# NguyenThaiHoc1/CustomKnowledgeGraphEmbedding

Measured on AMD Instinct MI355X. Metric: scored (pos+neg) triples/sec, WN18RR InterHT d=1000 n_neg=256, 1/2/4/8 GPU, higher is better.
Workload: dtype f32; 1 GPU; WN18RR InterHT d=1000 -de -tr gamma=24 n_neg=256 bz=512; global_batch=512, n_neg=256, hidden_dim=1000, score_function=InterHT, parallelism=single

## Files before the change

### customknowledgegraphembedding_amd/_lib.py

```python
from __future__ import annotations

import ctypes
import os
import threading

_HERE = os.path.dirname(os.path.abspath(__file__))
LIB_PATH = os.environ.get("KGE_HIP_LIB", os.path.join(_HERE, "libkge_hip.so"))

FN_IDS = {
    "TransE": 0,
    "DistMult": 1,
    "ComplEx": 2,
    "RotatE": 3,
    "InterHT": 4,
    "pRotatE": 5,
    "PairRE": 7,
}
HEAD_BATCH, TAIL_BATCH, SINGLE = 0, 1, 3

_c_i64 = ctypes.c_int64
_c_f = ctypes.c_float
_c_p = ctypes.c_void_p
_c_i = ctypes.c_int



class Forms(ctypes.Structure):
    _fields_ = [("step_order", ctypes.c_int), ("xcd_phases", ctypes.c_int), ("tile_rows", ctypes.c_int),
                ("tile_q2slots", ctypes.c_int), ("tile_waves", ctypes.c_int), ("gemm_form", ctypes.c_int),
                ("transparse_form", ctypes.c_int)]


_ORDERS = {"row": 0, "xcd": 1, "tile": 2}


def forms(step_order=None, xcd_phases=0, tile_rows=0, tile_q2slots=None, tile_waves=0, gemm_form=0,
          transparse_form=0):
    so = -1 if step_order is None else (_ORDERS[step_order] if isinstance(step_order, str) else int(step_order))
    return Forms(so, int(xcd_phases), int(tile_rows or 0), -1 if tile_q2slots is None else int(tile_q2slots),
                 int(tile_waves or 0), int(gemm_form), int(transparse_form))


SIGNATURES = {
    "kge_abi_version": (_c_i, []),
    "kge_last_error": (ctypes.c_char_p, []),
    "kge_max_dim": (_c_i64, [_c_i]),
    "kge_step_forward_order": (_c_i, [_c_i64, _c_i64]),
    "kge_score_indexed": (
        _c_i,
        [_c_i, _c_i, _c_p, _c_i64, _c_i64, _c_p, _c_i64, _c_i64, _c_i64, _c_p, _c_p, _c_i64,
         _c_i64, _c_i64, _c_i64, _c_f, _c_f, _c_f, _c_p, _c_i64, _c_p],
    ),
    "kge_step_forward": (
        _c_i,
        [_c_i, _c_i, _c_p, _c_i64, _c_i64, _c_p, _c_i64, _c_i64, _c_i64, _c_p, _c_p, _c_i64,
         _c_i64, _c_i64, _c_i64, _c_f, _c_f, _c_f, _c_f, _c_i, _c_p, _c_i64, _c_p, _c_p, _c_p, _c_p, _c_p],
    ),
    "kge_score_indexed_ex": (
        _c_i,
        [_c_i, _c_i, _c_p, _c_i64, _c_i64, _c_p, _c_i64, _c_i64, _c_i64, _c_p, _c_p, _c_i64,
         _c_i64, _c_i64, _c_i64, _c_f, _c_f, _c_f, _c_p, _c_i64, _c_p, _c_p],
    ),
    "kge_step_forward_ex": (
        _c_i,
        [_c_i, _c_i, _c_p, _c_i64, _c_i64, _c_p, _c_i64, _c_i64, _c_i64, _c_p, _c_p, _c_i64,
         _c_i64, _c_i64, _c_i64, _c_f, _c_f, _c_f, _c_f, _c_i, _c_p, _c_i64, _c_p, _c_p, _c_p, _c_p, _c_p, _c_p],
    ),
    "kge_step_plan_size": (_c_i64, [_c_i, _c_i64, _c_i64, _c_i64, _c_i64, _c_i64, _c_i64, _c_i64, _c_i64]),
    "kge_step_plan": (
        _c_i, [_c_i, _c_i, _c_i64, _c_i64, _c_i64, _c_i64, _c_i64, _c_p, _c_p, _c_i64, _c_i64, _c_i64, _c_i64, _c_p,
               _c_p]),
    "kge_step_forward_planned": (
        _c_i,
        [_c_i, _c_i, _c_p, _c_i64, _c_i64, _c_p, _c_i64, _c_i64, _c_i64, _c_i64, _c_i64, _c_i64, _c_f, _c_f, _c_f,
         _c_f, _c_i, _c_p, _c_p, _c_p, _c_i64, _c_i, _c_p, _c_p, _c_i64, _c_p, _c_p, _c_p, _c_p],
    ),
    "kge_step_planner_create": (
        _c_i, [_c_p, _c_i, _c_p, _c_i64, _c_i64, _c_p, _c_i64, _c_i64, _c_i64, _c_i64, _c_i64, _c_i64, _c_f, _c_f, _c_f,
               _c_f, _c_i, _c_p, _c_p, _c_i64, _c_p]),
    "kge_step_planner_set_modulus": (_c_i, [_c_p, _c_f]),
    "kge_step_planner_set_sweep": (_c_i, [_c_p, _c_i]),
    "kge_step_planner_set_form": (_c_i, [_c_p, _c_i, _c_i]),
    "kge_step_board_size": (_c_i64, []),
    "kge_step_planner_set_board": (_c_i, [_c_p, _c_p, _c_i64]),
    "kge_step_planner_set_lead": (_c_i, [_c_p, _c_i]),
    "kge_step_planner_get": (_c_i, [_c_p, _c_i]),
    "kge_step_planner_plan_size": (_c_i64, [_c_i, _c_i64, _c_i64, _c_i64, _c_i64, _c_i64, _c_i64, _c_i64, _c_i64]),
    "kge_step_planner_set_rows": (_c_i, [_c_p, _c_i]),
    "kge_step_planned_rows": (_c_i, [_c_i, _c_i64, _c_i64, _c_i64, _c_i64, _c_i64, _c_i64, _c_i64, _c_i64, _c_i,
                                     _c_i64, _c_p]),
    "kge_step_planner_set_clocks": (_c_i, [_c_p, _c_p, _c_i64]),
    "kge_step_planner_plan": (_c_i, [_c_p, _c_p, _c_p, _c_i64, _c_i]),
    "kge_step_planner_step": (_c_i, [_c_p, _c_p, _c_p, _c_i64, _c_i, _c_p, _c_p, _c_p, _c_p]),
    "kge_step_planner_destroy": (_c_i, [_c_p]),
    "kge_step_finish": (
        _c_i,
        [_c_i, _c_p, _c_i64, _c_i64, _c_p, _c_i64, _c_i64, _c_i64, _c_p, _c_i64, _c_i64,
         _c_f, _c_f, _c_f, _c_p, _c_i64, _c_i64, _c_f, _c_i, _c_p, _c_p, _c_p, _c_p],
    ),
    "kge_score_sharded": (
        _c_i,
        [_c_i, _c_i, _c_p, _c_i64, _c_p, _c_i64, _c_i64, _c_i64, _c_p, _c_i64, _c_i64, _c_i64,
         _c_p, _c_p, _c_i64, _c_i64, _c_i64, _c_i64, _c_f, _c_f, _c_f, _c_p, _c_i64, _c_p],
    ),
    "kge_gather_rows": (
        _c_i, [_c_p, _c_i64, _c_i64, _c_i64, _c_p, _c_i64, _c_i64, _c_i64, _c_p, _c_i64, _c_p]),
    "kge_build_id": (ctypes.c_char_p, []),
    "kge_source_hash": (ctypes.c_char_p, []),
    "kge_shard_plan": (
        _c_i, [_c_p, _c_p, _c_i64, _c_i64, _c_i64, _c_i64, _c_i, _c_i, _c_i, _c_i, _c_i, _c_p, _c_p, _c_p, _c_p, _c_p,
               _c_p, _c_p, _c_p]),
    "kge_shard_gather_queries": (
        _c_i, [_c_p, _c_i64, _c_i64, _c_i64, _c_p, _c_i64, _c_i, _c_i, _c_i64, _c_i, _c_i, _c_i, _c_i, _c_p, _c_p,
               _c_p, _c_p, _c_p, _c_p]),
    "kge_shard_score": (
        _c_i,
        [_c_i, _c_i, _c_p, _c_i64, _c_i64, _c_p, _c_p, _c_i64, _c_i64, _c_i64, _c_p, _c_i64, _c_i64, _c_i64,
         _c_p, _c_i64, _c_i64, _c_i64, _c_f, _c_f, _c_f, _c_p, _c_p, _c_p, _c_p, _c_p, _c_i, _c_i, _c_i64,
         _c_i64, _c_p, _c_p],
    ),
    "kge_shard_finish": (
        _c_i, [_c_p, _c_p, _c_p, _c_p, _c_p, _c_i64, _c_i64, _c_i64, _c_i64, _c_i, _c_i, _c_i, _c_f, _c_i, _c_p,
               _c_i64, _c_p, _c_p, _c_p, _c_p]),
    "kge_comm_unique_id": (_c_i, [_c_p]),
    "kge_comm_loopback_group": (_c_p, [_c_i]),
    "kge_comm_loopback_group_destroy": (_c_i, [_c_p]),
    "kge_comm_loopback_init": (_c_i, [_c_p, _c_p, _c_i]),
    "kge_comm_init": (_c_i, [_c_p, _c_p, _c_i, _c_i]),
    "kge_comm_destroy": (_c_i, [_c_p]),
    "kge_comm_all_to_allv": (_c_i, [_c_p, _c_p, _c_p, _c_p, _c_p, _c_p]),
    "kge_comm_all_reduce_sum": (_c_i, [_c_p, _c_p, _c_i64, _c_p]),
    "kge_shard_exec_workspace_size": (_c_i64, [_c_i64, _c_i64, _c_i64, _c_i, _c_i]),
    "kge_shard_exec_host_ints": (_c_i64, [_c_i, _c_i]),
    "kge_shard_exec_create": (
        _c_i, [_c_p, _c_p, _c_i, _c_i, _c_i64, _c_i64, _c_i64, _c_i64, _c_i64, _c_i64, _c_i, _c_i, _c_i, _c_p, _c_i64,
               _c_p, _c_i64]),
    "kge_shard_exec_destroy": (_c_i, [_c_p]),
    "kge_shard_exec_host_wait_us": (ctypes.c_double, [_c_p, _c_i]),
    "kge_shard_exec_timings": (_c_i, [_c_p, _c_p, _c_i]),
    "kge_comm_size": (_c_i, [_c_p]),
    "kge_shard_exec_plan": (_c_i, [_c_p, _c_p, _c_p, _c_i64, _c_i, _c_p]),
    "kge_shard_exec_step": (
        _c_i, [_c_p, _c_p, _c_i64, _c_i64, _c_p, _c_i64, _c_i64, _c_i64, _c_p, _c_p, _c_i64, _c_i, _c_f, _c_f, _c_f,
               _c_f, _c_i, _c_p, _c_p, _c_i, _c_p, _c_i64, _c_p, _c_p, _c_p, _c_p]),
    "kge_eval_query": (
        _c_i, [_c_i, _c_i, _c_p, _c_i64, _c_i64, _c_p, _c_i64, _c_i64, _c_p, _c_i64, _c_i64, _c_p, _c_i64, _c_p]),
    "kge_eval_query_planes": (
        _c_i, [_c_i, _c_i, _c_p, _c_i64, _c_i64, _c_p, _c_i64, _c_i64, _c_p, _c_i64, _c_i64, _c_p, _c_i64, _c_p]),
    "kge_gemm_nt": (_c_i, [_c_p, _c_i64, _c_p, _c_i64, _c_p, _c_i64, _c_i64, _c_i64, _c_i64, _c_p]),
    "kge_gemm_nt_bf16x3": (_c_i, [_c_p, _c_i64, _c_p, _c_i64, _c_p, _c_i64, _c_i64, _c_i64, _c_i64, _c_p]),
    "kge_gemm_nt_bf16x3_ex": (_c_i, [_c_p, _c_i64, _c_p, _c_i64, _c_p, _c_i64, _c_i64, _c_i64, _c_i64, _c_p, _c_p]),
    "kge_split_bf16x3_bytes": (_c_i64, [_c_i64, _c_i64]),
    "kge_split_bf16x3": (_c_i, [_c_p, _c_i64, _c_i64, _c_i64, _c_p, _c_i64, _c_p]),
    "kge_gemm_nt_bf16x3_planes": (_c_i, [_c_p, _c_i64, _c_p, _c_i64, _c_i64, _c_p, _c_i64, _c_i64, _c_i64, _c_p]),
    "kge_eval_rank_planes_workspace_size": (_c_i64, [_c_i64, _c_i64]),
    "kge_eval_rank_planes": (_c_i, [_c_p, _c_i64, _c_p, _c_i64, _c_i64, _c_i64, _c_i64, _c_p, _c_p, _c_p, _c_i64, _c_p,
                                    _c_p, ctypes.c_size_t, _c_p]),
    "kge_eval_rank_planes_ex": (_c_i, [_c_p, _c_i64, _c_p, _c_i64, _c_i64, _c_i64, _c_i64, _c_p, _c_p, _c_p, _c_i64,
                                       _c_p, _c_p, ctypes.c_size_t, _c_p, _c_p]),
    "kge_eval_rank_planes_phases": (_c_i, [_c_p, _c_i64, _c_p, _c_i64, _c_i64, _c_i64, _c_i64, _c_p, _c_p, _c_p,
                                           _c_i64, _c_p, _c_p, ctypes.c_size_t, _c_i, _c_p, _c_p]),
    "kge_eval_rank_sweep_workspace_size": (_c_i64, [_c_i64, _c_i64]),
    "kge_eval_rank_sweep": (_c_i, [_c_i, _c_i, _c_p, _c_i64, _c_i64, _c_p, _c_i64, _c_i64, _c_i64, _c_p, _c_i64, _c_i64,
                                   _c_f, _c_f, _c_f, _c_p, _c_p, _c_p, _c_i64, _c_p, _c_p, ctypes.c_size_t, _c_p]),
    "kge_eval_rank_candidates": (_c_i, [_c_i, _c_i, _c_p, _c_i64, _c_i64, _c_p, _c_i64, _c_i64, _c_i64, _c_p, _c_i64,
                                        _c_i64, _c_f, _c_f, _c_f, _c_p, _c_p, _c_i64, _c_i64, _c_p, _c_p, _c_i64, _c_p,
                                        _c_p, _c_p, _c_p]),
    "kge_eval_topk_sweep_workspace_size": (_c_i64, [_c_i64, _c_i64]),
    "kge_eval_topk_sweep": (_c_i, [_c_i, _c_i, _c_p, _c_i64, _c_i64, _c_p, _c_i64, _c_i64, _c_i64, _c_p, _c_i64, _c_i64,
                                   _c_f, _c_f, _c_f, _c_p, _c_p, _c_i64, _c_i64, _c_p, _c_i64, _c_p, _c_i64, _c_p,
                                   ctypes.c_size_t, _c_p]),
    "kge_topk_rows": (_c_i, [_c_p, _c_i64, _c_i64, _c_i64, _c_p, _c_p, _c_i64, _c_i64, _c_p, _c_i64, _c_p, _c_i64,
                             _c_p]),
    "kge_eval_topk_planes_workspace_size": (_c_i64, [_c_i64, _c_i64, _c_i64]),
    "kge_eval_topk_planes": (_c_i, [_c_p, _c_i64, _c_p, _c_i64, _c_i64, _c_i64, _c_i64, _c_p, _c_p, _c_i64, _c_i64,
                                    _c_p, _c_i64, _c_p, _c_i64, _c_p, ctypes.c_size_t, _c_p]),
    "kge_gemm_nt_bf16x3_planes_ex": (_c_i, [_c_p, _c_i64, _c_p, _c_i64, _c_i64, _c_p, _c_i64, _c_i64, _c_i64, _c_p,
                                            _c_p]),
    "kge_rank_filtered": (_c_i, [_c_p, _c_i64, _c_i64, _c_i64, _c_p, _c_p, _c_p, _c_p, _c_p]),
    "kge_score_dense": (
        _c_i,
        [_c_i, _c_i, _c_p, _c_i64, _c_p, _c_i64, _c_i64, _c_p, _c_i64, _c_i64, _c_i64, _c_i64,
         _c_f, _c_f, _c_f, _c_p, _c_i64, _c_p],
    ),
    "kge_score_dense_bwd": (
        _c_i,
        [_c_i, _c_i, _c_p, _c_i64, _c_p, _c_i64, _c_i64, _c_p, _c_i64, _c_i64, _c_i64, _c_i64,
         _c_f, _c_f, _c_f, _c_p, _c_i64, _c_p, _c_p, _c_p, _c_p, _c_p],
    ),
    "kge_neg_reduce": (_c_i, [_c_p, _c_i64, _c_i64, _c_i64, _c_f, _c_i, _c_p, _c_p]),
    "kge_neg_reduce_bwd": (
        _c_i, [_c_p, _c_i64, _c_i64, _c_i64, _c_f, _c_i, _c_i, _c_p, _c_p, _c_i64, _c_p]),
    "kge_log_sigmoid": (_c_i, [_c_p, _c_i64, _c_p, _c_p]),
    "kge_log_sigmoid_bwd": (_c_i, [_c_p, _c_p, _c_i64, _c_p, _c_p]),
    "kge_adam_update": (
        _c_i, [_c_p, _c_p, _c_p, _c_p, _c_i64, _c_f, _c_f, _c_f, _c_f, _c_i64, _c_i, _c_i, _c_p]),
    "kge_step_backward_workspace_size": (_c_i64, [_c_i, _c_i64, _c_i64, _c_i64, _c_i64]),
    "kge_step_backward": (
        _c_i,
        [_c_i, _c_i, _c_p, _c_i64, _c_i64, _c_p, _c_i64, _c_i64, _c_i64, _c_p, _c_p, _c_i64,
         _c_i64, _c_i64, _c_i64, _c_f, _c_f, _c_f, _c_f, _c_i, _c_i, _c_p, _c_i64, _c_p, _c_p, _c_p,
         _c_p, _c_p, _c_p, _c_p, _c_p, _c_i64, _c_p],
    ),
    "kge_step_backward_adam_workspace_size": (_c_i64, [_c_i, _c_i64, _c_i64, _c_i64, _c_i64, _c_i64, _c_i64]),
    "kge_step_backward_adam": (
        _c_i,
        [_c_i, _c_i, _c_p, _c_i64, _c_i64, _c_p, _c_i64, _c_i64, _c_i64, _c_p, _c_p, _c_i64,
         _c_i64, _c_i64, _c_i64, _c_f, _c_f, _c_p, _c_f, _c_f, _c_i, _c_i, _c_p, _c_i64, _c_p, _c_p, _c_p,
         _c_p, _c_p, _c_p, _c_p, _c_p, _c_p, _c_f, _c_f, _c_f, _c_f, _c_i64, _c_i, _c_p, _c_p, _c_i64, _c_p],
    ),
    "kge_train_step_workspace_size": (_c_i64, [_c_i, _c_i64, _c_i64, _c_i64, _c_i64, _c_i64, _c_i64]),
    "kge_train_step": (
        _c_i,
        [_c_i, _c_i, _c_p, _c_i64, _c_i64, _c_p, _c_i64, _c_i64, _c_i64, _c_p, _c_p, _c_i64,
         _c_i64, _c_i64, _c_i64, _c_f, _c_f, _c_f, _c_i, _c_i, _c_p, _c_p, _c_p, _c_p, _c_p,
         _c_p, _c_p, _c_p, _c_p, _c_f, _c_f, _c_f, _c_f, _c_i64, _c_i, _c_p, _c_i64, _c_p],
    ),
    "kge_train_step_reg_workspace_size": (_c_i64, [_c_i, _c_i64, _c_i64, _c_i64, _c_i64, _c_i64, _c_i64]),
    "kge_train_step_reg": (
        _c_i,
        [_c_i, _c_i, _c_p, _c_i64, _c_i64, _c_p, _c_i64, _c_i64, _c_i64, _c_p, _c_p, _c_i64,
         _c_i64, _c_i64, _c_i64, _c_f, _c_f, _c_f, _c_i, _c_i, _c_p, _c_p, _c_p, _c_p, _c_p,
         _c_p, _c_p, _c_p, _c_p, _c_f, _c_f, _c_f, _c_f, _c_i64, _c_i, _c_p, _c_i64, _c_p, _c_f, _c_p],
    ),
    "kge_train_step_lazy_workspace_size": (_c_i64, [_c_i, _c_i64, _c_i64, _c_i64, _c_i64, _c_i64, _c_i64]),
    "kge_train_step_lazy": (
        _c_i,
        [_c_i, _c_i, _c_p, _c_i64, _c_i64, _c_p, _c_i64, _c_i64, _c_i64, _c_p, _c_p, _c_i64,
         _c_i64, _c_i64, _c_i64, _c_f, _c_f, _c_f, _c_i, _c_i, _c_p, _c_p, _c_p, _c_p, _c_p,
         _c_p, _c_p, _c_p, _c_p, _c_f, _c_f, _c_f, _c_f, _c_i64, _c_i, _c_p, _c_i64, _c_p, _c_p],
    ),
    "kge_sampler_create": (_c_p, [_c_p, _c_i64, _c_i64, _c_i64, _c_i64, _c_i]),
    "kge_sampler_seed": (_c_i, [_c_p, ctypes.c_uint32]),
    "kge_sampler_get": (_c_i, [_c_p, _c_p, _c_i64, _c_p, _c_p, _c_p]),
    "kge_sampler_destroy": (None, [_c_p]),
    "kge_dsampler_table_size": (_c_i64, [_c_i64]),
    "kge_dsampler_table_build": (_c_i, [_c_p, _c_i64, _c_i64, _c_i64, _c_p, _c_i64]),
    "kge_dsampler_sample": (_c_i, [_c_p, _c_i64, _c_p, _c_i64, _c_i64, _c_i64, _c_i, ctypes.c_uint64, _c_i64, _c_p,
                                   _c_p, _c_p, _c_i64, _c_p, _c_p]),
    "kge_filter_table_size": (_c_i64, [_c_i64]),
    "kge_filter_table_build": (_c_i, [_c_p, _c_i64, _c_p, _c_i64]),
# ... 101 lines not shown
```

### customknowledgegraphembedding_amd/csrc/kge_abi.hip

```cpp
#include <string.h>

#include <algorithm>
#include <cmath>

#include <string>

#include "kge_device.h"
#include "kge_scan.h"

namespace kge_impl {
namespace {

__global__ __launch_bounds__(kBlock) void neg_reduce_kernel(const float* __restrict__ s, int64_t B, int64_t N,
                                                            int64_t ld, float T, int adversarial,
                                                            float* __restrict__ out) {
    const int64_t b = (int64_t)blockIdx.x * kWavesPerBlock + (threadIdx.x >> 6);
    if (b >= B) return;
    const int lane = threadIdx.x & 63;
    const float res = row_reduce_fast(s + b * ld, N, T, adversarial, lane);
    if (lane == 0) out[b] = res;
}

__global__ __launch_bounds__(kBlock) void neg_rows_kernel(ScoreParams p) {
    const int64_t b = (int64_t)blockIdx.x * kWavesPerBlock + (threadIdx.x >> 6);
// ... 379 lines not shown

int check_launch(const char* what) {
    const hipError_t e = hipGetLastError();
    if (e != hipSuccess) return fail(KGE_EHIP, std::string(what) + ": " + hipGetErrorString(e));
    return ok();
}

bool aligned(const void* ptr, int bytes) { return ptr == nullptr || ((uintptr_t)ptr % (uintptr_t)bytes) == 0; }

bool valid_fn(int fn) {
    switch (fn) {
        case KGE_TRANSE:
        case KGE_DISTMULT:
        case KGE_COMPLEX:
        case KGE_ROTATE:
        case KGE_INTERHT:
        case KGE_PROTATE:
        case KGE_PAIRRE: return true;
        default: return false;
    }
}

int check_rel_width(int fn, int64_t D, int64_t rel_off, int64_t rel_ld) {
    if (fn == KGE_PAIRRE && (rel_off < 0 || rel_ld < rel_off + 2 * D))
        return fail(KGE_EINVAL, "PairRE relation rows hold two halves: rel_ld >= rel_off + 2 D");
    return 0;
}

int refuse_sharded(int fn, const char* who) {
    if (fn == KGE_PAIRRE) return fail(KGE_ENOTSUP, std::string(who) + ": PairRE has no row-sharded form");
    return 0;
}

struct Tables {
    int fn;
    const float* ent;
    int64_t nentity, ent_ld;
    const float* rel;
    int64_t nrelation, rel_ld, rel_off;
    int64_t D;
    float gamma, emb_range, modulus;
};
struct Batch {
    int mode;
    const int64_t* pos;
    const int64_t* neg;
    int64_t neg_ld, B, N;
};
struct StepGrads {
    float temperature;
    int adversarial, detach;
    const float* neg_scores;
    int64_t ns_ld;
    const float* pos_scores;
    const float* d_out_neg;
    const float* d_out_pos;
    float* d_ent;
    float* d_rel;
    float* d_modulus;
    const float* cand_stats;
};

int pick_vg(const ScoreParams& p, int& V, int& G) {
    const int cand[3] = {4, 2, 1};
    V = 1;
    for (int v : cand) {
        if (p.D % v == 0 && p.q_ld % v == 0 && p.r_ld % v == 0 && p.r_off % v == 0 && p.c_ld % v == 0 &&
            aligned(p.qent, 4 * v) && aligned(p.rel, 4 * v) && aligned(p.cent, 4 * v) &&
            aligned(p.qent_pos, 4 * v) && aligned(p.sh_dq, 4 * v)) {
            V = v;
            break;
        }
    }
    const int groups = (p.D / V + kWave - 1) / kWave;
    G = 1;
    while (G < groups) G <<= 1;
    if (G > kMaxG)
        return fail(KGE_ENOTSUP, "per-half dim " + std::to_string(p.D) + " exceeds the register-resident limit " +
                                     std::to_string(kMaxG * kWave * V) + " for vector width " + std::to_string(V));
    return 0;
}

int pick_cpw(int64_t B, int64_t N) {
    if (N <= 1) return 1;
    int64_t cpw = 16;
    while (cpw > 4 && B * ((N + cpw - 1) / cpw) < 8192) cpw >>= 1;
    return (int)cpw;
}

int pick_cpw_sharded(int64_t B, int64_t N) {
    if (N <= 1) return 1;
    int64_t cpw = 512;
    while (cpw > 16 && B * ((N + cpw - 1) / cpw) < 8192) cpw >>= 1;
    return (int)cpw;
}

int dispatch(int fn, const ScoreParams& p, int kind, hipStream_t st, int blocks, bool ch, int V, int G) {
    switch (fn) {
        case KGE_TRANSE: return launch_transe(p, kind, st, blocks, ch, V, G);
        case KGE_DISTMULT: return launch_distmult(p, kind, st, blocks, ch, V, G);
        case KGE_COMPLEX: return launch_complex(p, kind, st, blocks, ch, V, G);
        case KGE_ROTATE: return launch_rotate(p, kind, st, blocks, ch, V, G);
        case KGE_INTERHT: return launch_interht(p, kind, st, blocks, ch, V, G);
        case KGE_PROTATE: return launch_protate(p, kind, st, blocks, ch, V, G);
        case KGE_PAIRRE: return launch_pairre(p, kind, st, blocks, ch, V, G);
        default: return KGE_EINVAL;
    }
}

int check_fn_mode(int fn, int mode) {
    if (mode != KGE_HEAD_BATCH && mode != KGE_TAIL_BATCH && mode != KGE_SINGLE)
        return fail(KGE_EINVAL, "mode must be 0 (head-batch), 1 (tail-batch) or 3 (single)");
    if (!valid_fn(fn)) return fail(KGE_EINVAL, "unknown score function id " + std::to_string(fn));
    return 0;
}

int run_score(int fn, int mode, ScoreParams& p, int kind, void* stream) {
    int rc = check_fn_mode(fn, mode);
    if (rc) return rc;
    if (p.B < 0 || p.N < 0 || p.D <= 0) return fail(KGE_EINVAL, "bad shape (B, N, D)");
    if (p.B == 0 || (p.N == 0 && kind != KIND_RANK_CAND)) return ok();
    const bool no_rows =
        p.c_rows == 0 && (kind == KIND_SHARD_FWD_GRAD || kind == KIND_SHARD_POS || kind == KIND_SHARD_EPILOGUE);
    rc = check_rel_width(fn, p.D, p.r_off, p.r_ld);
    if (rc) return rc;
    if (!p.qent || !p.rel || (!p.cent && !no_rows)) return fail(KGE_EINVAL, "null table pointer");
    int V = 1, G = 1;
    rc = pick_vg(p, V, G);
    if (rc) return rc;
    if (kind == KIND_BWD) {
        int g1 = 1;
        while (g1 * kWave < p.D) g1 <<= 1;
        if (g1 <= kBwdMaxG) {
            V = 1;
            G = g1;
        }
    }
    const KindInfo& k = kKinds[kind];
    int64_t waves = 0;
    switch (k.grid) {
        case GRID_WAVE_PER_ROW:
            if (kind == KIND_FINISH) p.cpw = p.wpr = 1;
            waves = p.B;
            break;
        case GRID_BLOCK_PER_ROW: waves = p.B * kWavesPerBlock; break;
        case GRID_WAVE_PER_ENT: waves = p.lz_list ? p.lz_rows : p.c_rows; break;
        case GRID_BLOCK_PER_ENT: waves = (p.lz_list ? p.lz_rows : p.c_rows) * kWavesPerBlock; break;
        case GRID_XCD_SLICES:
            waves = (p.B + kWavesPerBlock - 1) / kWavesPerBlock * kWavesPerBlock * 8;
            if (kind == KIND_STEP_FWD_XCD && p.xcd_phases > 1) waves *= p.xcd_phases;
            break;
        case GRID_TILE_GROUPS: {
            if (p.tile_rows < 1 || p.tile_lds > kTileLdsMax) return fail(KGE_EINVAL, "tile plan missing");
            const int64_t groups = (p.B + p.tile_rows - 1) / p.tile_rows;
            p.tile_blocks = (int)(groups * 8);
            waves = (groups * 8 + (p.tile_next.plan ? p.tile_plan_blocks : 0)) * kWavesPerBlock;
            break;
        }
        case GRID_CAND_PER_WAVE:
            p.cpw = p.skip_foreign ? pick_cpw_sharded(p.B, p.N) : pick_cpw(p.B, p.N);
            p.wpr = (int)((p.N + p.cpw - 1) / p.cpw);
            waves = p.B * p.wpr;
            break;
        case GRID_STEP_EPILOGUE: {
            const int64_t ev = p.B * p.N + 3 * p.B;
            const int64_t sb = std::min<int64_t>(std::max<int64_t>((ev + 4 * kBlock - 1) / (4 * kBlock), 1), 256);
            waves = (3 * p.B + kWavesPerBlock - 1) / kWavesPerBlock * kWavesPerBlock + (sb + 1) * kWavesPerBlock;
            break;
        }
        case GRID_SHARD_EPILOGUE:
            waves = (2 * p.B + kWavesPerBlock - 1) / kWavesPerBlock * kWavesPerBlock + kWavesPerBlock;
            break;
        case GRID_RANK_PAIRS: waves = p.B + p.rk.nf; break;
        case GRID_RANK_SWEEP:
            if (p.tile_rows < 1 || p.rk.chunks < 1 || p.tile_lds > kTileLdsMax) return fail(KGE_EINVAL, "sweep plan missing");
            waves = (p.B + p.tile_rows - 1) / p.tile_rows * 8 * p.rk.chunks * kWavesPerBlock;
            break;
        case GRID_TOPK_SWEEP:
            if (p.tile_rows < 1 || p.tk.chunks < 1 || p.tile_lds > kTileLdsMax || p.tk.k < 1 || p.tk.k > kTopkMax || !p.tk.parts)
                return fail(KGE_EINVAL, "sweep plan missing");
            waves = (p.B + p.tile_rows - 1) / p.tile_rows * 8 * p.tk.chunks * kWavesPerBlock;
            break;
        case GRID_RANK_CAND: {
            p.wpr = rank_cand_wpr(p.N);
            const int64_t rows = kWavesPerBlock / p.wpr;
            waves = (p.B + rows - 1) / rows * kWavesPerBlock;
            break;
        }
    }
    const int64_t blocks = (waves + kWavesPerBlock - 1) / kWavesPerBlock;
    if (blocks > INT32_MAX) return fail(KGE_EINVAL, "problem too large for one launch");
    const bool ch = k.ch && mode == KGE_HEAD_BATCH;
    if (k.no_protate && (G > k.max_g || fn == KGE_PROTATE))
        return fail(KGE_ENOTSUP, "the fused forward + query gradient needs D / V <= 256 and no pRotatE");
    if (G > k.max_g) return fail(KGE_ENOTSUP, "dimension too large");
    if (k.g_whole_waves && G % kWavesPerBlock) return fail(KGE_ENOTSUP, "the streaming backward needs G % 4 == 0");
    rc = kind_has(kind, fn, ch, G) ? dispatch(fn, p, kind, (hipStream_t)stream, (int)blocks, ch, V, G) : KGE_ENOTSUP;
    if (rc) return fail(rc, "no kernel for this (function, width) combination");
    return check_launch(k.what);
}

float phase_div_for(int fn, float emb_range) {
    const double pi = (fn == KGE_PROTATE) ? 3.14159262358979323846 : 3.14159265358979323846;
    return (float)((double)emb_range / pi);
}

void fill_indexed(ScoreParams& p, const Tables& t, const Batch& b) {
    memset(&p, 0, sizeof(p));
    const bool ch = b.mode == KGE_HEAD_BATCH;
    p.qent = t.ent;
    p.q_idx = b.pos ? b.pos + (ch ? 2 : 0) : nullptr;
    p.q_ld = t.ent_ld;
    p.q_stride = 3;
    p.q_rows = t.nentity;
    p.rel = t.rel;
    p.r_idx = b.pos ? b.pos + 1 : nullptr;
    p.r_ld = t.rel_ld;
    p.r_stride = 3;
    p.r_rows = t.nrelation;
    p.r_off = t.rel_off;
    p.cent = t.ent;
    p.c_ld = t.ent_ld;
    p.c_rows = t.nentity;
    if (b.mode == KGE_SINGLE) {
        p.c_idx = b.pos ? b.pos + 2 : nullptr;
        p.c_stride = 3;
    } else {
        p.c_idx = b.neg;
        p.c_stride = b.neg_ld;
    }
    p.B = b.B;
    p.N = b.mode == KGE_SINGLE ? 1 : b.N;
    p.D = (int)t.D;
    p.gamma = t.gamma;
    p.phase_div = phase_div_for(t.fn, t.emb_range);
    p.modulus = t.modulus;
}
Batch single_of(const Batch& b) { return {KGE_SINGLE, b.pos, nullptr, 0, b.B, 1}; }

void fill_dense(ScoreParams& p, int fn, int mode, const float* head, int64_t head_ld, const float* rel,
                int64_t rel_ld, int64_t rel_off, const float* tail, int64_t tail_ld, int64_t B, int64_t N, int64_t D,
                float gamma, float emb_range, float modulus) {
    memset(&p, 0, sizeof(p));
    const bool ch = mode == KGE_HEAD_BATCH;
    if (mode == KGE_SINGLE) N = 1;
    p.qent = ch ? tail : head;
    p.q_ld = ch ? tail_ld : head_ld;
    p.q_rows = B;
    p.rel = rel;
    p.r_ld = rel_ld;
    p.r_off = rel_off;
    p.r_rows = B;
    p.cent = ch ? head : tail;
    p.c_ld = ch ? head_ld : tail_ld;
    p.c_dense = N;
    p.c_rows = B * N;
    p.B = B;
    p.N = N;
    p.D = (int)D;
    p.gamma = gamma;
    p.phase_div = phase_div_for(fn, emb_range);
    p.modulus = modulus;
}

bool empty(int64_t B, int64_t N) { return B == 0 || N == 0; }

int xcd_phases(int64_t nentity, int64_t ent_ld, const kge_forms* forms) {
    const int forced = forms ? forms->xcd_phases : 0;
    if (forced > 0) return std::min(forced, 16);
    const int64_t bytes = nentity * ent_ld * 4, mall = (int64_t)256 << 20, phase = (int64_t)96 << 20;
    if (bytes <= mall) return 1;
    return (int)std::min<int64_t>((bytes + phase - 1) / phase, 8);
}

int step_order(int64_t nentity, int64_t N, const kge_forms* forms = nullptr) {
    const int forced = forms ? forms->step_order : -1;
    if (nentity >= (int64_t)8 << 25) return 0;
    if (forced >= 0 && forced <= 2) return forced;
    return N >= 128 ? 2 : 0;
}
bool use_xcd_order(int64_t nentity, int64_t N, const kge_forms* forms = nullptr) {
    return step_order(nentity, N, forms) != 0;
}

int tile_plan(int fn, ScoreParams& p, const kge_forms* forms = nullptr) {
    int V = 1, G = 1;
    if (pick_vg(p, V, G)) return 0;
    if (G > kFwdGradMaxG || p.N + 1 > 65536 || p.c_rows <= 0) return 0;
    const int64_t opb = (int64_t)G * kWave * V * 4;
    int64_t P2 = 0;
    if (fn == KGE_INTERHT && p.B <= kTileSortMaxB) {
        P2 = kWave;
        while (P2 < p.B) P2 <<= 1;
    }
    const int64_t row_bytes = (int64_t)p.D * 4 * (is_split(fn) ? 2 : 1);
    p.tile_waves = row_bytes >= 4096 ? 12 : 16;
    p.tile_depth = 2;
    const int fw = forms ? forms->tile_waves : 0;
    if (fw == 8 || fw == 12 || fw == 16) p.tile_waves = fw;
    const int64_t NT = (int64_t)p.tile_waves * kWave;
    const int64_t qrow = tile_nq(fn) * opb + 8 + 8 + 8 + 4, lrow = (p.N + 1) * 4;
    const int64_t fixed = kTileBuckets * 4 + 16;
    const int64_t sort_ints = P2 ? (kTileSortMaxB + NT - 1) / NT * p.tile_waves * kTileSortRel : 0;
    auto lds = [&](int64_t R, int64_t QS) { return R * qrow + QS * opb + fixed + std::max(R * lrow, sort_ints * 4); };
    int64_t R = kTileRows;
    if (forms && forms->tile_rows > 0) R = std::min<int64_t>(R, forms->tile_rows);
    while (R >= 1 && lds(R, 0) > kTileLdsMax) --R;
    if (R < 1) return 0;
    int64_t QS = 0;
    if (fn == KGE_INTERHT)
        while (QS < R && lds(R, QS + 1) <= kTileLdsMax) ++QS;
    if (forms && forms->tile_q2slots >= 0) QS = std::min<int64_t>(QS, forms->tile_q2slots);
#ifdef KGE_PROFILING_KNOBS
    p.tile_dry = getenv("KGE_TILE_DRY") ? std::max(1, atoi(getenv("KGE_TILE_DRY"))) : 0;
    if (getenv("KGE_TILE_NOSORT")) P2 = 0;
#endif
    p.tile_rows = (int)R;
    p.tile_q2slots = (int)QS;
    p.tile_sort = (int)P2;
    p.tile_lds = (int)lds(R, QS);
    return 1;
}

int planned_tile_params(const Tables& t, int64_t B, int64_t N, ScoreParams& p, const kge_forms* forms = nullptr) {
    if (B <= 0 || N <= 0 || t.D <= 0 || t.nentity <= 0 || t.nentity >= ((int64_t)1 << 31) || B >= ((int64_t)1 << 31))
        return 0;
    Tables a = t;
    a.ent = a.rel = reinterpret_cast<const float*>((uintptr_t)4096);
    fill_indexed(p, a, {KGE_TAIL_BATCH, nullptr, nullptr, 0, B, N});
    return tile_plan(t.fn, p, forms) ? p.tile_rows : 0;
}

int planned_tile_layout(int fn, ScoreParams& p, int64_t R) {
    int V = 1, G = 1;
    if (pick_vg(p, V, G)) return 0;
    const int64_t opb = (int64_t)G * kWave * V * 4;
    const int64_t qrow = tile_nq(fn) * opb + 8 + 8 + 8 + 4, fixed = kTileBuckets * 4 + 16;
    auto lds = [&](int64_t r, int64_t qs) { return r * qrow + qs * opb + fixed; };
    if (R < 1 || R > std::min(kTileMaxRows, 2 * p.tile_waves) || lds(R, 0) > kTileLdsMax) return 0;
    int64_t QS = 0;
    if (fn == KGE_INTERHT)
        while (QS < R && lds(R, QS + 1) <= kTileLdsMax) ++QS;
    p.tile_rows = (int)R;
    p.tile_q2slots = (int)QS;
    p.tile_lds = (int)lds(R, QS);
    return 1;
}

template <class Cap>
int planned_rows_rule(const Tables& t, int64_t B, int64_t N, int waves, int64_t plan_bytes, Cap cap) {
    ScoreParams tp;
    const int R0 = planned_tile_params(t, B, N, tp);
    if (!R0) return 0;
    const int qs0 = tp.tile_q2slots;
    if (waves) tp.tile_waves = waves;
    const int64_t c0 = cap(R0);
    if (c0 <= 0 || 8 * plan_groups(B, R0) <= c0 - 8) return R0;
    for (int R = R0 + 1; R <= kTileMaxRows; ++R) {
        if (!planned_tile_layout(t.fn, tp, R) || tp.tile_q2slots < qs0) continue;
        if (plan_bytes > 0 && plan_words(B, N, R) * 4 > plan_bytes) continue;
        const int64_t c = cap(R);
        if (c > 0 && 8 * plan_groups(B, R) <= c - 8) return R;
    }
    return R0;
}

struct SweepForm {
    int waves, depth, lead, tag;
    int rev;
    int* board;
    long long* clk;
};

void planned_sweep_defaults(int fn, int64_t D, int& waves, int& depth, int& lead) {
    const int64_t row_bytes = D * 4 * (is_split(fn) ? 2 : 1);
    waves = row_bytes >= 4096 ? 12 : 16;
    depth = 2;
    lead = 0;
    if (row_bytes >= 4096 && fn == KGE_INTERHT) lead = 12;
    if (row_bytes >= 4096 && fn == KGE_ROTATE) depth = 1;
}

PlanArgs plan_args(const ScoreParams& tp, const Tables& t, const Batch& b, void* plan) {
    PlanArgs a;
    a.pos = b.pos;
    a.neg = b.neg;
    a.neg_ld = b.neg_ld;
    a.B = b.B;
    a.N = b.N;
    a.nent = t.nentity;
    a.nrel = t.nrelation;
    a.mode = b.mode;
    a.R = tp.tile_rows;
    a.sort = tp.tile_sort != 0;
    a.plan = reinterpret_cast<int*>(plan);
    return a;
}

int launch_neg_rows(const ScoreParams& p, const char* what, void* stream) {
    const int64_t blocks = (p.B + kWavesPerBlock - 1) / kWavesPerBlock;
    hipLaunchKernelGGL(neg_rows_kernel, dim3((unsigned)blocks), dim3(kBlock), 0, (hipStream_t)stream, p);
    return check_launch(what);
}

}

int set_error(int code, const char* msg) { return fail(code, msg); }
}

using namespace kge_impl;

extern "C" {

int kge_abi_version(void) { return KGE_ABI_VERSION; }

const char* kge_last_error(void) { return g_last_error.c_str(); }

int64_t kge_max_dim(int fn) {
    if (!valid_fn(fn)) return 0;
    return (int64_t)kMaxG * kWave * 4;
}

int kge_step_forward_order(int64_t nentity, int64_t N) { return step_order(nentity, N); }

int kge_score_indexed(int fn, int mode, const float* ent, int64_t nentity, int64_t ent_ld, const float* rel,
                      int64_t nrelation, int64_t rel_ld, int64_t rel_off, const int64_t* pos, const int64_t* neg,
                      int64_t neg_ld, int64_t B, int64_t N, int64_t D, float gamma, float emb_range, float modulus,
                      float* scores, int64_t scores_ld, void* stream) {
    return kge_score_indexed_ex(fn, mode, ent, nentity, ent_ld, rel, nrelation, rel_ld, rel_off, pos, neg, neg_ld, B,
                                N, D, gamma, emb_range, modulus, scores, scores_ld, nullptr, stream);
}

int kge_score_indexed_ex(int fn, int mode, const float* ent, int64_t nentity, int64_t ent_ld, const float* rel,
                         int64_t nrelation, int64_t rel_ld, int64_t rel_off, const int64_t* pos, const int64_t* neg,
                         int64_t neg_ld, int64_t B, int64_t N, int64_t D, float gamma, float emb_range, float modulus,
                         float* scores, int64_t scores_ld, const kge_forms* forms, void* stream) {
    int rc = check_fn_mode(fn, mode);
    if (rc) return rc;
    if (B < 0 || N < 0 || D <= 0) return fail(KGE_EINVAL, "bad shape (B, N, D)");
    if (empty(B, mode == KGE_SINGLE ? 1 : N)) return ok();
    if (!pos) return fail(KGE_EINVAL, "pos must not be NULL");
    if (mode != KGE_SINGLE && !neg) return fail(KGE_EINVAL, "neg must not be NULL in head/tail-batch mode");
    if (!scores) return fail(KGE_EINVAL, "scores must not be NULL");
    const Tables t = {fn, ent, nentity, ent_ld, rel, nrelation, rel_ld, rel_off, D, gamma, emb_range, modulus};
    ScoreParams p;
    fill_indexed(p, t, {mode, pos, neg, neg_ld, B, N});
    p.out = scores;
    p.out_ld = scores_ld;
    if (mode != KGE_SINGLE && nentity < ((int64_t)1 << 31) && use_xcd_order(nentity, N, forms)) {
        if (step_order(nentity, N, forms) == 2 && tile_plan(fn, p, forms))
            return run_score(fn, mode, p, KIND_SCORE_TILE, stream);
        return run_score(fn, mode, p, KIND_SCORE_SHARD_XCD, stream);
    }
    return run_score(fn, mode, p, KIND_FWD, stream);
}

int kge_step_finish(int fn, const float* ent, int64_t nentity, int64_t ent_ld, const float* rel, int64_t nrelation,
                    int64_t rel_ld, int64_t rel_off, const int64_t* pos, int64_t B, int64_t D, float gamma,
                    float emb_range, float modulus, const float* neg_scores, int64_t N, int64_t ns_ld,
                    float temperature, int adversarial, float* out_neg, float* pos_scores, float* out_pos,
                    void* stream) {
    int rc = check_fn_mode(fn, KGE_SINGLE);
    if (rc) return rc;
    if (B < 0 || N <= 0 || D <= 0) return fail(KGE_EINVAL, "bad shape (B, N, D)");
    if (B == 0) return ok();
    if (!pos || !neg_scores || !out_neg || !out_pos) return fail(KGE_EINVAL, "null pointer");
    const Tables t = {fn, ent, nentity, ent_ld, rel, nrelation, rel_ld, rel_off, D, gamma, emb_range, modulus};
    ScoreParams f;
    fill_indexed(f, t, {KGE_SINGLE, pos, nullptr, 0, B, 1});
    f.neg_scores = neg_scores;
    f.ns_ld = ns_ld;
    f.n_neg = N;
    f.temperature = temperature;
    f.adversarial = adversarial;
    f.out_neg = out_neg;
    f.out_pos_raw = pos_scores;
    f.out_pos_ls = out_pos;
    return run_score(fn, KGE_SINGLE, f, KIND_FINISH, stream);
}

int kge_step_forward(int fn, int mode, const float* ent, int64_t nentity, int64_t ent_ld, const float* rel,
                     int64_t nrelation, int64_t rel_ld, int64_t rel_off, const int64_t* pos, const int64_t* neg,
                     int64_t neg_ld, int64_t B, int64_t N, int64_t D, float gamma, float emb_range, float modulus,
                     float temperature, int adversarial, float* neg_scores, int64_t ns_ld, float* out_neg,
                     float* pos_scores, float* out_pos, float* cand_stats, void* stream) {
    return kge_step_forward_ex(fn, mode, ent, nentity, ent_ld, rel, nrelation, rel_ld, rel_off, pos, neg, neg_ld, B, N,
                               D, gamma, emb_range, modulus, temperature, adversarial, neg_scores, ns_ld, out_neg,
                               pos_scores, out_pos, cand_stats, nullptr, stream);
}

int kge_step_forward_ex(int fn, int mode, const float* ent, int64_t nentity, int64_t ent_ld, const float* rel,
                        int64_t nrelation, int64_t rel_ld, int64_t rel_off, const int64_t* pos, const int64_t* neg,
                        int64_t neg_ld, int64_t B, int64_t N, int64_t D, float gamma, float emb_range, float modulus,
                        float temperature, int adversarial, float* neg_scores, int64_t ns_ld, float* out_neg,
                        float* pos_scores, float* out_pos, float* cand_stats, const kge_forms* forms, void* stream) {
    int rc = check_fn_mode(fn, mode);
    if (rc) return rc;
    if (mode == KGE_SINGLE) return fail(KGE_EINVAL, "kge_step_forward needs a negative mode (0 or 1)");
    if (B < 0 || N <= 0 || D <= 0) return fail(KGE_EINVAL, "bad shape (B, N, D)");
    if (B == 0) return ok();
    if (!pos || !neg || !neg_scores || !out_neg || !out_pos) return fail(KGE_EINVAL, "null pointer");
    const Tables t = {fn, ent, nentity, ent_ld, rel, nrelation, rel_ld, rel_off, D, gamma, emb_range, modulus};
    ScoreParams p;
    fill_indexed(p, t, {mode, pos, neg, neg_ld, B, N});
    p.out = neg_scores;
    p.out_ld = ns_ld;
    p.cand_stats = reinterpret_cast<float2*>(cand_stats);
    p.pos_base = pos;
    p.temperature = temperature;
    p.adversarial = adversarial;
    p.out_neg = out_neg;
    p.out_pos_raw = pos_scores;
    p.out_pos_ls = out_pos;
    const int order = step_order(nentity, N, forms);
    if (!(cand_stats && fn == KGE_INTERHT) && order != 0) {
        if (order == 2 && tile_plan(fn, p, forms)) {
            p.tile_pos = 1;
            rc = run_score(fn, mode, p, KIND_STEP_FWD_TILE, stream);
        } else {
            p.xcd_phases = xcd_phases(nentity, ent_ld, forms);
            rc = run_score(fn, mode, p, KIND_STEP_FWD_XCD, stream);
        }
        if (rc) return rc;
        return launch_neg_rows(p, "kge_step_forward row reductions", stream);
    }
    return run_score(fn, mode, p, (cand_stats && fn == KGE_INTERHT) ? KIND_STEP_FWD_STATS : KIND_STEP_FWD, stream);
}

static int64_t step_plan_bytes(const Tables& t, int64_t B, int64_t N) {
    if (!valid_fn(t.fn)) return 0;
    ScoreParams tp;
    const int R = planned_tile_params(t, B, N, tp);
    return R ? plan_words(B, N, R) * 4 : 0;
}

int64_t kge_step_plan_size(int fn, int64_t nentity, int64_t ent_ld, int64_t nrelation, int64_t rel_ld,
                           int64_t rel_off, int64_t B, int64_t N, int64_t D) {
    return step_plan_bytes({fn, nullptr, nentity, ent_ld, nullptr, nrelation, rel_ld, rel_off, D, 0.f, 0.f, 0.f}, B, N);
}

static int step_plan(const Tables& t, const Batch& b, void* plan, void* stream, int rows = 0) {
    if (!valid_fn(t.fn)) return fail(KGE_EINVAL, "unknown score function id " + std::to_string(t.fn));
    if (b.mode != KGE_HEAD_BATCH && b.mode != KGE_TAIL_BATCH)
        return fail(KGE_EINVAL, "kge_step_plan needs a negative mode (0 or 1)");
    if (b.B <= 0 || b.N <= 0 || t.D <= 0) return fail(KGE_EINVAL, "bad shape (B, N, D)");
    if (!b.pos || !b.neg || !plan) return fail(KGE_EINVAL, "null pointer");
    if (!aligned(plan, 16)) return fail(KGE_EINVAL, "the plan must be 16-B aligned");
    ScoreParams tp;
    if (!planned_tile_params(t, b.B, b.N, tp))
        return fail(KGE_ENOTSUP, "the tile form does not apply to this shape (kge_step_plan_size is 0)");
    if (rows) tp.tile_rows = rows;
    const PlanArgs a = plan_args(tp, t, b, plan);
    const unsigned groups = (unsigned)plan_groups(b.B, tp.tile_rows);
    if (tp.tile_waves == 16)
        hipLaunchKernelGGL(tile_plan_kernel<16>, dim3(groups), dim3(16 * kWave), plan_lds_ints(16 * kWave) * 4,
                           (hipStream_t)stream, a);
    else
        hipLaunchKernelGGL(tile_plan_kernel<12>, dim3(groups), dim3(12 * kWave), plan_lds_ints(12 * kWave) * 4,
                           (hipStream_t)stream, a);
    return check_launch("kge_step_plan");
}

int kge_step_plan(int fn, int mode, int64_t nentity, int64_t ent_ld, int64_t nrelation, int64_t rel_ld,
                  int64_t rel_off, const int64_t* pos, const int64_t* neg, int64_t neg_ld, int64_t B, int64_t N,
                  int64_t D, void* plan, void* stream) {
    return step_plan({fn, nullptr, nentity, ent_ld, nullptr, nrelation, rel_ld, rel_off, D, 0.f, 0.f, 0.f},
                     {mode, pos, neg, neg_ld, B, N}, plan, stream);
}

struct StepOut {
    float* neg_scores;
    int64_t ns_ld;
    float *out_neg, *pos_scores, *out_pos;
};

static int step_forward_planned(const Tables& t, const Batch& b, float temperature, int adversarial, const void* plan,
                                const Batch& next, void* next_plan, const StepOut& o, const SweepForm* sf,
                                void* stream, int rows = 0, int* occ = nullptr, int plan_blocks = 0) {
    int rc = check_fn_mode(t.fn, b.mode);
    if (rc) return rc;
    if (b.mode == KGE_SINGLE) return fail(KGE_EINVAL, "kge_step_forward_planned needs a negative mode (0 or 1)");
    if (b.B <= 0 || b.N <= 0 || t.D <= 0) return fail(KGE_EINVAL, "bad shape (B, N, D)");
    if (!t.ent || !t.rel || !plan || !o.neg_scores || !o.out_neg || !o.out_pos) return fail(KGE_EINVAL, "null pointer");
    if (next_plan) {
        if (next.mode != KGE_HEAD_BATCH && next.mode != KGE_TAIL_BATCH)
            return fail(KGE_EINVAL, "the next batch needs a negative mode (0 or 1)");
        if (!next.pos || !next.neg) return fail(KGE_EINVAL, "next_plan needs next_pos and next_neg");
        if (next_plan == plan) return fail(KGE_EINVAL, "next_plan must not be the plan this step reads");
        if (!aligned(next_plan, 16)) return fail(KGE_EINVAL, "the plan must be 16-B aligned");
    }
    if (!aligned(plan, 16)) return fail(KGE_EINVAL, "the plan must be 16-B aligned");
    ScoreParams tp;
    const int R = planned_tile_params(t, b.B, b.N, tp);
    ScoreParams p;
    fill_indexed(p, t, {b.mode, nullptr, nullptr, 0, b.B, b.N});
    kge_forms fm = {-1, 0, 0, -1, sf ? sf->waves : 0, 0, 0};
    if (!R || !tile_plan(t.fn, p, &fm) || p.tile_rows != R)
        return fail(KGE_ENOTSUP, "the tile form does not apply to these tables (unaligned rows, or "
                                 "kge_step_plan_size is 0): use kge_step_forward");
    if (!planned_tile_layout(t.fn, p, rows ? rows : R))
        return fail(KGE_ENOTSUP, "this many rows per group do not fit a block of the planned step");
    tp.tile_rows = p.tile_rows;
    p.out = o.neg_scores;
    p.out_ld = o.ns_ld;
    p.pos_base = nullptr;
    p.temperature = temperature;
    p.adversarial = adversarial;
    p.out_neg = o.out_neg;
    p.out_pos_raw = o.pos_scores;
    p.out_pos_ls = o.out_pos;
    p.tile_pos = 1;
    p.tile_plan = reinterpret_cast<const int*>(plan);
    if (sf) {
        p.tile_rev = sf->rev;
        p.tile_depth = sf->depth;
        p.tile_board = sf->board;
        p.tile_tag = sf->tag;
        p.tile_lead = sf->lead;
        p.tile_clk = sf->clk;
    }
    if (next_plan) {
        p.tile_next = plan_args(tp, t, next, next_plan);
        const int ng = (int)plan_groups(next.B, tp.tile_rows);
        p.tile_plan_blocks = (plan_blocks > 0 && p.tile_waves == kTileSharedWaves) ? std::min(plan_blocks, ng) : ng;
        p.tile_lds = std::max(p.tile_lds, plan_lds_ints(p.tile_waves * kWave) * 4);
    }
    p.tile_occ = occ;
    rc = run_score(t.fn, b.mode, p, KIND_STEP_FWD_TILE, stream);
    if (rc || occ) return rc;
    return launch_neg_rows(p, "kge_step_forward_planned row reductions", stream);
}

int kge_step_forward_planned(int fn, int mode, const float* ent, int64_t nentity, int64_t ent_ld, const float* rel,
                             int64_t nrelation, int64_t rel_ld, int64_t rel_off, int64_t B, int64_t N, int64_t D,
                             float gamma, float emb_range, float modulus, float temperature, int adversarial,
                             const void* plan, const int64_t* next_pos, const int64_t* next_neg, int64_t next_neg_ld,
                             int next_mode, void* next_plan, float* neg_scores, int64_t ns_ld, float* out_neg,
                             float* pos_scores, float* out_pos, void* stream) {
    const Tables t = {fn, ent, nentity, ent_ld, rel, nrelation, rel_ld, rel_off, D, gamma, emb_range, modulus};
    return step_forward_planned(t, {mode, nullptr, nullptr, 0, B, N}, temperature, adversarial, plan,
                                {next_mode, next_pos, next_neg, next_neg_ld, B, N}, next_plan,
                                {neg_scores, ns_ld, out_neg, pos_scores, out_pos}, nullptr, stream);
}

int planner_row_rule(int fn, int64_t D) {
    const int64_t row_bytes = D * 4 * (is_split(fn) ? 2 : 1);
    return row_bytes >= 4096 && (fn == KGE_INTERHT || fn == KGE_ROTATE);
}

struct kge_step_planner {
    Tables t = {};
    int64_t B = 0, N = 0;
    float temperature = 1.f;
    int adversarial = 1;
    void* plans[2] = {nullptr, nullptr};
    int cur = -1;
    int mode = 0;
    int sweep = 1;
    int waves = 0, depth = 0, lead = -1;
    int* board = nullptr;
    long long* clk = nullptr;
    int cus = 0;
    int64_t groups = 0;
    int rows = 0;
    int rule = 0;
    int plan_blocks = 0;
    int64_t plan_bytes = 0;
    int64_t steps = 0;
    void* stream = nullptr;
};

static SweepForm planner_form(const kge_step_planner* sp, int64_t groups = -1) {
    if (groups < 0) groups = sp->groups;
    SweepForm f = {0, 0, 0, 0, sp->sweep ? (int)(sp->steps & 1) : 0, nullptr, sp->clk};
    planned_sweep_defaults(sp->t.fn, sp->t.D, f.waves, f.depth, f.lead);
    if (sp->waves) f.waves = sp->waves;
    if (sp->depth) f.depth = sp->depth;
    if (f.waves == 8) f.depth = 2;
    if (sp->lead >= 0) f.lead = sp->lead;
    f.tag = (int)(sp->steps % kSweepTagMask) + 1;
    if (sp->board && f.lead > 0 && groups <= kSweepBoardLine && groups * 8 <= sp->cus) f.board = sp->board;
    return f;
}

static int64_t planner_capacity(const kge_step_planner* sp, int R) {
    if (sp->cus <= 0) return 0;
    const SweepForm sf = planner_form(sp, plan_groups(sp->B, R));
    int per_cu = INT32_MAX;
    float* const none = reinterpret_cast<float*>(sp->plans[0]);
    const int64_t* const ids = reinterpret_cast<const int64_t*>(sp->plans[0]);
    for (int mode : {KGE_HEAD_BATCH, KGE_TAIL_BATCH}) {
        int occ = 0;
        if (step_forward_planned(sp->t, {mode, nullptr, nullptr, 0, sp->B, sp->N}, sp->temperature, sp->adversarial,
                                 sp->plans[0], {mode, ids, ids, sp->N, sp->B, sp->N}, sp->plans[1],
                                 {none, sp->N, none, none, none}, &sf, sp->stream, R, &occ, 8))
            return 0;
        per_cu = std::min(per_cu, occ);
    }
    return (int64_t)sp->cus * per_cu;
}

static int planner_rows(kge_step_planner* sp) {
    if (!sp->rows) {
        sp->rows = planned_rows_rule(sp->t, sp->B, sp->N, planner_form(sp).waves, sp->plan_bytes,
                                     [&](int R) { return sp->rule ? planner_capacity(sp, R) : 0; });
        if (plan_groups(sp->B, sp->rows) > sp->groups) sp->clk = nullptr;
        sp->groups = plan_groups(sp->B, sp->rows);
        const int64_t cap = sp->rule ? planner_capacity(sp, sp->rows) : 0;
        sp->plan_blocks = (cap > 0 && 8 * sp->groups <= cap - 8) ? 8 : 0;
    }
    return sp->rows;
}

int64_t kge_step_planner_plan_size(int fn, int64_t nentity, int64_t ent_ld, int64_t nrelation, int64_t rel_ld,
                                   int64_t rel_off, int64_t B, int64_t N, int64_t D) {
    const Tables t = {fn, nullptr, nentity, ent_ld, nullptr, nrelation, rel_ld, rel_off, D, 0.f, 0.f, 0.f};
    if (!valid_fn(fn)) return 0;
    ScoreParams tp;
    const int R0 = planned_tile_params(t, B, N, tp);
    int64_t words = 0;
    for (int R = R0; R0 && R <= kTileMaxRows; ++R) words = std::max(words, plan_words(B, N, R));
    return words * 4;
}

int kge_step_planned_rows(int fn, int64_t nentity, int64_t ent_ld, int64_t nrelation, int64_t rel_ld, int64_t rel_off,
                          int64_t B, int64_t N, int64_t D, int waves, int64_t capacity, int* out) {
    if (!valid_fn(fn)) return fail(KGE_EINVAL, "unknown score function id " + std::to_string(fn));
    if (!out || (waves != 0 && waves != 8 && waves != 12 && waves != 16))
        return fail(KGE_EINVAL, "kge_step_planned_rows: out[4]; waves 0, 8, 12 or 16");
    const Tables t = {fn, nullptr, nentity, ent_ld, nullptr, nrelation, rel_ld, rel_off, D, 0.f, 0.f, 0.f};
    const int R = planned_rows_rule(t, B, N, waves, 0, [&](int) { return capacity; });
    ScoreParams tp;
    if (!R || !planned_tile_params(t, B, N, tp)) return fail(KGE_ENOTSUP, "the tile form does not apply to this shape");
    if (waves) tp.tile_waves = waves;
    if (!planned_tile_layout(fn, tp, R)) return fail(KGE_ENOTSUP, "the rows do not fit this wave count");
    out[0] = R;
    out[1] = tp.tile_q2slots;
    out[2] = std::max(tp.tile_lds, plan_lds_ints(tp.tile_waves * kWave) * 4);
    out[3] = (int)(8 * plan_groups(B, R));
    return ok();
}

int kge_step_planner_create(kge_step_planner** out, int fn, const float* ent, int64_t nentity, int64_t ent_ld,
                            const float* rel, int64_t nrelation, int64_t rel_ld, int64_t rel_off, int64_t B, int64_t N,
                            int64_t D, float gamma, float emb_range, float modulus, float temperature, int adversarial,
                            void* plan0, void* plan1, int64_t plan_bytes, void* stream) {
    if (!out) return fail(KGE_EINVAL, "kge_step_planner_create: null pointer");
    *out = nullptr;
    const Tables t = {fn, ent, nentity, ent_ld, rel, nrelation, rel_ld, rel_off, D, gamma, emb_range, modulus};
    const int64_t need = step_plan_bytes(t, B, N);
    if (need <= 0) return fail(KGE_ENOTSUP, "kge_step_planner_create: the tile form does not apply to this shape");
    if (!ent || !rel || !plan0 || !plan1 || plan0 == plan1) return fail(KGE_EINVAL, "kge_step_planner_create: bad pointers");
    if (plan_bytes < need || !aligned(plan0, 16) || !aligned(plan1, 16))
        return fail(KGE_EINVAL, "kge_step_planner_create: plan buffers too small or not 16-B aligned");
    kge_step_planner* sp = new kge_step_planner;
    sp->t = t;
    sp->B = B;
    sp->N = N;
    sp->temperature = temperature;
    sp->adversarial = adversarial;
    sp->plans[0] = plan0;
    sp->plans[1] = plan1;
    sp->stream = stream;
    sp->plan_bytes = plan_bytes;
    sp->rule = planner_row_rule(fn, D);
    ScoreParams tp;
    sp->groups = plan_groups(B, planned_tile_params(t, B, N, tp));
    int dev = 0;
    if (hipGetDevice(&dev) != hipSuccess ||
        hipDeviceGetAttribute(&sp->cus, hipDeviceAttributeMultiprocessorCount, dev) != hipSuccess)
        sp->cus = 0;
    *out = sp;
    return ok();
}

int kge_step_planner_set_form(kge_step_planner* sp, int waves, int depth) {
    if (!sp) return fail(KGE_EINVAL, "kge_step_planner_set_form: null pointer");
    if ((waves != 0 && waves != 8 && waves != 12 && waves != 16) || depth < 0 || depth > 2 || (waves == 8 && depth == 1))
        return fail(KGE_EINVAL, "kge_step_planner_set_form: waves 0, 8, 12 or 16; depth 0, 1 or 2 (8 waves: not 1)");
    if (waves) {
        ScoreParams tp, tw;
        kge_forms fm = {-1, 0, 0, -1, waves, 0, 0};
        if (planned_tile_params(sp->t, sp->B, sp->N, tw, &fm) != planned_tile_params(sp->t, sp->B, sp->N, tp))
            return fail(KGE_ENOTSUP, "kge_step_planner_set_form: this wave count changes the rows per group");
    }
    if (waves && sp->rows > 2 * waves)
        return fail(KGE_ENOTSUP, "kge_step_planner_set_form: this wave count changes the rows per group");
    sp->waves = waves;
    sp->depth = depth;
    return ok();
}

int kge_step_planner_set_rows(kge_step_planner* sp, int rows) {
    if (!sp) return fail(KGE_EINVAL, "kge_step_planner_set_rows: null pointer");
    const bool chosen = rows > 0 || rows < KGE_PLANNER_ROWS_RULE;
    if (chosen) {
        ScoreParams tp;
        if (rows < 0 || !planned_tile_params(sp->t, sp->B, sp->N, tp)) return fail(KGE_EINVAL, "kge_step_planner_set_rows: bad rows");
        tp.tile_waves = planner_form(sp).waves;
        if (!planned_tile_layout(sp->t.fn, tp, rows))
            return fail(KGE_ENOTSUP, "kge_step_planner_set_rows: this many rows do not fit a block of this form");
        if (plan_words(sp->B, sp->N, rows) * 4 > sp->plan_bytes)
            return fail(KGE_EINVAL, "kge_step_planner_set_rows: the plan buffers are too small (kge_step_planner_plan_size)");
        if (plan_groups(sp->B, rows) > sp->groups) sp->clk = nullptr;
        sp->groups = plan_groups(sp->B, rows);
    }
    sp->rule = rows == KGE_PLANNER_ROWS_RULE || (rows == 0 && planner_row_rule(sp->t.fn, sp->t.D));
    sp->plan_blocks = 0;
    sp->rows = chosen ? rows : 0;
    return ok();
}

int64_t kge_step_board_size(void) { return (int64_t)kSweepBoardInts * 4; }

int kge_step_planner_set_board(kge_step_planner* sp, void* board, int64_t board_bytes) {
    if (!sp) return fail(KGE_EINVAL, "kge_step_planner_set_board: null pointer");
    if (board && (board_bytes < kge_step_board_size() || !aligned(board, 4)))
        return fail(KGE_EINVAL, "kge_step_planner_set_board: kge_step_board_size bytes, 4-B aligned");
    sp->board = reinterpret_cast<int*>(board);
    return ok();
}

int kge_step_planner_set_lead(kge_step_planner* sp, int lead) {
    if (!sp) return fail(KGE_EINVAL, "kge_step_planner_set_lead: null pointer");
    if (lead < -1 || lead >= kTileBuckets) return fail(KGE_EINVAL, "kge_step_planner_set_lead: -1, 0 or 1..255 buckets");
    sp->lead = lead;
    return ok();
}

int kge_step_planner_get(const kge_step_planner* sp, int what) {
    if (!sp) return -1;
    const SweepForm f = planner_form(sp);
    switch (what) {
        case KGE_PLANNER_WAVES: return f.waves;
        case KGE_PLANNER_DEPTH: return f.depth;
        case KGE_PLANNER_LEAD: return f.lead;
        case KGE_PLANNER_THROTTLE: return f.board != nullptr;
        case KGE_PLANNER_TAG: return f.tag;
        case KGE_PLANNER_ROWS: return sp->rows;
        case KGE_PLANNER_PLAN_BLOCKS:
            return !sp->rows ? 0 : (sp->plan_blocks > 0 && f.waves == kTileSharedWaves) ? (int)std::min<int64_t>(sp->plan_blocks, sp->groups) : (int)sp->groups;
        default: return -1;
    }
}

int kge_step_planner_set_clocks(kge_step_planner* sp, void* clocks, int64_t clocks_bytes) {
#ifdef KGE_PROFILING_KNOBS
    if (!sp) return fail(KGE_EINVAL, "kge_step_planner_set_clocks: null pointer");
    if (clocks && (clocks_bytes < kge_sweep_clk_words(sp->groups) * 8 || !aligned(clocks, 8)))
        return fail(KGE_EINVAL, "kge_step_planner_set_clocks: groups * (8 * 40 + 2) * 8 bytes, 8-B aligned");
    sp->clk = reinterpret_cast<long long*>(clocks);
    return ok();
#else
    (void)sp;
    (void)clocks;
    (void)clocks_bytes;
    return fail(KGE_ENOTSUP, "kge_step_planner_set_clocks: a -DKGE_PROFILING_KNOBS build only");
#endif
}

int kge_step_planner_set_modulus(kge_step_planner* sp, float modulus) {
    if (!sp) return fail(KGE_EINVAL, "kge_step_planner_set_modulus: null pointer");
    sp->t.modulus = modulus;
    return ok();
}

int kge_step_planner_set_sweep(kge_step_planner* sp, int alternate) {
    if (!sp) return fail(KGE_EINVAL, "kge_step_planner_set_sweep: null pointer");
    if (alternate != 0 && alternate != 1) return fail(KGE_EINVAL, "kge_step_planner_set_sweep: 0 or 1");
    sp->sweep = alternate;
    return ok();
}

int kge_step_planner_plan(kge_step_planner* sp, const int64_t* pos, const int64_t* neg, int64_t neg_ld, int mode) {
    if (!sp) return fail(KGE_EINVAL, "kge_step_planner_plan: null pointer");
    const int buf = sp->cur < 0 ? 0 : sp->cur;
    const int rc = step_plan(sp->t, {mode, pos, neg, neg_ld, sp->B, sp->N}, sp->plans[buf], sp->stream, planner_rows(sp));
    if (rc) return rc;
    sp->cur = buf;
    sp->mode = mode;
    return ok();
}

int kge_step_planner_step(kge_step_planner* sp, const int64_t* next_pos, const int64_t* next_neg, int64_t next_neg_ld,
                          int next_mode, float* neg_scores, float* out_neg, float* pos_scores, float* out_pos) {
    if (!sp) return fail(KGE_EINVAL, "kge_step_planner_step: null pointer");
    if (sp->cur < 0) return fail(KGE_EINVAL, "kge_step_planner_step: no batch planned (kge_step_planner_plan first)");
    const bool nxt = next_pos && next_neg;
    const int rows = planner_rows(sp);
    const SweepForm sf = planner_form(sp);
    const int rc = step_forward_planned(sp->t, {sp->mode, nullptr, nullptr, 0, sp->B, sp->N}, sp->temperature,
                                        sp->adversarial, sp->plans[sp->cur],
                                        {next_mode, next_pos, next_neg, next_neg_ld, sp->B, sp->N},
                                        nxt ? sp->plans[1 - sp->cur] : nullptr,
                                        {neg_scores, sp->N, out_neg, pos_scores, out_pos}, &sf, sp->stream, rows,
                                        nullptr, sp->plan_blocks);
    if (rc) return rc;
    ++sp->steps;
    if (nxt) {
        sp->cur = 1 - sp->cur;
        sp->mode = next_mode;
    } else {
        sp->cur = -1;
    }
    return ok();
}

int kge_step_planner_destroy(kge_step_planner* sp) {
    delete sp;
    return ok();
}

int kge_score_sharded(int fn, int mode, const float* qent, int64_t q_ld, const float* rel, int64_t nrelation,
                      int64_t rel_ld, int64_t rel_off, const float* shard, int64_t shard_rows, int64_t shard_ld,
                      int64_t shard_lo, const int64_t* pos, const int64_t* neg, int64_t neg_ld, int64_t B, int64_t N,
                      int64_t D, float gamma, float emb_range, float modulus, float* scores, int64_t scores_ld,
                      void* stream) {
    int rc = check_fn_mode(fn, mode);
    if (rc) return rc;
    rc = refuse_sharded(fn, "kge_score_sharded");
    if (rc) return rc;
    if (B < 0 || N < 0 || D <= 0 || shard_rows < 0) return fail(KGE_EINVAL, "bad shape");
    if (empty(B, mode == KGE_SINGLE ? 1 : N)) return ok();
    if (!pos || (mode != KGE_SINGLE && !neg) || !scores || !qent || !shard)
        return fail(KGE_EINVAL, "null pointer");
    const Tables t = {fn, shard, shard_rows, shard_ld, rel, nrelation, rel_ld, rel_off, D, gamma, emb_range, modulus};
    ScoreParams p;
    fill_indexed(p, t, {mode, pos, neg, neg_ld, B, N});
    p.qent = qent;
    p.q_idx = nullptr;
    p.q_ld = q_ld;
    p.q_rows = B;
    p.c_base = shard_lo;
    p.skip_foreign = 1;
    p.out = scores;
    p.out_ld = scores_ld;
    if (mode != KGE_SINGLE && shard_lo >= 0 && shard_lo + shard_rows < ((int64_t)1 << 31) &&
        use_xcd_order(shard_rows, N))
        return run_score(fn, mode, p, KIND_SCORE_SHARD_XCD, stream);
    return run_score(fn, mode, p, KIND_FWD, stream);
}

int kge_shard_score(int fn, int mode, const float* qent, int64_t q_rows, int64_t q_ld, const int64_t* q_idx,
                    const float* rel, int64_t nrelation, int64_t rel_ld, int64_t rel_off, const float* shard,
                    int64_t shard_rows, int64_t shard_ld, int64_t shard_lo, const int64_t* pos, int64_t B, int64_t N,
                    int64_t D, float gamma, float emb_range, float modulus, const int* bucket,
                    const int* bucket_start, const int* pre, const int* cnt, const int* tot, int world, int rank,
                    int64_t home_B, int64_t home0, float* send, void* stream) {
    if (mode != KGE_HEAD_BATCH && mode != KGE_TAIL_BATCH)
        return fail(KGE_EINVAL, "kge_shard_score: mode must be 0 (head-batch) or 1 (tail-batch)");
    int rc = check_fn_mode(fn, mode);
    if (rc) return rc;
    rc = refuse_sharded(fn, "kge_shard_score");
    if (rc) return rc;
    if (B < 0 || N < 0 || D <= 0 || shard_rows <= 0 || q_rows < 0) return fail(KGE_EINVAL, "bad shape");
    if (world < 1 || rank < 0 || rank >= world || home_B <= 0 || B % home_B || home0 < 0 ||
        home0 + B / home_B > world)
        return fail(KGE_EINVAL, "kge_shard_score: rows must be whole homes of home_B rows");
    if (shard_lo < 0 || shard_rows >= ((int64_t)1 << 25))
        return fail(KGE_ENOTSUP, "kge_shard_score: the shard must hold < 2^25 rows");
    if (B == 0) return ok();
    if (!pos || !send || !qent || !q_idx || !shard || !bucket || !bucket_start || !pre || !cnt || !tot)
        return fail(KGE_EINVAL, "null pointer");
    const Tables t = {fn, shard, shard_rows, shard_ld, rel, nrelation, rel_ld, rel_off, D, gamma, emb_range, modulus};
    ScoreParams p;
    fill_indexed(p, t, {mode, pos, nullptr, 0, B, N + 1});
    p.qent = qent;
    p.q_idx = q_idx;
    p.q_stride = 1;
    p.q_ld = q_ld;
    p.q_rows = q_rows;
    p.c_idx = nullptr;
    p.c_base = shard_lo;
    p.skip_foreign = 1;
    p.pos_base = pos;
    p.bk_ent = reinterpret_cast<const int2*>(bucket);
    p.bk_start = bucket_start;
    p.bk_ld = N + 1;
    p.cmp_pre = pre;
    p.cmp_cnt = cnt;
    p.cmp_tot = tot;
    p.cmp_home0 = home0;
    p.home_B = home_B;
    p.world = world;
    p.rank = rank;
    p.out = send;
    p.out_ld = 0;
    return run_score(fn, mode, p, KIND_SHARD_BUCKET, stream);
}

int kge_gather_rows(const float* table, int64_t rows, int64_t ld, int64_t lo, const int64_t* ids, int64_t id_stride,
                    int64_t n, int64_t width, float* out, int64_t out_ld, void* stream) {
    if (n < 0 || width < 0 || rows < 0) return fail(KGE_EINVAL, "bad shape");
    if (n == 0 || width == 0) return ok();
    if (!table || !ids || !out) return fail(KGE_EINVAL, "null pointer");
    const int vec4 = (width % 4 == 0 && ld % 4 == 0 && out_ld % 4 == 0 && aligned(table, 16) && aligned(out, 16));
    const int64_t blocks = (n + kWavesPerBlock - 1) / kWavesPerBlock;
    hipLaunchKernelGGL(gather_owned_kernel, dim3((unsigned)blocks), dim3(kBlock), 0, (hipStream_t)stream, table, rows,
                       ld, lo, ids, id_stride, n, width, out, out_ld, vec4);
    return check_launch("kge_gather_rows");
}

int kge_eval_query(int fn, int mode, const float* ent, int64_t nentity, int64_t ent_ld, const float* rel,
                   int64_t nrelation, int64_t rel_ld, const int64_t* pos, int64_t B, int64_t D, float* Q, int64_t ldq,
                   void* stream) {
    int rc = check_fn_mode(fn, mode);
    if (rc) return rc;
    if (fn != KGE_DISTMULT && fn != KGE_COMPLEX)
        return fail(KGE_ENOTSUP, "kge_eval_query: only DistMult and ComplEx score as a dense contraction");
    if (mode == KGE_SINGLE) return fail(KGE_EINVAL, "kge_eval_query needs mode 0 or 1");
    if (B < 0 || D <= 0) return fail(KGE_EINVAL, "bad shape");
    if (B == 0) return ok();
    if (!ent || !rel || !pos || !Q) return fail(KGE_EINVAL, "null pointer");
    ScoreParams p;
    fill_indexed(p, {fn, ent, nentity, ent_ld, rel, nrelation, rel_ld, 0, D, 0.f, 1.f, 0.f},
                 {mode, pos, nullptr, 0, B, 1});
    int V = 1, G = 1;
    rc = pick_vg(p, V, G);
    if (rc) return rc;
    if (ldq % V) V = 1;
    while (V > 1 && !aligned(Q, 4 * V)) V >>= 1;
    G = 1;
    while (G * kWave * V < D) G <<= 1;
    if (G > kMaxG) return fail(KGE_ENOTSUP, "dimension too large");
    const int64_t blocks = (B + kWavesPerBlock - 1) / kWavesPerBlock;
    rc = launch_eval_query_any(fn, mode == KGE_HEAD_BATCH, p, (hipStream_t)stream, (int)blocks, V, G, Q, ldq);
    if (rc) return fail(rc, "no eval-query kernel for this width");
    return check_launch("kge_eval_query");
}

int kge_eval_query_planes(int fn, int mode, const float* ent, int64_t nentity, int64_t ent_ld, const float* rel,
                          int64_t nrelation, int64_t rel_ld, const int64_t* pos, int64_t B, int64_t D, void* planes,
                          int64_t plane_rows, void* stream) {
    int rc = check_fn_mode(fn, mode);
    if (rc) return rc;
    if (fn != KGE_DISTMULT && fn != KGE_COMPLEX)
        return fail(KGE_ENOTSUP, "kge_eval_query_planes: only DistMult and ComplEx score as a dense contraction");
    if (mode == KGE_SINGLE) return fail(KGE_EINVAL, "kge_eval_query_planes needs mode 0 or 1");
    if (B < 0 || D <= 0 || plane_rows < B) return fail(KGE_EINVAL, "bad shape");
    if (B == 0) return ok();
    if (!ent || !rel || !pos || !planes) return fail(KGE_EINVAL, "null pointer");
    if (!aligned(planes, 16)) return fail(KGE_EINVAL, "kge_eval_query_planes: planes not 16-B aligned");
    ScoreParams p;
    fill_indexed(p, {fn, ent, nentity, ent_ld, rel, nrelation, rel_ld, 0, D, 0.f, 1.f, 0.f},
                 {mode, pos, nullptr, 0, B, 1});
    int V = 1, G = 1;
    rc = pick_vg(p, V, G);
    if (rc) return rc;
    if (V != 4) return fail(KGE_ENOTSUP, "kge_eval_query_planes needs D % 4 == 0 and 16-B aligned tables");
// ... 1285 lines not shown
```

### customknowledgegraphembedding_amd/csrc/kge_device.h

```cpp
#pragma once

#include <math.h>

#include <type_traits>

#include "kge_internal.h"

namespace kge_impl {

template <int V>
struct alignas(4 * V) vecf {
    float a[V];
};

template <int V>
__device__ __forceinline__ vecf<V> vzero() {
    vecf<V> r;
#pragma unroll
    for (int i = 0; i < V; ++i) r.a[i] = 0.f;
    return r;
}

template <int V>
__device__ __forceinline__ vecf<V> vload(const float* p, bool ok) {
// ... 718 lines not shown
        const uint64_t m = __ballot(own);
        const int cnt = __popcll(m);
        const int n32 = (int)n;
        if (cnt == 0) continue;
        const int row32 = (int)row;
        const int d = lane - fill;
        const bool take = d >= 0 && d < cnt;
        const int src = kth_set_bit(m, take ? d : 0);
        const int r1 = lane_pull(row32, src), n1 = lane_pull(n32, src);
        if (take) {
            buf_row = r1;
            buf_n = n1;
        }
        if (fill + cnt >= kWave) {
            body(buf_row, buf_n, kWave);
            const int rest = fill + cnt - kWave;
            const int src2 = kth_set_bit(m, lane < rest ? (kWave - fill) + lane : 0);
            buf_row = lane_pull(row32, src2);
            buf_n = lane_pull(n32, src2);
            fill = rest;
        } else {
            fill += cnt;
        }
    }
    if (fill > 0) body(buf_row, buf_n, fill);
}

template <int FN, bool CH, int V, int G>
__device__ __forceinline__ void score_owned(const ScoreParams& p, const Query<FN, CH, V, G>& q, int64_t b, int64_t lo,
                                            int64_t hi, int lane) {
    for_owned_runs(p, b, lo, hi, lane, true, [&](int row, int n, int cnt) {
        const int64_t my_id = (int64_t)row + p.c_base;
        float2 st;
        const float s = score_lanes<FN, CH, V, G, false>(p, q, my_id, cnt, lane, st);
        if (lane < cnt) p.out[b * p.out_ld + n] = s;
    });
}

template <class Body>
__device__ __forceinline__ void for_slice_runs_sorted(const ScoreParams& p, int64_t b, int64_t e_lo, int64_t e_hi,
                                                      bool take_invalid, bool zero_foreign, int lane, Body&& body) {
    int buf_key = INT32_MAX, buf_id = -1, buf_n = 0, fill = 0;
    auto flush = [&](int cnt) {
        const int key = wave_sort_asc(lane < cnt ? buf_key : INT32_MAX, lane);
        const int src = key & (kWave - 1);
        const int id = lane_pull(buf_id, src), n = lane_pull(buf_n, src);
        body(id, n, cnt);
    };
    for (int64_t c0 = 0; c0 < p.N; c0 += kWave) {
        const int64_t n = c0 + lane;
        int64_t id = -1;
        if (n < p.N) id = p.c_idx[b * p.c_stride + n];
        const bool valid = id >= p.c_base && id < p.c_base + p.c_rows;
        const bool own = n < p.N && (valid ? (id >= e_lo && id < e_hi) : take_invalid);
        if (zero_foreign && n < p.N && !valid) p.out[b * p.out_ld + n] = 0.f;
        const int n32 = (int)n;
        const uint64_t m = __ballot(own);
        const int cnt = __popcll(m);
        if (cnt == 0) continue;
        const int id32 = valid ? (int)id : -1, rl = valid ? (int)(id - e_lo) : 0;
        const int d = lane - fill;
        const bool take = d >= 0 && d < cnt;
        const int src = kth_set_bit(m, take ? d : 0);
        const int i1 = lane_pull(id32, src), n1 = lane_pull(n32, src), r1 = lane_pull(rl, src);
        if (take) {
            buf_id = i1;
            buf_n = n1;
            buf_key = (r1 << 6) | lane;
        }
        if (fill + cnt >= kWave) {
            flush(kWave);
            const int rest = fill + cnt - kWave;
            const int src2 = kth_set_bit(m, lane < rest ? (kWave - fill) + lane : 0);
            buf_id = lane_pull(id32, src2);
            buf_n = lane_pull(n32, src2);
            buf_key = (lane_pull(rl, src2) << 6) | lane;
            fill = rest;
        } else {
            fill += cnt;
        }
    }
    if (fill > 0) flush(fill);
}

template <int FN, bool CH, int V, int G>
__global__ __attribute__((amdgpu_flat_work_group_size(1, kBlock), amdgpu_waves_per_eu(G <= 4 ? 4 : 1))) void
step_fwd_xcd_kernel(ScoreParams p) {
    __shared__ vecf<V> q2img[kWavesPerBlock][FN == KGE_INTERHT ? G * kWave : 1];
    const int P = p.xcd_phases > 1 ? p.xcd_phases : 1;
    const int64_t per_phase = (p.B + kWavesPerBlock - 1) / kWavesPerBlock * 8;
    const int phase = (int)(blockIdx.x / per_phase);
    const int64_t bi = blockIdx.x - phase * per_phase;
    const int x = (int)(bi & 7) + 8 * phase;
    const int w = threadIdx.x >> 6;
    const int64_t b = (bi >> 3) * kWavesPerBlock + w;
    if (b >= p.B) return;
    const int lane = threadIdx.x & 63;
    const int64_t S = (p.c_rows + 8 * P - 1) / (8 * P);
    const int64_t e_lo = min((int64_t)x * S, p.c_rows), e_hi = min(p.c_rows, e_lo + S);
    const int64_t t = p.pos_base[b * 3 + 2];
    const bool t_here = (t >= 0 && t < p.c_rows) ? (t >= e_lo && t < e_hi) : x == 0;
    Query<FN, CH, V, G> q;
    int64_t qi, ri;
    bool qok, rok;
    build_query_for<FN, CH, V, G>(p, b, lane, q, qi, ri, qok, rok);
    auto run = [&](const auto& qq) {
        for_slice_runs_sorted(p, b, e_lo, e_hi, x == 0, false, lane, [&](int id, int n, int cnt) {
            float2 st;
            const float s = score_lanes<FN, CH, V, G, false, std::decay_t<decltype(qq)>, 1>(p, qq, (int64_t)id, cnt, lane, st);
            if (lane < cnt) p.out[b * p.out_ld + n] = s;
        });
        if (!t_here) return;
        bool ok;
        Cand<FN, V, G> c;
        c.load(cand_row(p, t, ok), ok, p.D, lane);
        float s;
        if constexpr (!CH) {
            s = cand_score<FN, false, V, G>(c, fresh(qq), p);
        } else {
            Query<FN, false, V, G> qp;
            const int64_t hi = p.pos_base[b * 3], rj = p.pos_base[b * 3 + 1];
            const bool hok = hi >= 0 && hi < p.q_rows, rjok = rj >= 0 && rj < p.r_rows;
            qp.build(p.qent + (hok ? hi : 0) * p.q_ld, hok, p.rel + (rjok ? rj : 0) * p.r_ld + p.r_off, rjok, p.D,
                     lane, p);
            s = cand_score<FN, false, V, G>(c, qp, p);
        }
        if (lane == 0) {
            if (p.out_pos_raw) p.out_pos_raw[b] = s;
            p.out_pos_ls[b] = log_sigmoid(s);
        }
    };
    if constexpr (FN == KGE_INTERHT) {
        QueryL2<FN, CH, V, G> ql;
#pragma unroll
        for (int k = 0; k < G; ++k) {
            q2img[w][lane + k * kWave] = q.q2[k];
            ql.q0[k] = q.q0[k];
            ql.q1[k] = q.q1[k];
        }
        ql.q2 = LdsOperand<V>{q2img[w], lane};
        run(ql);
    } else {
        run(q);
    }
}


template <int V, int G>
struct TileQueryIH {
    LdsOperand<V> q0, q1;
    vecf<V> q2[G];
};

template <int NWV>
__device__ void tile_plan_group(const PlanArgs& a, int g, int* sm) {
    constexpr int NT = NWV * kWave, NB = kTileSortRel, MU = (kTileSortMaxB + NT - 1) / NT;
    const int t = threadIdx.x, lane = t & 63, w = t >> 6;
    const int R = a.R;
    const int64_t g0 = (int64_t)g * R;
    const int nr = (int)min<int64_t>(R, a.B - g0);
    int* brow = sm;
    int* hist = brow + kTileMaxRows;
    int* wc = hist + 8 * kTileBuckets;
    if (a.sort) {
        int bk[MU], wr[MU];
        int64_t rv[MU];
#pragma unroll
        for (int u = 0; u < MU; ++u) rv[u] = a.pos[min<int64_t>(u * NT + t, a.B - 1) * 3 + 1];
#pragma unroll
        for (int u = 0; u < MU; ++u) {
            const int64_t rr = rv[u];
            bk[u] = u * NT + t >= a.B ? NB : ((rr >= 0 && rr < a.nrel) ? (int)min<int64_t>(rr, NB - 2) : NB - 1);
        }
        for (int i = t; i < MU * NWV * NB; i += NT) wc[i] = 0;
        __syncthreads();
#pragma unroll
        for (int u = 0; u < MU; ++u) {
            wr[u] = 0;
            if (u * NT >= a.B) continue;
            uint64_t todo = __ballot(bk[u] < NB);
            while (todo) {
                const int v = __builtin_amdgcn_readlane(bk[u], __builtin_ctzll(todo));
                const uint64_t m = __ballot(bk[u] == v);
                if (bk[u] == v) wr[u] = lanes_below(m);
                if (lane == 0) wc[(u * NWV + w) * NB + v] = __popcll(m);
                todo &= ~m;
            }
        }
        __syncthreads();
        if (w == 0) {
            int y[MU * NWV];
#pragma unroll
            for (int c = 0; c < MU * NWV; ++c) y[c] = wc[c * NB + lane];
            int run = 0;
#pragma unroll
            for (int c = 0; c < MU * NWV; ++c) {
                const int v = y[c];
                y[c] = run;
                run += v;
            }
            int incl = run;
#pragma unroll
            for (int o = 1; o < kWave; o <<= 1) {
                const int v = __shfl_up(incl, o, kWave);
                if (lane >= o) incl += v;
            }
            const int base = incl - run;
#pragma unroll
            for (int c = 0; c < MU * NWV; ++c) wc[c * NB + lane] = y[c] + base;
        }
        __syncthreads();
#pragma unroll
        for (int u = 0; u < MU; ++u) {
            if (bk[u] >= NB) continue;
            const int64_t rank = wc[(u * NWV + w) * NB + bk[u]] + wr[u];
            if (rank >= g0 && rank < g0 + nr) brow[rank - g0] = u * NT + t;
        }
    } else if (t < nr) {
        brow[t] = (int)(g0 + t);
    }
    for (int i = t; i < 8 * kTileBuckets; i += NT) hist[i] = 0;
    __syncthreads();
    const int Np = a.mode == KGE_HEAD_BATCH ? (int)a.N : (int)a.N + 1;
    const int nf = nr * Np;
    const int64_t S = (a.nent + 7) / 8;
    const int S32 = (int)S;
    const float invS = 1.f / (float)S, bscale = (float)kTileBuckets / (float)S, inv_np = 1.f / (float)Np;
    auto item_row = [&](int f, int& r) {
        r = (int)((float)f * inv_np);
        if (r * Np > f) --r;
        if ((r + 1) * Np <= f) ++r;
        const int n = f - r * Np;
        const int64_t b = brow[r];
        const int64_t* src = n < a.N ? a.neg + b * a.neg_ld + n : a.pos + b * 3 + 2;
        return src;
    };
    auto classify = [&](int f, int r, int64_t id, int& key, int& idc, int& code) {
        const int n = f - r * Np;
        const bool valid = id >= 0 && id < a.nent;
        const int i32 = valid ? (int)id : 0;
        int x = min(7, (int)((float)i32 * invS));
        if (x * S32 > i32) --x;
        if (x < 7 && (x + 1) * S32 <= i32) ++x;
        const int bk = valid ? min(kTileBuckets - 1, (int)((float)(i32 - x * S32) * bscale)) : 0;
        if (!valid) x = 0;
        key = x * kTileBuckets + bk;
        idc = valid ? (int)id : -1;
        code = (r << 16) | n;
    };
    auto item = [&](int f, int& key, int& idc, int& code) {
        int r;
        const int64_t id = *item_row(f, r);
        classify(f, r, id, key, idc, code);
    };
    constexpr int TPI = 17;
    const bool in_regs = nf <= TPI * NT;
    int ky[TPI], ic[TPI], cd[TPI], rk[TPI];
    int64_t ph = -1, pr = -1, pt = -1;
    if (t < nr) {
        const int64_t b = brow[t];
        ph = a.pos[b * 3];
        pr = a.pos[b * 3 + 1];
        pt = a.pos[b * 3 + 2];
    }
    if (in_regs) {
        int64_t idv[TPI];
        int rr[TPI];
#pragma unroll
        for (int u = 0; u < TPI; ++u) idv[u] = *item_row(min(u * NT + t, nf - 1), rr[u]);
#pragma unroll
        for (int u = 0; u < TPI; ++u) {
            const int f = u * NT + t;
            ky[u] = -1;
            if (f < nf) classify(f, rr[u], idv[u], ky[u], ic[u], cd[u]);
        }
#pragma unroll
        for (int u = 0; u < TPI; ++u)
            if (ky[u] >= 0) rk[u] = atomicAdd(&hist[ky[u]], 1);
    } else {
        for (int f = t; f < nf; f += NT) {
            int k, i, c;
            item(f, k, i, c);
            atomicAdd(&hist[k], 1);
        }
    }
    __syncthreads();
    if (w == 0) {
        constexpr int PL = 8 * kTileBuckets / kWave;
        int v[PL], sum = 0;
#pragma unroll
        for (int i = 0; i < PL; ++i) {
            v[i] = hist[lane * PL + i];
            sum += v[i];
        }
        int incl = sum;
#pragma unroll
        for (int o = 1; o < kWave; o <<= 1) {
            const int y = __shfl_up(incl, o, kWave);
            if (lane >= o) incl += y;
        }
        int run = incl - sum;
        int* soff = a.plan + plan_soff(a.B, R) + (int64_t)g * 9;
        if ((lane * PL) % kTileBuckets == 0) soff[lane * PL / kTileBuckets] = run;
        if (lane == kWave - 1) soff[8] = incl;
#pragma unroll
        for (int i = 0; i < PL; ++i) {
            hist[lane * PL + i] = run;
            run += v[i];
        }
    }
    __syncthreads();
    int2* list = reinterpret_cast<int2*>(a.plan + plan_list(a.B, R)) + (int64_t)g * R * (a.N + 1);
    if (in_regs) {
#pragma unroll
        for (int u = 0; u < TPI; ++u)
            if (ky[u] >= 0) list[hist[ky[u]] + rk[u]] = make_int2(ic[u], cd[u]);
    } else {
        for (int f = t; f < nf; f += NT) {
            int k, i, c;
            item(f, k, i, c);
            list[atomicAdd(&hist[k], 1)] = make_int2(i, c);
        }
    }
    auto chk = [](int64_t id, int64_t n) { return (id >= 0 && id < n) ? (int)id : -1; };
    if (t < R)
        reinterpret_cast<int4*>(a.plan + kPlanHdr)[(int64_t)g * R + t] =
            t < nr ? make_int4(brow[t], chk(ph, a.nent), chk(pr, a.nrel), chk(pt, a.nent)) : make_int4(-1, -1, -1, -1);
    if (g == 0 && t == 0) {
        int* h = a.plan;
        h[0] = kPlanMagic;
        h[1] = (int)a.B;
        h[2] = (int)a.N;
        h[3] = a.mode;
        h[4] = R;
        h[5] = (int)a.nent;
        h[6] = a.sort;
    }
}

template <int NWV>
__global__ __launch_bounds__(NWV * kWave) void tile_plan_kernel(PlanArgs a) {
    extern __shared__ __attribute__((aligned(16))) unsigned char plan_smem[];
    tile_plan_group<NWV>(a, (int)blockIdx.x, reinterpret_cast<int*>(plan_smem));
}

template <int FN, bool CH, int V, int G, int NWV, int DEPTH, bool PLANNED = false, bool BOARD = false, bool SHARED = false>
__global__ __launch_bounds__(NWV * kWave) void step_fwd_tile_kernel(ScoreParams p) {
    static_assert(DEPTH == 1 || DEPTH == 2, "candidate rows in flight per wave");
    static_assert(PLANNED || !BOARD, "the board belongs to a planned step");
    extern __shared__ __attribute__((aligned(16))) unsigned char tile_smem[];
#ifdef KGE_PROFILING_KNOBS
    const long long clk_entry = wall_clock64();
#endif
    constexpr int NQ = tile_nq(FN);
    constexpr int W = G * kWave;
    constexpr int NT = NWV * kWave;
    const int R = p.tile_rows, QS = p.tile_q2slots;
    vecf<V>* qimg = reinterpret_cast<vecf<V>*>(tile_smem);
    vecf<V>* q2img = qimg + (size_t)R * NQ * W;
    int64_t* rrow = reinterpret_cast<int64_t*>(q2img + (size_t)QS * W);
    int64_t* brow = rrow + R;
    int64_t* qid = brow + R;
    int* q2slot = reinterpret_cast<int*>(qid + R);
    int* hist = q2slot + R;
    int* cntp = hist + kTileBuckets;
    int* list = cntp + 4;
    const int t = threadIdx.x, lane = t & 63, w = t >> 6;
    if constexpr (PLANNED) {
        if (p.tile_next.plan && (int)blockIdx.x >= p.tile_blocks) {
            if constexpr (SHARED) {
                const int ng = (int)plan_groups(p.tile_next.B, p.tile_next.R);
                for (int g = (int)blockIdx.x - p.tile_blocks; g < ng; g += p.tile_plan_blocks) {
                    tile_plan_group<NWV>(p.tile_next, g, reinterpret_cast<int*>(tile_smem));
                    __syncthreads();
                }
            } else {
                tile_plan_group<NWV>(p.tile_next, (int)blockIdx.x - p.tile_blocks, reinterpret_cast<int*>(tile_smem));
            }
#ifdef KGE_PROFILING_KNOBS
            if (p.tile_clk && t == 0) {
                long long* const pc = p.tile_clk + (int64_t)p.tile_blocks * kSweepClkMarks + 2 * ((int)blockIdx.x - p.tile_blocks);
                pc[0] = clk_entry;
                pc[1] = wall_clock64();
            }
#endif
            return;
        }
    }
    const int x = (int)(blockIdx.x & 7);
    const int gi = (int)(blockIdx.x >> 3);
    const int64_t g0 = (int64_t)gi * R;
    const int nr = (int)min<int64_t>(R, p.B - g0);
    if (nr <= 0) return;
    const int64_t S = (p.c_rows + 7) / 8;
    const int64_t e_lo = min((int64_t)x * S, p.c_rows), e_hi = min(p.c_rows, e_lo + S);
    const int64_t Np = (p.tile_pos && !CH) ? p.N + 1 : p.N;
    const float bscale = (float)kTileBuckets / (float)S;
    int cnt = 0;
    [[maybe_unused]] rsrc_t prs = make_rsrc(nullptr, 0u);
    [[maybe_unused]] int pre_id = 0, pre_code = 0;
    [[maybe_unused]] const int4* pmeta = nullptr;

    if constexpr (PLANNED) {
        const int* pl = p.tile_plan;
        pmeta = reinterpret_cast<const int4*>(pl + kPlanHdr) + (int64_t)gi * R;
        const int2* plist = reinterpret_cast<const int2*>(pl + plan_list(p.B, R)) + (int64_t)gi * R * (p.N + 1);
        constexpr bool TWO = NWV < kTileRows;
        static_assert(TWO || kTileMaxRows <= 2 * NWV, "two rows per wave (8 and 12 waves: the host caps the rows)");
        const int* so = pl + plan_soff(p.B, R) + (int64_t)gi * 9;
        const bool hasA = w < nr, hasB = TWO && w + NWV < nr;
        const int rA = hasA ? w : 0, rB = hasB ? w + NWV : rA;
        const int h0 = pl[0], h1 = pl[1], h2 = pl[2], h3 = pl[3], h4 = pl[4], h5 = pl[5], h6 = pl[6];
        const int plo = so[x], phi = so[x + 1];
        const int4 mA = pmeta[rA], mB = pmeta[rB];
        const int4 ml = pmeta[min(lane, R - 1)];
        const int mode = CH ? KGE_HEAD_BATCH : KGE_TAIL_BATCH;
        if (h0 != kPlanMagic || h1 != (int)p.B || h2 != (int)p.N || h3 != mode || h4 != R || h5 != (int)p.c_rows ||
            (h6 != 0) != (p.tile_sort != 0)) {
            if (x == 0)
                for (int r = w; r < nr; r += NWV) {
                    for (int64_t n = lane; n < p.N; n += kWave) p.out[(g0 + r) * p.out_ld + n] = __builtin_nanf("");
                    if (lane == 0) {
                        if (p.out_pos_raw) p.out_pos_raw[g0 + r] = __builtin_nanf("");
                        p.out_pos_ls[g0 + r] = __builtin_nanf("");
                    }
                }
            return;
        }
        cnt = max(phi - plo, 0);
        const bool inl = lane < nr;
        const int relv = (inl && ml.z >= 0 && ml.z < p.r_rows) ? ml.z : -1;
        if (w == 0 && inl) {
            brow[lane] = ml.x;
            qid[lane] = CH ? ml.w : ml.y;
            rrow[lane] = relv;
        }
        if (p.tile_dry == 1) return;
        prs = make_rsrc(plist + plo, (uint32_t)cnt * 8u);
        {
            const int ci = p.tile_rev ? cnt - 1 - (w + NWV * lane) : w + NWV * lane;
            const auto e = __builtin_amdgcn_raw_buffer_load_b64(prs, (uint32_t)((ci >= 0 && ci < cnt) ? ci : cnt) * 8u, 0, 0);
            pre_id = (int)e[0];
            pre_code = (int)e[1];
        }
        [[maybe_unused]] vecf<V> t2a[G], t2b[G];
        [[maybe_unused]] int slA = -1, slB = -1;
        [[maybe_unused]] int slv = -1;
        if constexpr (FN == KGE_INTERHT) {
            static_assert(kTileMaxRows <= kWave, "one lane per row");
            const int prev = __shfl_up(relv, 1, kWave);
            const bool open = inl && (lane == 0 || relv != prev);
            const uint64_t m = __ballot(open);
            const int sl = __popcll(m & (lane == 63 ? ~0ull : (2ull << lane) - 1)) - 1;
            slv = (inl && sl < QS) ? sl : -1;
            if (w == 0 && inl) q2slot[lane] = slv;
            auto third = [&](int r, bool has, int& slot, vecf<V>* t2) {
                const int s = __builtin_amdgcn_readlane(slv, r);
                const int sp = __builtin_amdgcn_readlane(slv, r > 0 ? r - 1 : 0);
                const int ri = __builtin_amdgcn_readlane(relv, r);
                slot = (has && s >= 0 && !(r > 0 && sp == s)) ? s : -1;
                const rsrc_t sr = make_rsrc(p.rel + (ri >= 0 ? ri : 0) * p.r_ld + p.r_off,
                                            (slot >= 0 && ri >= 0) ? (uint32_t)p.D * 4u : 0u);
#pragma unroll
                for (int k = 0; k < G; ++k) t2[k] = bload<V>(sr, goff<V>(lane, k));
            };
            third(rA, hasA, slA, t2a);
            if constexpr (TWO) third(rB, hasB, slB, t2b);
        }
        auto build_m = [&](const int4& m, bool has, Query<FN, CH, V, G>& q) {
            const int64_t qi = CH ? m.w : m.y, ri = m.z;
            const bool qok = has && qi >= 0 && qi < p.q_rows, rok = has && ri >= 0 && ri < p.r_rows;
            q.build(p.qent + (qok ? qi : 0) * p.q_ld, qok, p.rel + (rok ? ri : 0) * p.r_ld + p.r_off, rok, p.D, lane, p);
        };
        auto put_q = [&](int r, const Query<FN, CH, V, G>& q) {
            vecf<V>* qr = qimg + (size_t)r * NQ * W;
#pragma unroll
            for (int k = 0; k < G; ++k) {
                qr[lane + k * kWave] = q.q0[k];
                if constexpr (NQ > 1) qr[W + lane + k * kWave] = q.q1[k];
            }
        };
        {
            Query<FN, CH, V, G> qa, qb;
            build_m(mA, hasA, qa);
            if constexpr (TWO) build_m(mB, hasB, qb);
            if (hasA) put_q(rA, qa);
            if constexpr (TWO) {
                if (hasB) put_q(rB, qb);
            }
        }
        if constexpr (FN == KGE_INTERHT) {
            if (slA >= 0) {
#pragma unroll
                for (int k = 0; k < G; ++k) q2img[(size_t)slA * W + lane + k * kWave] = t2a[k];
            }
            if constexpr (TWO) {
                if (slB >= 0) {
#pragma unroll
                    for (int k = 0; k < G; ++k) q2img[(size_t)slB * W + lane + k * kWave] = t2b[k];
                }
            }
        }
        if constexpr (!TWO) {
            if (w + NWV < nr) {
                const int rC = w + NWV;
                Query<FN, CH, V, G> qc;
                build_m(pmeta[rC], true, qc);
                put_q(rC, qc);
                if constexpr (FN == KGE_INTERHT) {
                    const int s = __builtin_amdgcn_readlane(slv, rC), sp = __builtin_amdgcn_readlane(slv, rC - 1);
                    const int ri = __builtin_amdgcn_readlane(relv, rC);
                    if (s >= 0 && sp != s) {
                        const rsrc_t sr = make_rsrc(p.rel + (ri >= 0 ? ri : 0) * p.r_ld + p.r_off, ri >= 0 ? (uint32_t)p.D * 4u : 0u);
#pragma unroll
                        for (int k = 0; k < G; ++k) q2img[(size_t)s * W + lane + k * kWave] = bload<V>(sr, goff<V>(lane, k));
                    }
                }
            }
        }
        __syncthreads();
    } else {
        if (p.tile_sort) {
            constexpr int MU = (kTileSortMaxB + NT - 1) / NT, NB = kTileSortRel;
            int* wc = list;
            int bk[MU], wr[MU];
            int64_t rv[MU], qv[MU];
#pragma unroll
            for (int u = 0; u < MU; ++u) {
                const int i = u * NT + t;
                bk[u] = NB;
                rv[u] = qv[u] = 0;
                if (i < p.B) {
                    const int64_t rr = p.r_idx ? p.r_idx[i * p.r_stride] : i;
                    rv[u] = rr;
                    qv[u] = p.q_idx ? p.q_idx[i * p.q_stride] : i;
                    bk[u] = (rr >= 0 && rr < p.r_rows) ? (int)min<int64_t>(rr, NB - 2) : NB - 1;
                }
            }
            for (int i = t; i < MU * NWV * NB; i += NT) wc[i] = 0;
            __syncthreads();
#pragma unroll
            for (int u = 0; u < MU; ++u) {
                wr[u] = 0;
                if (u * NT >= p.B) continue;
                uint64_t todo = __ballot(bk[u] < NB);
                while (todo) {
                    const int v = __builtin_amdgcn_readlane(bk[u], __builtin_ctzll(todo));
                    const uint64_t m = __ballot(bk[u] == v);
                    if (bk[u] == v) wr[u] = lanes_below(m);
                    if (lane == 0) wc[(u * NWV + w) * NB + v] = __popcll(m);
                    todo &= ~m;
                }
            }
            __syncthreads();
            if (w == 0) {
                int y[MU * NWV];
#pragma unroll
                for (int c = 0; c < MU * NWV; ++c) y[c] = wc[c * NB + lane];
                int run = 0;
#pragma unroll
                for (int c = 0; c < MU * NWV; ++c) {
                    const int v = y[c];
                    y[c] = run;
                    run += v;
                }
                int incl = run;
#pragma unroll
                for (int o = 1; o < kWave; o <<= 1) {
                    const int v = __shfl_up(incl, o, kWave);
                    if (lane >= o) incl += v;
                }
// ... 21 lines not shown
        __syncthreads();
        if (p.tile_dry == 1) return;

        const int64_t nf = (int64_t)nr * Np;
        const int Np32 = (int)Np;
        const float inv_np = 1.f / (float)Np32;
        auto item = [&](int64_t f64, int& bucket, int& code) -> bool {
            const int f = (int)f64;
            int r = (int)((float)f * inv_np);
            if (r * Np32 > f) --r;
            if ((r + 1) * Np32 <= f) ++r;
            const int n = f - r * Np32;
            const int64_t b = brow[r];
            const int64_t id = n < p.N ? p.c_idx[b * p.c_stride + n] : p.pos_base[b * 3 + 2];
            const int64_t row = id - p.c_base;
            const bool valid = row >= 0 && row < p.c_rows;
            if (valid ? (row < e_lo || row >= e_hi) : x != 0) return false;
            bucket = valid ? min(kTileBuckets - 1, (int)((float)(int)(row - e_lo) * bscale)) : 0;
            code = (r << 16) | n;
            return true;
        };
        constexpr int TPI = NWV >= 16 ? 17 : 16;
        int wbk[TPI], wcd[TPI];
        const bool in_regs = nf <= (int64_t)TPI * NT;
        if (in_regs) {
#pragma unroll
            for (int u = 0; u < TPI; ++u) {
                const int64_t f = (int64_t)u * NT + t;
                wbk[u] = -1;
                if (f < nf && !item(f, wbk[u], wcd[u])) wbk[u] = -1;
            }
        }

        auto build_row = [&](int r, Query<FN, CH, V, G>& q, int64_t& ri, bool& rok) {
            const int64_t qi = qid[r];
            ri = rrow[r];
            bool qok = qi >= 0 && qi < p.q_rows;
            rok = ri >= 0 && ri < p.r_rows;
            q.build(p.qent + (qok ? qi : 0) * p.q_ld, qok, p.rel + (rok ? ri : 0) * p.r_ld + p.r_off, rok, p.D, lane, p);
        };
        auto put = [&](int r, const Query<FN, CH, V, G>& q, int64_t ri, bool rok) {
            vecf<V>* qr = qimg + (size_t)r * NQ * W;
#pragma unroll
            for (int k = 0; k < G; ++k) {
                qr[lane + k * kWave] = q.q0[k];
                if constexpr (NQ > 1) qr[W + lane + k * kWave] = q.q1[k];
            }
            if (lane == 0) rrow[r] = rok ? ri : -1;
        };
        if constexpr (2 * NWV <= kTileRows) {
            for (int r = w; r < nr; r += 2 * NWV) {
                const int r2 = r + NWV < nr ? r + NWV : r;
                Query<FN, CH, V, G> qa, qb;
                int64_t ri, ri2;
                bool rok, rok2;
                build_row(r, qa, ri, rok);
                build_row(r2, qb, ri2, rok2);
                put(r, qa, ri, rok);
                if (r2 != r) put(r2, qb, ri2, rok2);
            }
        } else {
            for (int r = w; r < nr; r += NWV) {
                Query<FN, CH, V, G> q;
                int64_t ri;
                bool rok;
                build_row(r, q, ri, rok);
                put(r, q, ri, rok);
            }
        }
        for (int i = t; i < kTileBuckets; i += NT) hist[i] = 0;
        __syncthreads();
        if (p.tile_dry == 2) return;
        if constexpr (FN == KGE_INTERHT) {
            static_assert(kTileMaxRows <= kWave, "one lane per row");
            if (w == 0) {
                const bool in = lane < nr;
                const int64_t cur = in ? rrow[lane] : 0;
                const bool open = in && (lane == 0 || cur != rrow[lane - 1]);
                const uint64_t m = __ballot(open);
                if (in) {
                    const int sl = __popcll(m & (lane == 63 ? ~0ull : (2ull << lane) - 1)) - 1;
                    q2slot[lane] = sl < QS ? sl : -1;
                }
            }
        }
        int wrk[TPI];
        if (in_regs) {
#pragma unroll
            for (int u = 0; u < TPI; ++u)
                if (wbk[u] >= 0) wrk[u] = atomicAdd(&hist[wbk[u]], 1);
        } else {
            for (int64_t f = t; f < nf; f += NT) {
                int bk, code;
                if (item(f, bk, code)) atomicAdd(&hist[bk], 1);
            }
        }
        __syncthreads();
        if (p.tile_dry == 3) return;
        if constexpr (FN == KGE_INTERHT) {
            for (int r = w; r < nr; r += NWV) {
                const int sl = q2slot[r];
                if (sl < 0 || (r > 0 && q2slot[r - 1] == sl)) continue;
                const int64_t ri = rrow[r];
                const rsrc_t sr = make_rsrc(p.rel + (ri >= 0 ? ri : 0) * p.r_ld + p.r_off, ri >= 0 ? (uint32_t)p.D * 4u : 0u);
#pragma unroll
                for (int k = 0; k < G; ++k) q2img[(size_t)sl * W + lane + k * kWave] = bload<V>(sr, goff<V>(lane, k));
            }
        }
        if (w == 0) {
            constexpr int PL = kTileBuckets / kWave;
            int v[PL], s = 0;
#pragma unroll
            for (int i = 0; i < PL; ++i) {
                v[i] = hist[lane * PL + i];
                s += v[i];
            }
            int incl = s;
#pragma unroll
            for (int o = 1; o < kWave; o <<= 1) {
                const int y = __shfl_up(incl, o, kWave);
                if (lane >= o) incl += y;
            }
            int run = incl - s;
#pragma unroll
            for (int i = 0; i < PL; ++i) {
                hist[lane * PL + i] = run;
                run += v[i];
            }
            if (lane == kWave - 1) cntp[0] = incl;
        }
        __syncthreads();
        if (in_regs) {
#pragma unroll
            for (int u = 0; u < TPI; ++u)
                if (wbk[u] >= 0) list[hist[wbk[u]] + wrk[u]] = wcd[u];
        } else {
            for (int64_t f = t; f < nf; f += NT) {
                int bk, code;
                if (item(f, bk, code)) list[atomicAdd(&hist[bk], 1)] = code;
            }
        }
        __syncthreads();
        cnt = cntp[0];
    }

    if (p.tile_dry) return;
    struct Item {
        Cand<FN, V, G> c;
        vecf<V> q2[FN == KGE_INTERHT ? G : 1];
    };
    constexpr bool has_board = BOARD;
    const rsrc_t brs = make_rsrc(has_board ? p.tile_board + x * kSweepBoardLine : nullptr, has_board ? kSweepBoardLine * 4u : 0u);
    const uint32_t boff_ld = (uint32_t)(lane & (kSweepBoardLine - 1)) * 4u;
    const uint32_t boff_st = t == 0 ? (uint32_t)gi * 4u : kSweepBoardLine * 4u;
    const int btag = p.tile_tag << kSweepTagShift;
    const bool bpeer = has_board && lane < (p.tile_blocks >> 3) && lane != gi;
    int bv = 0;
#ifdef KGE_PROFILING_KNOBS
    long long* const bclk = (PLANNED && p.tile_clk) ? p.tile_clk + ((int64_t)x * (p.tile_blocks >> 3) + gi) * kSweepClkMarks : nullptr;
    long long* const clk = w == 0 ? bclk : nullptr;
    int cmark = 0;
    if (clk && lane == 0) {
        clk[0] = wall_clock64();
        clk[5] = __builtin_amdgcn_s_getreg((3 << 11) | 20) & 15;
        clk[6] = clk_entry;
    }
#endif
    for (int c0 = w; c0 < cnt; c0 += NT) {
        const int nc = min(kWave, (cnt - c0 + NWV - 1) / NWV);
        int code = 0;
        int64_t my_id = 0;
        if (lane < nc) {
            const int ci = p.tile_rev ? cnt - 1 - (c0 + NWV * lane) : c0 + NWV * lane;
            if constexpr (PLANNED) {
                if (c0 == w) {
                    code = pre_code;
                    my_id = pre_id;
                } else {
                    const auto e = __builtin_amdgcn_raw_buffer_load_b64(prs, (uint32_t)ci * 8u, 0, 0);
                    code = (int)e[1];
                    my_id = (int)e[0];
                }
            } else {
                code = list[ci];
                const int r = code >> 16, n = code & 0xFFFF;
                const int64_t b = brow[r];
                my_id = n < p.N ? p.c_idx[b * p.c_stride + n] : p.pos_base[b * 3 + 2];
            }
        }
        auto load = [&](Item& it, int j) {
            bool ok;
            it.c.load(cand_row(p, readlane64(my_id, j), ok), ok, p.D, lane);
            if constexpr (FN == KGE_INTERHT) {
                const int r = __builtin_amdgcn_readlane(code, j) >> 16;
                const int sl = q2slot[r];
                if (sl >= 0) {
#pragma unroll
                    for (int k = 0; k < G; ++k) it.q2[k] = q2img[(size_t)sl * W + lane + k * kWave];
                } else {
                    const int64_t ri = rrow[r];
                    const rsrc_t sr = make_rsrc(p.rel + (ri >= 0 ? ri : 0) * p.r_ld + p.r_off,
                                                ri >= 0 ? (uint32_t)p.D * 4u : 0u);
#pragma unroll
                    for (int k = 0; k < G; ++k) it.q2[k] = bload<V>(sr, goff<V>(lane, k));
                }
            }
        };
        auto score = [&](const Item& it, int j) -> float {
            const int cj = __builtin_amdgcn_readlane(code, j);
            const int r = cj >> 16, n = cj & 0xFFFF;
            const vecf<V>* qr = qimg + (size_t)r * NQ * W;
            (void)n;
            if constexpr (FN == KGE_INTERHT) {
                TileQueryIH<V, G> q{{qr, lane}, {qr + W, lane}, {}};
#pragma unroll
                for (int k = 0; k < G; ++k) q.q2[k] = it.q2[k];
                return cand_score<FN, CH, V, G>(it.c, q, p);
            } else {
                const LdsQuery<V> q{{qr, lane}, {qr + (NQ > 1 ? W : 0), lane}, {qr, lane}};
                return cand_score<FN, CH, V, G>(it.c, q, p);
            }
        };
        const int my_bk = my_id >= e_lo ? max(0, min(kTileBuckets - 1, (int)((float)(int)(my_id - e_lo) * bscale))) : 0;
        const int my_prog = p.tile_rev ? kTileBuckets - 1 - my_bk : my_bk;
        auto fetch = [&](Item& it, int j) {
            const int own = __builtin_amdgcn_readlane(my_prog, j);
            if constexpr (has_board) {
                const bool led = bpeer && (bv & ~kSweepDone) == btag && (bv & kSweepDone) + p.tile_lead < own;
                if (__ballot(led)) __builtin_amdgcn_s_sleep(kSweepNap);
                vecf<1> pub;
                pub.a[0] = __int_as_float(btag | own);
                bstore<1>(brs, boff_st, pub);
                bv = (int)__builtin_amdgcn_raw_buffer_load_b32(brs, boff_ld, 0, kAuxSC1);
            }
#ifdef KGE_PROFILING_KNOBS
            if (clk) {
                while (cmark < 3 && own >= 64 * (cmark + 1)) {
                    ++cmark;
                    if (lane == 0) clk[cmark] = wall_clock64();
                }
            }
#endif
            load(it, j);
        };
        float my_score = 0.f;
        if constexpr (DEPTH == 2) {
            Item x0, x1;
            fetch(x0, 0);
            for (int j = 0; j < nc; j += 2) {
                if (j + 1 < nc) fetch(x1, j + 1);
                float s = score(x0, j);
                if (lane == j) my_score = s;
                if (j + 1 < nc) {
                    if (j + 2 < nc) fetch(x0, j + 2);
                    s = score(x1, j + 1);
                    if (lane == j + 1) my_score = s;
                }
            }
        } else {
            Item x0;
            for (int j = 0; j < nc; ++j) {
                fetch(x0, j);
                const float s = score(x0, j);
                if (lane == j) my_score = s;
            }
        }
        if (lane < nc) {
            const int r = code >> 16, n = code & 0xFFFF;
            const int64_t b = brow[r];
            if (n < p.N) {
                p.out[b * p.out_ld + n] = my_score;
            } else {
                if (p.out_pos_raw) p.out_pos_raw[b] = my_score;
                p.out_pos_ls[b] = log_sigmoid(my_score);
            }
        }
    }
    if constexpr (has_board) {
        vecf<1> pub;
        pub.a[0] = __int_as_float(btag | kSweepDone);
        bstore<1>(brs, boff_st, pub);
    }
#ifdef KGE_PROFILING_KNOBS
    if (clk && lane == 0) clk[4] = wall_clock64();
    if (bclk && lane == 0) bclk[kSweepClkWave + 2 * w] = wall_clock64();
#endif
    if constexpr (CH) {
        if (!p.tile_pos) return;
        for (int r = w; r < nr; r += NWV) {
            const int64_t b = brow[r];
            const int4 pm = PLANNED ? pmeta[r] : make_int4(0, 0, 0, 0);
            const int64_t tt = PLANNED ? pm.w : p.pos_base[b * 3 + 2], row = tt - p.c_base;
            const bool valid = row >= 0 && row < p.c_rows;
            if (valid ? (row < e_lo || row >= e_hi) : x != 0) continue;
            Query<FN, false, V, G> qp;
            const int64_t hi = PLANNED ? pm.y : p.pos_base[b * 3], rj = PLANNED ? pm.z : p.pos_base[b * 3 + 1];
            const bool hok = hi >= 0 && hi < p.q_rows, rjok = rj >= 0 && rj < p.r_rows;
            qp.build(p.qent + (hok ? hi : 0) * p.q_ld, hok, p.rel + (rjok ? rj : 0) * p.r_ld + p.r_off, rjok, p.D,
                     lane, p);
            bool ok;
            Cand<FN, V, G> c;
            c.load(cand_row(p, tt, ok), ok, p.D, lane);
            const float s = cand_score<FN, false, V, G>(c, qp, p);
            if (lane == 0) {
                if (p.out_pos_raw) p.out_pos_raw[b] = s;
                p.out_pos_ls[b] = log_sigmoid(s);
            }
        }
    }
#ifdef KGE_PROFILING_KNOBS
    if (bclk && lane == 0) bclk[kSweepClkWave + 2 * w + 1] = wall_clock64();
#endif
// ... 2403 lines not shown
```

### customknowledgegraphembedding_amd/csrc/kge_internal.h

```cpp
#pragma once

#include <hip/hip_runtime.h>
#include <stdint.h>

#include "kge_hip.h"

namespace kge_impl {

constexpr int kWave = 64;
constexpr int kBlock = 256;
constexpr int kWavesPerBlock = kBlock / kWave;
constexpr int kMaxG = 8;
constexpr int kBwdMaxG = 16;

enum Kind {
    KIND_FWD = 0,
    KIND_BWD = 1,
    KIND_FINISH = 2,
    KIND_BWD_ROWS = 3,
    KIND_BWD_ENT = 4,
    KIND_BWD_STREAM = 5,
    KIND_BWD_CHAIN = 6,
    KIND_FWD_STATS = 7,
    KIND_STEP_FWD = 8,
    KIND_STEP_FWD_STATS = 9,
    KIND_BWD_ENT_STREAM = 10,
    KIND_STEP_FWD_GRAD = 11,
    KIND_STEP_EPILOGUE = 12,
    KIND_SHARD_FWD_GRAD = 13,
    KIND_SHARD_POS = 14,
    KIND_SHARD_EPILOGUE = 15,
    KIND_STEP_FWD_XCD = 16,
    KIND_SCORE_SHARD_XCD = 17,
    KIND_SHARD_BUCKET = 18,
    KIND_STEP_FWD_TILE = 19,
    KIND_SCORE_TILE = 20,
    KIND_RANK_PAIRS = 21,
    KIND_RANK_SWEEP = 22,
    KIND_TOPK_SWEEP = 23,
    KIND_RANK_CAND = 24,
    KIND_COUNT
};
constexpr int kFwdGradMaxG = 4;
constexpr int kSweepMaxG = 4;
constexpr int kSweepWaves = 16;
constexpr int kSweepMaxRows = 16;
constexpr int kSweepLdsMax = 144 * 1024;
constexpr int kSweepMinBlocks = 256;
constexpr int kTopkMax = KGE_TOPK_MAX;
constexpr int kTopkEmpty = 0x7fffffff;
static_assert(kTopkMax <= kWave, "one list entry per lane");
inline int64_t sweep_chunks(int64_t groups, int64_t S) {
    const int64_t want = (kSweepMinBlocks + groups * 8 - 1) / (groups * 8);
    const int64_t most = S / (2 * kSweepWaves) > 1 ? S / (2 * kSweepWaves) : 1;
    const int64_t c = want < most ? want : most;
    return c > 1 ? c : 1;
}
constexpr int64_t topk_ws_lists(int64_t B) { return 8 * ((int64_t)kSweepMinBlocks / 8 * kSweepMaxRows + B); }

enum GridRule {
    GRID_WAVE_PER_ROW,
    GRID_BLOCK_PER_ROW,
    GRID_WAVE_PER_ENT,
    GRID_BLOCK_PER_ENT,
    GRID_XCD_SLICES,
    GRID_TILE_GROUPS,
    GRID_CAND_PER_WAVE,
    GRID_STEP_EPILOGUE,
    GRID_SHARD_EPILOGUE,
    GRID_RANK_PAIRS,
    GRID_RANK_SWEEP,
    GRID_TOPK_SWEEP,
    GRID_RANK_CAND,
};
constexpr int rank_cand_wpr(int64_t C) { return C <= kWave ? 1 : (C <= 2 * kWave ? 2 : kWavesPerBlock); }

struct KindInfo {
    GridRule grid;
    bool ch;
    int max_g;
    bool g_whole_waves;
    bool no_protate;
    bool interht_only;
    const char* what;
    bool distance_only = false;
    bool no_pairre = false;
};
constexpr KindInfo kKinds[KIND_COUNT] = {
                 {GRID_CAND_PER_WAVE, true, kMaxG, false, false, false, "kge score launch"},
                 {GRID_CAND_PER_WAVE, true, kBwdMaxG, false, false, false, "kge score backward launch"},
              {GRID_WAVE_PER_ROW, false, kMaxG, false, false, false, "kge finish launch"},
            {GRID_BLOCK_PER_ROW, true, kMaxG, false, false, false, "kge score launch"},
             {GRID_WAVE_PER_ENT, true, kMaxG, false, false, false, "kge score launch"},
          {GRID_BLOCK_PER_ROW, true, kMaxG, true, false, false, "kge score launch", false, true},
           {GRID_WAVE_PER_ROW, true, kMaxG, false, false, false, "kge score launch"},
           {GRID_CAND_PER_WAVE, true, kMaxG, false, false, true, "kge score launch"},
            {GRID_BLOCK_PER_ROW, true, kMaxG, false, false, false, "kge score launch"},
      {GRID_BLOCK_PER_ROW, true, kMaxG, false, false, true, "kge score launch"},
      {GRID_BLOCK_PER_ENT, true, kMaxG, true, false, false, "kge score launch"},
       {GRID_BLOCK_PER_ROW, true, kFwdGradMaxG, false, true, false, "kge score launch"},
       {GRID_STEP_EPILOGUE, true, kFwdGradMaxG, false, true, false, "kge score launch"},
      {GRID_BLOCK_PER_ROW, true, kFwdGradMaxG, false, true, false, "kge score launch", false, true},
           {GRID_WAVE_PER_ROW, false, kFwdGradMaxG, false, true, false, "kge score launch", false, true},
      {GRID_SHARD_EPILOGUE, true, kFwdGradMaxG, false, true, false, "kge score launch", false, true},
        {GRID_XCD_SLICES, true, kMaxG, false, false, false, "kge score launch"},
     {GRID_XCD_SLICES, true, kMaxG, false, false, false, "kge score launch"},
        {GRID_XCD_SLICES, true, kMaxG, false, false, false, "kge score launch", false, true},
       {GRID_TILE_GROUPS, true, kFwdGradMaxG, false, false, false, "kge score launch"},
          {GRID_TILE_GROUPS, true, kFwdGradMaxG, false, false, false, "kge score launch"},
          {GRID_RANK_PAIRS, true, kSweepMaxG, false, false, false, "kge_eval_rank_sweep", true},
          {GRID_RANK_SWEEP, true, kSweepMaxG, false, false, false, "kge_eval_rank_sweep", true},
          {GRID_TOPK_SWEEP, true, kSweepMaxG, false, false, false, "kge_eval_topk_sweep", true},
           {GRID_RANK_CAND, true, kMaxG, false, false, false, "kge_eval_rank_candidates"},
};
constexpr bool kind_has(int k, int fn, bool ch, int G) {
    return G <= kKinds[k].max_g && (!kKinds[k].g_whole_waves || G % kWavesPerBlock == 0) &&
           (!kKinds[k].distance_only || (fn != KGE_DISTMULT && fn != KGE_COMPLEX)) &&
           (!kKinds[k].no_protate || fn != KGE_PROTATE) && (!kKinds[k].interht_only || fn == KGE_INTERHT) &&
           (!kKinds[k].no_pairre || fn != KGE_PAIRRE) && (kKinds[k].ch || !ch);
}
constexpr int kTileBuckets = 256;
constexpr int kTileRows = 16;
constexpr int kTileMaxRows = 20;
constexpr int kTileLdsMax = 160 * 1024;
constexpr int kTileSortRel = 64;
constexpr int kTileSortMaxB = 2048;
constexpr int tile_nq(int fn) {
    return (fn == KGE_COMPLEX || fn == KGE_ROTATE || fn == KGE_INTERHT || fn == KGE_PAIRRE) ? 2 : 1;
}
constexpr int shard_nq(int fn) {
    return fn == KGE_INTERHT ? 3 : ((fn == KGE_COMPLEX || fn == KGE_ROTATE || fn == KGE_PAIRRE) ? 2 : 1);
}

constexpr int kSweepBoardLine = 32;
constexpr int kSweepBoardInts = 8 * kSweepBoardLine;
constexpr int kSweepTagShift = 9;
constexpr int kSweepDone = (1 << kSweepTagShift) - 1;
constexpr int kSweepTagMask = (1 << (31 - kSweepTagShift)) - 1;
constexpr int kSweepNap = 8;
constexpr int kSweepClkWave = 8;
constexpr int kSweepClkMarks = kSweepClkWave + 2 * 16;
constexpr int64_t kge_sweep_clk_words(int64_t groups) { return groups * 8 * kSweepClkMarks + groups * 2; }

constexpr int kPlanMagic = 0x4B475031;
constexpr int kPlanHdr = 16;
__host__ __device__ inline int64_t plan_groups(int64_t B, int R) { return (B + R - 1) / R; }
__host__ __device__ inline int64_t plan_soff(int64_t B, int R) { return kPlanHdr + plan_groups(B, R) * R * 4; }
__host__ __device__ inline int64_t plan_list(int64_t B, int R) { return (plan_soff(B, R) + plan_groups(B, R) * 9 + 3) & ~(int64_t)3; }
__host__ __device__ inline int64_t plan_words(int64_t B, int64_t N, int R) {
    return plan_list(B, R) + plan_groups(B, R) * R * (N + 1) * 2;
}
struct PlanArgs {
    const int64_t* pos;
    const int64_t* neg;
    int64_t neg_ld;
    int64_t B, N, nent, nrel;
    int mode;
    int R;
    int sort;
    int* plan;
};
__host__ __device__ constexpr int plan_lds_ints(int NT) {
    return kTileMaxRows + 8 * kTileBuckets + (kTileSortMaxB + NT - 1) / NT * (NT / 64) * kTileSortRel;
}

struct ScoreParams {
    const float* qent;
    const int64_t* q_idx;
    int64_t q_ld, q_stride, q_rows;
    const float* rel;
    const int64_t* r_idx;
    int64_t r_ld, r_stride, r_rows, r_off;
    const float* cent;
    const int64_t* c_idx;
    int64_t c_ld, c_stride, c_rows, c_dense;
    int64_t c_base;
    int skip_foreign;
    const int* cmp_pre;
    const int* cmp_cnt;
    const int* cmp_tot;
    int64_t cmp_home0;
    const int2* bk_ent;
    const int* bk_start;
    int64_t bk_ld;
    int xcd_phases;
    int tile_rows;
    int tile_lds;
    int tile_pos;
    int tile_q2slots;
    int tile_sort;
    int tile_waves;
    int tile_depth;
    int* tile_board;
    int tile_tag;
    int tile_lead;
    long long* tile_clk;
    int tile_dry;
    int tile_rev;
    const int* tile_plan;
    int* tile_occ;
    int tile_blocks;
    PlanArgs tile_next;
    int tile_plan_blocks;
    struct {
        const int64_t* truth;
        const int64_t* fptr;
        const int64_t* fids;
        int64_t nf;
        float* ts;
        int* cnt;
        float* fs;
        int chunks;
    } rk;
    struct {
        const int64_t* xptr;
        const int64_t* xids;
        int k;
        int chunks;
        int2* parts;
    } tk;
    float* out;
    int64_t out_ld;
    int64_t B, N;
    int D;
    int cpw;
    int wpr;
    float gamma;
    float phase_div;
    float modulus;
    const float* d_scores;
    int64_t d_ld;
    float* d_qent;
    float* d_rel;
    float* d_cent;
    float* d_modulus;
    const float* neg_scores;
    int64_t ns_ld, n_neg;
    float temperature;
    int adversarial;
    int detach;
    const float* dq_scale;
    const float* weight;
    const float* pos_raw;
    float* loss;
    float* loss_sum;
    int* ev_count;
    int* ev_cursor;
    int* ev_code_w;
    const int* ev_tile_sum;
    int* ev_off_fix;
    int ev_ntiles;
    float* out_neg;
    float* out_pos_raw;
    float* out_pos_ls;
    float* qbuf;
    float* qg_ent;
    float* qg_rel;
    float* dmod_part;
    int64_t slot0;
    float2* cand_stats;
    const int64_t* pos_base;
    float* dqbuf;
    int64_t ent_w, rel_w;
    const int* ev_off;
    const int* ev_code;
    const float* d_ns;
    const float* d_ps;
    int64_t Bn, Nn;
    float* d_out_ent;
    const float* qent_pos;
    float* sh_stats;
    const float* sh_stats_all;
    float* sh_dq;
    float* sh_A;
    float* sh_B;
    float* sh_merged;
    int64_t home_B;
    int world, rank, nq;
    struct {
        float* m;
        float* v;
        float b1, b2, eps, alpha, step_size, bc2_sqrt;
        int keras, on;
    } adam;
    float* loss_parts;
    float reg3;
    float* reg_part;
    const int* lz_list;
    const int* lz_count;
    int64_t lz_rows;
    struct {
        int64_t* ranks;
        int64_t* ties;
    } rc;
};
constexpr int kTileSharedWaves = 12;
inline bool tile_plan_shared(const ScoreParams& p) {
    return p.tile_next.plan && p.tile_plan_blocks < plan_groups(p.tile_next.B, p.tile_next.R);
}

struct AdamArgs {
    float b1, b2, eps, alpha, step_size, bc2_sqrt;
    int keras, zero_grad;
};

int launch_transe(const ScoreParams& p, int kind, hipStream_t st, int blocks, bool ch, int V, int G);
int launch_distmult(const ScoreParams& p, int kind, hipStream_t st, int blocks, bool ch, int V, int G);
int launch_complex(const ScoreParams& p, int kind, hipStream_t st, int blocks, bool ch, int V, int G);
int launch_rotate(const ScoreParams& p, int kind, hipStream_t st, int blocks, bool ch, int V, int G);
int launch_interht(const ScoreParams& p, int kind, hipStream_t st, int blocks, bool ch, int V, int G);
int launch_protate(const ScoreParams& p, int kind, hipStream_t st, int blocks, bool ch, int V, int G);
int launch_pairre(const ScoreParams& p, int kind, hipStream_t st, int blocks, bool ch, int V, int G);

int launch_eval_query_any(int fn, bool ch, const ScoreParams& p, hipStream_t st, int blocks, int V, int G, float* Q,
                          int64_t ldq, void* P = nullptr, int64_t prows = 0);
int launch_gemm_nt(const float* A, const float* B, float* C, int M, int N, int K, int64_t lda, int64_t ldb,
                   int64_t ldc, hipStream_t st);
int launch_gemm_nt_f32x3(const float* A, const float* B, float* C, int M, int N, int K, int64_t lda, int64_t ldb,
                         int64_t ldc, hipStream_t st, int form = 0);
int launch_split3_planes(const float* X, int64_t rows, int64_t cols, int64_t ld, void* planes, int64_t plane_rows,
                         hipStream_t st);
int launch_gemm_nt_x3p(const void* Ap, int64_t a_rows, const void* Bp, int64_t b_rows, int64_t K, float* C, int64_t ldc,
                       int M, int N, hipStream_t st, int form);
int64_t eval_rank_ws_bytes(int64_t M, int64_t F);
int launch_eval_rank_planes(const void* Ap, int64_t a_rows, const void* Bp, int64_t b_rows, int64_t K, int M, int N,
                            const int64_t* truth, const int64_t* fptr, const int64_t* fids, int64_t F, int64_t* ranks,
                            void* ws, hipStream_t st, int form, int phases);
int launch_rank_finish(int64_t M, int64_t N, const int64_t* truth, const int64_t* fptr, const int64_t* fids, void* ws,
                       int64_t* ranks, hipStream_t st);
int64_t eval_topk_planes_parts(int64_t N);
int launch_eval_topk_planes(const void* Ap, int64_t a_rows, const void* Bp, int64_t b_rows, int64_t K, int M, int N,
                            const int64_t* xptr, const int64_t* xids, int k, int64_t* out_ids, int64_t ids_ld,
                            float* out_scores, int64_t scores_ld, void* ws, hipStream_t st);
int launch_topk_merge(const void* parts, int64_t B, int64_t nparts, int k, int64_t* out_ids, int64_t ids_ld,
                      float* out_scores, int64_t scores_ld, hipStream_t st);
int launch_topk_rows(const float* S, int64_t M, int64_t N, int64_t ld, const int64_t* xptr, const int64_t* xids, int k,
                     int64_t* out_ids, int64_t ids_ld, float* out_scores, int64_t scores_ld, hipStream_t st);
int launch_rank(const float* S, int64_t M, int64_t N, int64_t ld, const int64_t* truth, const int64_t* fptr,
                const int64_t* fids, int64_t* ranks, hipStream_t st);

}
```

### customknowledgegraphembedding_amd/ops.py

```python
from __future__ import annotations

import torch

from . import _lib
from ._lib import FN_IDS, HEAD_BATCH, SINGLE, TAIL_BATCH, check


def ctypes_ptr(t):
    return None if t is None else t.data_ptr()


def _stream(device) -> int:
    return torch.cuda.current_stream(device).cuda_stream


def _need_gpu(*ts):
    for t in ts:
        if t is not None and t.device.type != "cuda":
            raise _lib.KGEHipError(
                f"libkge_hip.so runs on ROCm devices only; got a tensor on {t.device} "
                "(there is no CPU fallback)")


def _fp32(t, name):
# ... 30 lines not shown
    if mode == 0:
        return HEAD_BATCH
    if mode == 3:
        return SINGLE
    return TAIL_BATCH


def _forms_ptr(forms):
    import ctypes
    if forms is None:
        return None, None
    if isinstance(forms, dict):
        forms = _lib.forms(**forms)
    return ctypes.addressof(forms), forms


def score_indexed_raw(fn, mode, ent, rel, rel_off, pos, neg, D, gamma, emb_range, modulus=0.0,
                      out=None, forms=None):
    _need_gpu(ent, rel, pos, neg)
    _fp32(ent, "entity_embedding")
    _fp32(rel, "relation_embedding")
    _i64(pos, "positive_sample")
    if pos.dim() != 2 or pos.shape[1] != 3 or not pos.is_contiguous():
        raise ValueError("positive_sample must be a contiguous [B, 3] int64 tensor")
    B = pos.shape[0]
    if mode == SINGLE:
        N, neg_ld, neg_p = 1, 0, None
    else:
        _i64(neg, "negative_sample")
        if neg.dim() != 2 or neg.shape[0] != B or neg.stride(1) != 1:
            raise ValueError("negative_sample must be a row-contiguous [B, N] int64 tensor")
        N, neg_ld, neg_p = neg.shape[1], neg.stride(0), neg.data_ptr()
    if out is None:
        out = torch.empty((B, N), dtype=torch.float32, device=ent.device)
    fp, _keep = _forms_ptr(forms)
    rc = _lib.load().kge_score_indexed_ex(
        fn, mode, ent.data_ptr(), ent.shape[0], ent.stride(0), rel.data_ptr(), rel.shape[0],
        rel.stride(0), rel_off, pos.data_ptr(), neg_p, neg_ld, B, N, D, float(gamma),
        float(emb_range), float(modulus), out.data_ptr(), out.stride(0), fp, _stream(ent.device))
    check(rc, "kge_score_indexed")
    return out


def score_indexed_bwd_raw(fn, mode, ent, rel, rel_off, pos, neg, D, gamma, emb_range, modulus,
                          d_scores, d_ent, d_rel, d_modulus=None):
    B = pos.shape[0]
    if mode == SINGLE:
        N, neg_ld, neg_p = 1, 0, None
    else:
        N, neg_ld, neg_p = neg.shape[1], neg.stride(0), neg.data_ptr()
    d_scores = d_scores.contiguous()
    rc = _lib.load().kge_score_indexed_bwd(
        fn, mode, ent.data_ptr(), ent.shape[0], ent.stride(0), rel.data_ptr(), rel.shape[0],
        rel.stride(0), rel_off, pos.data_ptr(), neg_p, neg_ld, B, N, D, float(gamma),
        float(emb_range), float(modulus), d_scores.data_ptr(), d_scores.stride(0),
        d_ent.data_ptr(), d_rel.data_ptr(), ctypes_ptr(d_modulus), None, _stream(ent.device))
    check(rc, "kge_score_indexed_bwd")


def step_forward_raw(fn, mode, ent, rel, rel_off, pos, neg, D, gamma, emb_range, modulus=0.0,
                     temperature=1.0, adversarial=True, neg_scores=None, cand_stats=None, forms=None):
    _need_gpu(ent, rel, pos, neg)
    _fp32(ent, "entity_embedding")
    _fp32(rel, "relation_embedding")
    _i64(pos, "positive_sample")
    _i64(neg, "negative_sample")
    if mode not in (HEAD_BATCH, TAIL_BATCH):
        raise ValueError("step_forward needs a negative mode (0 head-batch or 1 tail-batch)")
    if pos.dim() != 2 or pos.shape[1] != 3 or not pos.is_contiguous():
        raise ValueError("positive_sample must be a contiguous [B, 3] int64 tensor")
    B, N = neg.shape
    if neg.stride(1) != 1 or B != pos.shape[0]:
        raise ValueError("negative_sample must be a row-contiguous [B, N] int64 tensor")
    dev = ent.device
    if neg_scores is None:
        neg_scores = torch.empty((B, N), dtype=torch.float32, device=dev)
    out_neg = torch.empty((B,), dtype=torch.float32, device=dev)
    out_pos = torch.empty((B,), dtype=torch.float32, device=dev)
    pos_scores = torch.empty((B,), dtype=torch.float32, device=dev)
    fp, _keep = _forms_ptr(forms)
    rc = _lib.load().kge_step_forward_ex(
        fn, mode, ent.data_ptr(), ent.shape[0], ent.stride(0), rel.data_ptr(), rel.shape[0],
        rel.stride(0), rel_off, pos.data_ptr(), neg.data_ptr(), neg.stride(0), B, N, D,
        float(gamma), float(emb_range), float(modulus), float(temperature), int(bool(adversarial)),
        neg_scores.data_ptr(), neg_scores.stride(0), out_neg.data_ptr(), pos_scores.data_ptr(),
        out_pos.data_ptr(), None if cand_stats is None else cand_stats.data_ptr(), fp, _stream(dev))
    check(rc, "kge_step_forward")
    return out_neg, out_pos, neg_scores, pos_scores


class StepPlanner:

    def __init__(self, fn, ent, rel, rel_off, D, B, N, gamma, emb_range, modulus=0.0, temperature=1.0,
                 adversarial=True):
        import ctypes
        _need_gpu(ent, rel)
        _fp32(ent, "entity_embedding")
        _fp32(rel, "relation_embedding")
        self.fn, self.ent, self.rel, self.rel_off, self.D = fn, ent, rel, rel_off, D
        self.B, self.N = B, N
        lib = _lib.load()
        nbytes = int(lib.kge_step_planner_plan_size(fn, ent.shape[0], ent.stride(0), rel.shape[0], rel.stride(0),
                                                    rel_off, B, N, D))
        if nbytes <= 0:
            raise _lib.KGEHipError("kge_step_plan_size is 0: the tile form does not apply to this shape "
                                   "(use step_forward_raw)")
        self._bufs = [torch.empty(nbytes, dtype=torch.uint8, device=ent.device) for _ in range(2)]
        h = ctypes.c_void_p()
        check(lib.kge_step_planner_create(
            ctypes.addressof(h), fn, ent.data_ptr(), ent.shape[0], ent.stride(0), rel.data_ptr(), rel.shape[0],
            rel.stride(0), rel_off, B, N, D, float(gamma), float(emb_range), float(modulus), float(temperature),
            int(bool(adversarial)), self._bufs[0].data_ptr(), self._bufs[1].data_ptr(), nbytes,
            _stream(ent.device)), "kge_step_planner_create")
        self._h = h.value
        self._lib = lib
        self.board = torch.empty(int(lib.kge_step_board_size()), dtype=torch.uint8, device=ent.device)
        check(lib.kge_step_planner_set_board(self._h, self.board.data_ptr(), self.board.numel()),
              "kge_step_planner_set_board")
        self._step_fn = lib.kge_step_planner_step
        self._planned = False
        self._held = None
        self._pshape, self._nshape = (B, 3), (B, N)
        self._out_ok = None

    @staticmethod
    def plan_size(fn, ent, rel, rel_off, D, B, N):
        return int(_lib.load().kge_step_plan_size(fn, ent.shape[0], ent.stride(0), rel.shape[0], rel.stride(0),
                                                  rel_off, B, N, D))

    @classmethod
    def available(cls, fn, ent, rel, rel_off, D, B, N):
        return cls.plan_size(fn, ent, rel, rel_off, D, B, N) > 0

    def _check_batch(self, pos, neg, mode):
        if mode not in (HEAD_BATCH, TAIL_BATCH):
            raise ValueError("a planned step needs a negative mode (0 head-batch or 1 tail-batch)")
        if pos.shape != self._pshape or neg.shape != self._nshape:
            raise ValueError(f"a planned batch must be pos [{self.B}, 3] and neg [{self.B}, {self.N}]")
        if pos.dtype != torch.int64 or neg.dtype != torch.int64 or pos.device != self.ent.device or \
                neg.device != self.ent.device:
            raise TypeError("a planned batch must be int64 tensors on the tables' device")
        if pos.stride() != (3, 1) or neg.stride(1) != 1:
            raise ValueError("pos must be contiguous and neg row-contiguous")

    def set_sweep(self, alternate):
        check(self._lib.kge_step_planner_set_sweep(self._h, int(alternate)), "kge_step_planner_set_sweep")

    def set_form(self, waves=0, depth=0):
        check(self._lib.kge_step_planner_set_form(self._h, int(waves), int(depth)), "kge_step_planner_set_form")

    def set_rows(self, rows):
        check(self._lib.kge_step_planner_set_rows(self._h, int(rows)), "kge_step_planner_set_rows")

    def set_lead(self, lead):
        check(self._lib.kge_step_planner_set_lead(self._h, int(lead)), "kge_step_planner_set_lead")

    def form(self):
        return {k: int(self._lib.kge_step_planner_get(self._h, i))
                for k, i in (("waves", 0), ("depth", 1), ("lead", 2), ("throttle", 3), ("tag", 4), ("rows", 6),
                             ("plan_blocks", 7))}

    def set_modulus(self, modulus):
        check(self._lib.kge_step_planner_set_modulus(self._h, float(modulus)), "kge_step_planner_set_modulus")

    def plan(self, pos, neg, mode):
        self._check_batch(pos, neg, mode)
        check(self._lib.kge_step_planner_plan(self._h, pos.data_ptr(), neg.data_ptr(), neg.stride(0), mode),
              "kge_step_planner_plan")
        self._planned, self._held = True, (pos, neg)

    def outputs(self):
        dev = self.ent.device
        return (torch.empty((self.B,), dtype=torch.float32, device=dev),
                torch.empty((self.B,), dtype=torch.float32, device=dev),
                torch.empty((self.B, self.N), dtype=torch.float32, device=dev),
                torch.empty((self.B,), dtype=torch.float32, device=dev))

    def _check_outputs(self, out):
        if not isinstance(out, (tuple, list)) or len(out) != 4:
            raise ValueError("StepPlanner.step: out must be (out_neg, out_pos, neg_scores, pos_scores)")
        shapes = ((self.B,), (self.B,), (self.B, self.N), (self.B,))
        strides = ((1,), (1,), (self.N, 1), (1,))
        for t, shp, std, nm in zip(out, shapes, strides, ("out_neg", "out_pos", "neg_scores", "pos_scores")):
            if not isinstance(t, torch.Tensor) or t.dtype != torch.float32 or t.device != self.ent.device:
                raise TypeError(f"StepPlanner.step: {nm} must be a float32 tensor on {self.ent.device}")
            if tuple(t.shape) != shp or (t.numel() > 1 and tuple(t.stride()) != std):
                raise ValueError(f"StepPlanner.step: {nm} must have shape {shp} and strides {std}")

    def step(self, nxt=None, out=None):
        if not self._planned:
            raise RuntimeError("StepPlanner.step: no batch planned (call plan() first, or pass nxt to step)")
        if out is not None and out is not self._out_ok:
            self._check_outputs(out)
            self._out_ok = out
        out_neg, out_pos, neg_scores, pos_scores = out if out is not None else self.outputs()
        if nxt is None:
            rc = self._step_fn(self._h, None, None, 0, 0, neg_scores.data_ptr(), out_neg.data_ptr(),
                               pos_scores.data_ptr(), out_pos.data_ptr())
        else:
            npos, nneg, nmode = nxt
            self._check_batch(npos, nneg, nmode)
            rc = self._step_fn(self._h, npos.data_ptr(), nneg.data_ptr(), nneg.stride(0), nmode,
                               neg_scores.data_ptr(), out_neg.data_ptr(), pos_scores.data_ptr(), out_pos.data_ptr())
        check(rc, "kge_step_planner_step")
        if nxt is None:
            self._planned, self._held = False, None
        else:
            self._held = (nxt[0], nxt[1])
        return out_neg, out_pos, neg_scores, pos_scores

    def __del__(self):
        h = getattr(self, "_h", None)
        if h:
            try:
                self._lib.kge_step_planner_destroy(h)
            except Exception:
                pass
            self._h = None


def step_finish_raw(fn, ent, rel, rel_off, pos, D, gamma, emb_range, neg_scores, modulus=0.0,
                    temperature=1.0, adversarial=True):
    B, N = neg_scores.shape
    dev = ent.device
    out_neg = torch.empty((B,), dtype=torch.float32, device=dev)
    out_pos = torch.empty((B,), dtype=torch.float32, device=dev)
    pos_scores = torch.empty((B,), dtype=torch.float32, device=dev)
    rc = _lib.load().kge_step_finish(
        fn, ent.data_ptr(), ent.shape[0], ent.stride(0), rel.data_ptr(), rel.shape[0], rel.stride(0),
        rel_off, pos.data_ptr(), B, D, float(gamma), float(emb_range), float(modulus),
        neg_scores.data_ptr(), N, neg_scores.stride(0), float(temperature), int(bool(adversarial)),
        out_neg.data_ptr(), pos_scores.data_ptr(), out_pos.data_ptr(), _stream(dev))
    check(rc, "kge_step_finish")
    return out_neg, out_pos, pos_scores


def _dense_shapes(mode, head, relation, tail):
    B = head.shape[0]
    if mode == HEAD_BATCH:
        N = head.shape[1]
    elif mode == TAIL_BATCH:
        N = tail.shape[1]
    else:
        N = 1
    return B, N


def _rows(t):
    if t.dim() == 2:
        t = t.unsqueeze(1)
    if t.stride(-1) != 1 or (t.shape[1] > 1 and t.stride(0) != t.shape[1] * t.stride(1)):
        t = t.contiguous()
    ld = t.stride(1) if t.shape[1] > 1 else t.stride(0)
    return t, ld


def score_dense_raw(fn, mode, head, relation, tail, rel_off, D, gamma, emb_range, modulus=0.0):
    _need_gpu(head, relation, tail)
    for t, n in ((head, "head"), (relation, "relation"), (tail, "tail")):
        _fp32(t, n)
    B, N = _dense_shapes(mode, head, relation, tail)
    head, hld = _rows(head)
    tail, tld = _rows(tail)
    relation, rld = _rows(relation)
    out = torch.empty((B, N), dtype=torch.float32, device=head.device)
    rc = _lib.load().kge_score_dense(
        fn, mode, head.data_ptr(), hld, relation.data_ptr(), rld, rel_off, tail.data_ptr(), tld,
        B, N, D, float(gamma), float(emb_range), float(modulus), out.data_ptr(), out.stride(0),
        _stream(head.device))
    check(rc, "kge_score_dense")
    return out


def neg_reduce_raw(scores, temperature=1.0, adversarial=True):
    _need_gpu(scores)
    _fp32(scores, "scores")
    B, N = scores.shape
    out = torch.empty((B,), dtype=torch.float32, device=scores.device)
    rc = _lib.load().kge_neg_reduce(scores.data_ptr(), B, N, scores.stride(0), float(temperature),
                                    int(bool(adversarial)), out.data_ptr(), _stream(scores.device))
    check(rc, "kge_neg_reduce")
    return out


def log_sigmoid_raw(x):
    _need_gpu(x)
    x = x.contiguous()
    out = torch.empty_like(x)
    rc = _lib.load().kge_log_sigmoid(x.data_ptr(), x.numel(), out.data_ptr(), _stream(x.device))
    check(rc, "kge_log_sigmoid")
    return out



def transparse_premul(W, mask):
    M = torch.empty_like(W)
    check(_lib.load().kge_transparse_premul(W.data_ptr(), mask.data_ptr(), W.numel(), M.data_ptr(),
                                            _stream(W.device)), "kge_transparse_premul")
    return M


def _want_premul(W, pos, neg, mode):
    if W.numel() % 4 or W.data_ptr() % 16:
        return False
    rows = pos.shape[0] * (neg.shape[1] if (mode_id(mode) == HEAD_BATCH and neg is not None) else 1)
    return W.shape[0] * 4 <= max(1, rows // 128)


_WS_CACHE = {}


def _workspace(device, nbytes):
    if nbytes <= 0:
# ... 321 lines not shown
```

### include/kge_hip.h

```cpp
#ifndef KGE_HIP_H
#define KGE_HIP_H

#include <stdint.h>

#ifdef __cplusplus
extern "C" {
#endif

#define KGE_ABI_VERSION 1

enum kge_fn {
    KGE_TRANSE = 0,
    KGE_DISTMULT = 1,
    KGE_COMPLEX = 2,
    KGE_ROTATE = 3,
    KGE_INTERHT = 4,
    KGE_PROTATE = 5,
    KGE_PAIRRE = 7
};

enum kge_mode {
    KGE_HEAD_BATCH = 0,
    KGE_TAIL_BATCH = 1,
    KGE_SINGLE = 3
};

#define KGE_EINVAL (-22)
#define KGE_ENOTSUP (-95)
#define KGE_EHIP (-1000)

int kge_abi_version(void);

const char* kge_last_error(void);

const char* kge_build_id(void);
const char* kge_source_hash(void);

int64_t kge_max_dim(int fn);

typedef struct kge_forms {
    int step_order;
    int xcd_phases;
    int tile_rows;
    int tile_q2slots;
    int tile_waves;
    int gemm_form;
    int transparse_form;
} kge_forms;

int kge_step_forward_order(int64_t nentity, int64_t N);

int kge_score_indexed(int fn, int mode,
                      const float* ent, int64_t nentity, int64_t ent_ld,
                      const float* rel, int64_t nrelation, int64_t rel_ld, int64_t rel_off,
                      const int64_t* pos, const int64_t* neg, int64_t neg_ld,
                      int64_t B, int64_t N, int64_t D,
                      float gamma, float emb_range, float modulus,
                      float* scores, int64_t scores_ld, void* stream);
int kge_score_indexed_ex(int fn, int mode,
                         const float* ent, int64_t nentity, int64_t ent_ld,
                         const float* rel, int64_t nrelation, int64_t rel_ld, int64_t rel_off,
                         const int64_t* pos, const int64_t* neg, int64_t neg_ld,
                         int64_t B, int64_t N, int64_t D,
                         float gamma, float emb_range, float modulus,
                         float* scores, int64_t scores_ld, const kge_forms* forms, void* stream);

int kge_step_forward(int fn, int mode,
                     const float* ent, int64_t nentity, int64_t ent_ld,
                     const float* rel, int64_t nrelation, int64_t rel_ld, int64_t rel_off,
                     const int64_t* pos, const int64_t* neg, int64_t neg_ld,
                     int64_t B, int64_t N, int64_t D,
                     float gamma, float emb_range, float modulus,
                     float temperature, int adversarial,
                     float* neg_scores, int64_t ns_ld, float* out_neg,
                     float* pos_scores, float* out_pos, float* cand_stats, void* stream);
int kge_step_forward_ex(int fn, int mode,
                        const float* ent, int64_t nentity, int64_t ent_ld,
                        const float* rel, int64_t nrelation, int64_t rel_ld, int64_t rel_off,
                        const int64_t* pos, const int64_t* neg, int64_t neg_ld,
                        int64_t B, int64_t N, int64_t D,
                        float gamma, float emb_range, float modulus,
                        float temperature, int adversarial,
                        float* neg_scores, int64_t ns_ld, float* out_neg,
                        float* pos_scores, float* out_pos, float* cand_stats, const kge_forms* forms, void* stream);

int64_t kge_step_plan_size(int fn, int64_t nentity, int64_t ent_ld, int64_t nrelation, int64_t rel_ld,
                           int64_t rel_off, int64_t B, int64_t N, int64_t D);
int kge_step_plan(int fn, int mode, int64_t nentity, int64_t ent_ld, int64_t nrelation, int64_t rel_ld,
                  int64_t rel_off, const int64_t* pos, const int64_t* neg, int64_t neg_ld, int64_t B, int64_t N,
                  int64_t D, void* plan, void* stream);
int kge_step_forward_planned(int fn, int mode,
                             const float* ent, int64_t nentity, int64_t ent_ld,
                             const float* rel, int64_t nrelation, int64_t rel_ld, int64_t rel_off,
                             int64_t B, int64_t N, int64_t D,
                             float gamma, float emb_range, float modulus,
                             float temperature, int adversarial,
                             const void* plan,
                             const int64_t* next_pos, const int64_t* next_neg, int64_t next_neg_ld, int next_mode,
                             void* next_plan,
                             float* neg_scores, int64_t ns_ld, float* out_neg,
                             float* pos_scores, float* out_pos, void* stream);

typedef struct kge_step_planner kge_step_planner;
int kge_step_planner_create(kge_step_planner** out, int fn, const float* ent, int64_t nentity, int64_t ent_ld,
                            const float* rel, int64_t nrelation, int64_t rel_ld, int64_t rel_off, int64_t B, int64_t N,
                            int64_t D, float gamma, float emb_range, float modulus, float temperature, int adversarial,
                            void* plan0, void* plan1, int64_t plan_bytes, void* stream);
int kge_step_planner_set_modulus(kge_step_planner* planner, float modulus);
int kge_step_planner_set_sweep(kge_step_planner* planner, int alternate);
int kge_step_planner_set_form(kge_step_planner* planner, int waves, int depth);
int64_t kge_step_board_size(void);
int kge_step_planner_set_board(kge_step_planner* planner, void* board, int64_t board_bytes);
int kge_step_planner_set_lead(kge_step_planner* planner, int lead);
#define KGE_PLANNER_WAVES 0
#define KGE_PLANNER_DEPTH 1
#define KGE_PLANNER_LEAD 2
#define KGE_PLANNER_THROTTLE 3
#define KGE_PLANNER_TAG 4
#define KGE_PLANNER_ROWS 6
#define KGE_PLANNER_PLAN_BLOCKS 7
int kge_step_planner_get(const kge_step_planner* planner, int what);
int64_t kge_step_planner_plan_size(int fn, int64_t nentity, int64_t ent_ld, int64_t nrelation, int64_t rel_ld,
                                   int64_t rel_off, int64_t B, int64_t N, int64_t D);
#define KGE_PLANNER_ROWS_RULE (-1)
int kge_step_planner_set_rows(kge_step_planner* planner, int rows);
int kge_step_planned_rows(int fn, int64_t nentity, int64_t ent_ld, int64_t nrelation, int64_t rel_ld, int64_t rel_off,
                          int64_t B, int64_t N, int64_t D, int waves, int64_t capacity, int* out);
int kge_step_planner_set_clocks(kge_step_planner* planner, void* clocks, int64_t clocks_bytes);
int kge_step_planner_plan(kge_step_planner* planner, const int64_t* pos, const int64_t* neg, int64_t neg_ld, int mode);
int kge_step_planner_step(kge_step_planner* planner, const int64_t* next_pos, const int64_t* next_neg,
                          int64_t next_neg_ld, int next_mode, float* neg_scores, float* out_neg, float* pos_scores,
                          float* out_pos);
int kge_step_planner_destroy(kge_step_planner* planner);

int kge_step_finish(int fn,
                    const float* ent, int64_t nentity, int64_t ent_ld,
                    const float* rel, int64_t nrelation, int64_t rel_ld, int64_t rel_off,
                    const int64_t* pos, int64_t B, int64_t D,
                    float gamma, float emb_range, float modulus,
                    const float* neg_scores, int64_t N, int64_t ns_ld,
                    float temperature, int adversarial,
                    float* out_neg, float* pos_scores, float* out_pos, void* stream);

int kge_score_sharded(int fn, int mode,
                      const float* qent, int64_t q_ld,
                      const float* rel, int64_t nrelation, int64_t rel_ld, int64_t rel_off,
                      const float* shard, int64_t shard_rows, int64_t shard_ld, int64_t shard_lo,
                      const int64_t* pos, const int64_t* neg, int64_t neg_ld,
                      int64_t B, int64_t N, int64_t D,
                      float gamma, float emb_range, float modulus,
                      float* scores, int64_t scores_ld, void* stream);

int kge_gather_rows(const float* table, int64_t rows, int64_t ld, int64_t lo,
                    const int64_t* ids, int64_t id_stride, int64_t n, int64_t width,
                    float* out, int64_t out_ld, void* stream);

#define KGE_SHARD_TWO_COLUMNS 1
int kge_shard_plan(const int64_t* pos, const int64_t* neg, int64_t neg_ld, int64_t Bg, int64_t N,
                   int64_t nentity, int world, int chunks, int mode, int flags, int rank,
                   int* cnt, int* hpre, int* qown, int* qslot, int* summary,
                   int* bucket, int* bucket_start, void* stream);
int kge_shard_gather_queries(const float* shard, int64_t shard_rows, int64_t ld, int64_t shard_lo,
                             const int64_t* pos, int64_t Bg, int chunks, int chunk, int64_t width,
                             int world, int rank, int mode, int flags, const int* qown, const int* qslot,
                             const int* summary, float* send, int64_t* qidx, void* stream);
int kge_shard_score(int fn, int mode,
                    const float* qent, int64_t q_rows, int64_t q_ld, const int64_t* q_idx,
                    const float* rel, int64_t nrelation, int64_t rel_ld, int64_t rel_off,
                    const float* shard, int64_t shard_rows, int64_t shard_ld, int64_t shard_lo,
                    const int64_t* pos, int64_t B, int64_t N, int64_t D,
                    float gamma, float emb_range, float modulus,
                    const int* bucket, const int* bucket_start,
                    const int* pre, const int* cnt, const int* tot,
                    int world, int rank, int64_t home_B, int64_t home0,
                    float* send, void* stream);
int kge_shard_finish(const float* recv, const int* tot, const int* hpre,
                     const int64_t* pos, const int64_t* neg, int64_t neg_ld,
                     int64_t Bg, int64_t N, int64_t nentity, int world, int home, int mode,
                     float temperature, int adversarial,
                     float* scores, int64_t ns_ld, float* out_neg, float* pos_scores, float* out_pos,
                     void* stream);

typedef struct kge_comm kge_comm;
typedef struct kge_shard_exec kge_shard_exec;
typedef struct kge_loop_group kge_loop_group;
#define KGE_EXEC_PROBE 1
#define KGE_EXEC_ONE_STREAM 2
#define KGE_EXEC_TIMING 4
kge_loop_group* kge_comm_loopback_group(int world);
int kge_comm_loopback_group_destroy(kge_loop_group* group);
int kge_comm_loopback_init(kge_comm** out, kge_loop_group* group, int rank);
int kge_comm_unique_id(void* id);
int kge_comm_init(kge_comm** out, const void* id, int world, int rank);
int kge_comm_destroy(kge_comm* comm);
int kge_comm_all_to_allv(kge_comm* comm, const float* send, const int64_t* send_counts, float* recv,
                         const int64_t* recv_counts, void* stream);
int kge_comm_all_reduce_sum(kge_comm* comm, float* buf, int64_t n, void* stream);
int64_t kge_shard_exec_workspace_size(int64_t Bg, int64_t N, int64_t ent_dim, int world, int chunks);
int64_t kge_shard_exec_host_ints(int world, int chunks);
int kge_shard_exec_create(kge_shard_exec** out, kge_comm* comm, int flags, int fn, int64_t nentity,
                          int64_t shard_rows, int64_t ent_dim, int64_t D, int64_t Bg, int64_t N, int world,
                          int rank, int chunks, void* workspace, int64_t workspace_bytes, int* host_pinned,
                          int64_t host_ints);
int kge_shard_exec_destroy(kge_shard_exec* exec);
double kge_shard_exec_host_wait_us(kge_shard_exec* exec, int reset);
int kge_shard_exec_timings(kge_shard_exec* exec, float* out, int n);
int kge_comm_size(kge_comm* comm);
int kge_shard_exec_plan(kge_shard_exec* exec, const int64_t* pos, const int64_t* neg, int64_t neg_ld, int mode,
                        void* stream);
int kge_shard_exec_step(kge_shard_exec* exec, const float* shard, int64_t shard_ld, int64_t shard_lo,
                        const float* rel, int64_t nrelation, int64_t rel_ld, int64_t rel_off, const int64_t* pos,
                        const int64_t* neg, int64_t neg_ld, int mode, float gamma, float emb_range, float modulus,
                        float temperature, int adversarial, const int64_t* next_pos, const int64_t* next_neg,
                        int next_mode, float* scores, int64_t ns_ld, float* out_neg, float* pos_scores,
                        float* out_pos, void* stream);

int kge_eval_query(int fn, int mode,
                   const float* ent, int64_t nentity, int64_t ent_ld,
                   const float* rel, int64_t nrelation, int64_t rel_ld,
                   const int64_t* pos, int64_t B, int64_t D,
                   float* Q, int64_t ldq, void* stream);
int kge_gemm_nt(const float* A, int64_t lda, const float* B, int64_t ldb, float* C, int64_t ldc,
                int64_t M, int64_t N, int64_t K, void* stream);
int kge_gemm_nt_bf16x3(const float* A, int64_t lda, const float* B, int64_t ldb, float* C, int64_t ldc,
                       int64_t M, int64_t N, int64_t K, void* stream);
int kge_gemm_nt_bf16x3_ex(const float* A, int64_t lda, const float* B, int64_t ldb, float* C, int64_t ldc,
                          int64_t M, int64_t N, int64_t K, const kge_forms* forms, void* stream);
int kge_eval_query_planes(int fn, int mode, const float* ent, int64_t nentity, int64_t ent_ld, const float* rel,
                          int64_t nrelation, int64_t rel_ld, const int64_t* pos, int64_t B, int64_t D, void* planes,
                          int64_t plane_rows, void* stream);
int64_t kge_split_bf16x3_bytes(int64_t rows, int64_t cols);
int kge_split_bf16x3(const float* X, int64_t rows, int64_t cols, int64_t ld, void* planes, int64_t plane_rows,
                     void* stream);
int kge_gemm_nt_bf16x3_planes(const void* A_planes, int64_t a_rows, const void* B_planes, int64_t b_rows, int64_t K,
                              float* C, int64_t ldc, int64_t M, int64_t N, void* stream);
int kge_gemm_nt_bf16x3_planes_ex(const void* A_planes, int64_t a_rows, const void* B_planes, int64_t b_rows, int64_t K,
                                 float* C, int64_t ldc, int64_t M, int64_t N, const kge_forms* forms, void* stream);
int kge_rank_filtered(const float* scores, int64_t M, int64_t N, int64_t ld, const int64_t* truth,
                      const int64_t* filter_ptr, const int64_t* filter_ids, int64_t* ranks,
                      void* stream);
int64_t kge_eval_rank_planes_workspace_size(int64_t M, int64_t nfilter);
int kge_eval_rank_planes(const void* A_planes, int64_t a_rows, const void* B_planes, int64_t b_rows, int64_t K,
                         int64_t M, int64_t N, const int64_t* truth, const int64_t* filter_ptr,
                         const int64_t* filter_ids, int64_t nfilter, int64_t* ranks, void* workspace,
                         size_t workspace_bytes, void* stream);
int kge_eval_rank_planes_ex(const void* A_planes, int64_t a_rows, const void* B_planes, int64_t b_rows, int64_t K,
                            int64_t M, int64_t N, const int64_t* truth, const int64_t* filter_ptr,
                            const int64_t* filter_ids, int64_t nfilter, int64_t* ranks, void* workspace,
                            size_t workspace_bytes, const kge_forms* forms, void* stream);
#define KGE_RANK_PAIRS 1
#define KGE_RANK_COUNT 2
#define KGE_RANK_FINISH 4
#define KGE_RANK_ALL 7
int kge_eval_rank_planes_phases(const void* A_planes, int64_t a_rows, const void* B_planes, int64_t b_rows, int64_t K,
                                int64_t M, int64_t N, const int64_t* truth, const int64_t* filter_ptr,
                                const int64_t* filter_ids, int64_t nfilter, int64_t* ranks, void* workspace,
                                size_t workspace_bytes, int phases, const kge_forms* forms, void* stream);

int64_t kge_eval_rank_sweep_workspace_size(int64_t B, int64_t nfilter);
int kge_eval_rank_sweep(int fn, int mode, const float* ent, int64_t nentity, int64_t ent_ld, const float* rel,
                        int64_t nrelation, int64_t rel_ld, int64_t rel_off, const int64_t* pos, int64_t B, int64_t D,
                        float gamma, float emb_range, float modulus, const int64_t* truth, const int64_t* filter_ptr,
                        const int64_t* filter_ids, int64_t nfilter, int64_t* ranks, void* workspace,
                        size_t workspace_bytes, void* stream);

int kge_eval_rank_candidates(int fn, int mode, const float* ent, int64_t nentity, int64_t ent_ld, const float* rel,
                             int64_t nrelation, int64_t rel_ld, int64_t rel_off, const int64_t* pos, int64_t M,
                             int64_t D, float gamma, float emb_range, float modulus, const int64_t* truth,
                             const int64_t* cand, int64_t cand_ld, int64_t C, const int64_t* filter_ptr,
                             const int64_t* filter_ids, int64_t nfilter, int64_t* ranks, int64_t* ties,
                             float* truth_scores, void* stream);

#define KGE_TOPK_MAX 64
int64_t kge_eval_topk_sweep_workspace_size(int64_t B, int64_t k);
int kge_eval_topk_sweep(int fn, int mode, const float* ent, int64_t nentity, int64_t ent_ld, const float* rel,
                        int64_t nrelation, int64_t rel_ld, int64_t rel_off, const int64_t* pos, int64_t B, int64_t D,
                        float gamma, float emb_range, float modulus, const int64_t* excl_ptr, const int64_t* excl_ids,
                        int64_t nexcl, int64_t k, int64_t* out_ids, int64_t ids_ld, float* out_scores,
// ... 222 lines not shown
```

Baseline: 1.626 billion triples/s.

## Balance tile groups evenly and score late rows in plan blocks

Adds an even split of batch rows across tile groups, so groups differ by at most one row instead of leaving a short last group. It also holds back a few 'late' rows that the 8 plan-building blocks score after finishing the next batch's plan. The planner turns this on by default for InterHT with large rows when the row rule and 8 plan blocks apply. The goal is to even out per-block work and use idle plan blocks, at the cost of more complex plan indexing, a larger plan buffer and extra header checks.

```diff
diff --git a/customknowledgegraphembedding_amd/_lib.py b/customknowledgegraphembedding_amd/_lib.py
--- a/customknowledgegraphembedding_amd/_lib.py
+++ b/customknowledgegraphembedding_amd/_lib.py
@@ -87,6 +87,7 @@
     "kge_step_planner_get": (_c_i, [_c_p, _c_i]),
     "kge_step_planner_plan_size": (_c_i64, [_c_i, _c_i64, _c_i64, _c_i64, _c_i64, _c_i64, _c_i64, _c_i64, _c_i64]),
     "kge_step_planner_set_rows": (_c_i, [_c_p, _c_i]),
+    "kge_step_planner_set_split": (_c_i, [_c_p, _c_i, _c_i]),
     "kge_step_planned_rows": (_c_i, [_c_i, _c_i64, _c_i64, _c_i64, _c_i64, _c_i64, _c_i64, _c_i64, _c_i64, _c_i,
                                      _c_i64, _c_p]),
     "kge_step_planner_set_clocks": (_c_i, [_c_p, _c_p, _c_i64]),
diff --git a/customknowledgegraphembedding_amd/csrc/kge_abi.hip b/customknowledgegraphembedding_amd/csrc/kge_abi.hip
--- a/customknowledgegraphembedding_amd/csrc/kge_abi.hip
+++ b/customknowledgegraphembedding_amd/csrc/kge_abi.hip
@@ -555,9 +555,10 @@
             break;
         case GRID_TILE_GROUPS: {
             if (p.tile_rows < 1 || p.tile_lds > kTileLdsMax) return fail(KGE_EINVAL, "tile plan missing");
-            const int64_t groups = (p.B + p.tile_rows - 1) / p.tile_rows;
+            const int64_t groups = p.tile_groups > 0 ? p.tile_groups : (p.B + p.tile_rows - 1) / p.tile_rows;
             p.tile_blocks = (int)(groups * 8);
-            waves = (groups * 8 + (p.tile_next.plan ? p.tile_plan_blocks : 0)) * kWavesPerBlock;
+            const int64_t tail = p.tile_late > 0 ? 8 : (p.tile_next.plan ? p.tile_plan_blocks : 0);
+            waves = (groups * 8 + tail) * kWavesPerBlock;
             break;
         }
         case GRID_CAND_PER_WAVE:
@@ -784,8 +785,14 @@
     if (row_bytes >= 4096 && fn == KGE_ROTATE) depth = 1;
 }
 
-PlanArgs plan_args(const ScoreParams& tp, const Tables& t, const Batch& b, void* plan) {
+struct Split {
+    int G, L;
+};
+
+PlanArgs plan_args(const ScoreParams& tp, const Tables& t, const Batch& b, void* plan, Split s = {0, 0}) {
     PlanArgs a;
+    a.G = s.G;
+    a.L = s.L;
     a.pos = b.pos;
     a.neg = b.neg;
     a.neg_ld = b.neg_ld;
@@ -942,7 +949,7 @@
     return step_plan_bytes({fn, nullptr, nentity, ent_ld, nullptr, nrelation, rel_ld, rel_off, D, 0.f, 0.f, 0.f}, B, N);
 }
 
-static int step_plan(const Tables& t, const Batch& b, void* plan, void* stream, int rows = 0) {
+static int step_plan(const Tables& t, const Batch& b, void* plan, void* stream, int rows = 0, Split split = {0, 0}) {
     if (!valid_fn(t.fn)) return fail(KGE_EINVAL, "unknown score function id " + std::to_string(t.fn));
     if (b.mode != KGE_HEAD_BATCH && b.mode != KGE_TAIL_BATCH)
         return fail(KGE_EINVAL, "kge_step_plan needs a negative mode (0 or 1)");
@@ -953,8 +960,8 @@
     if (!planned_tile_params(t, b.B, b.N, tp))
         return fail(KGE_ENOTSUP, "the tile form does not apply to this shape (kge_step_plan_size is 0)");
     if (rows) tp.tile_rows = rows;
-    const PlanArgs a = plan_args(tp, t, b, plan);
-    const unsigned groups = (unsigned)plan_groups(b.B, tp.tile_rows);
+    const PlanArgs a = plan_args(tp, t, b, plan, split);
+    const unsigned groups = (unsigned)split_groups(b.B, tp.tile_rows, split.G, split.L);
     if (tp.tile_waves == 16)
         hipLaunchKernelGGL(tile_plan_kernel<16>, dim3(groups), dim3(16 * kWave), plan_lds_ints(16 * kWave) * 4,
                            (hipStream_t)stream, a);
@@ -979,7 +986,8 @@
 
 static int step_forward_planned(const Tables& t, const Batch& b, float temperature, int adversarial, const void* plan,
                                 const Batch& next, void* next_plan, const StepOut& o, const SweepForm* sf,
-                                void* stream, int rows = 0, int* occ = nullptr, int plan_blocks = 0) {
+                                void* stream, int rows = 0, int* occ = nullptr, int plan_blocks = 0,
+                                Split split = {0, 0}) {
     int rc = check_fn_mode(t.fn, b.mode);
     if (rc) return rc;
     if (b.mode == KGE_SINGLE) return fail(KGE_EINVAL, "kge_step_forward_planned needs a negative mode (0 or 1)");
@@ -1022,12 +1030,18 @@
         p.tile_lead = sf->lead;
         p.tile_clk = sf->clk;
     }
+    p.tile_groups = split.G;
+    p.tile_late = split.L;
+    const int ng = (int)split_groups(next.B, tp.tile_rows, split.G, split.L);
     if (next_plan) {
-        p.tile_next = plan_args(tp, t, next, next_plan);
-        const int ng = (int)plan_groups(next.B, tp.tile_rows);
+        p.tile_next = plan_args(tp, t, next, next_plan, split);
         p.tile_plan_blocks = (plan_blocks > 0 && p.tile_waves == kTileSharedWaves) ? std::min(plan_blocks, ng) : ng;
         p.tile_lds = std::max(p.tile_lds, plan_lds_ints(p.tile_waves * kWave) * 4);
     }
+    if (split.G > 0 && p.tile_waves != kTileSharedWaves)
+        return fail(KGE_ENOTSUP, "an even split needs a 12-wave step (kge_step_planner_set_split)");
+    if (split.L > 0 && std::min(plan_blocks, ng) != 8)
+        return fail(KGE_ENOTSUP, "late rows need a step with 8 plan blocks (kge_step_planner_set_split)");
     p.tile_occ = occ;
     rc = run_score(t.fn, b.mode, p, KIND_STEP_FWD_TILE, stream);
     if (rc || occ) return rc;
@@ -1068,6 +1082,10 @@
     int rows = 0;
     int rule = 0;
     int plan_blocks = 0;
+    int rule_plan_blocks = 0;
+    int even_ask = -1, late_ask = -1;
+    Split split = {0, 0};
+    int split_set = 0;
     int64_t plan_bytes = 0;
     int64_t steps = 0;
     void* stream = nullptr;
@@ -1103,6 +1121,40 @@
     return (int64_t)sp->cus * per_cu;
 }
 
+int planner_late_rows(int fn, int64_t D) {
+#ifdef KGE_PROFILING_KNOBS
+    if (getenv("KGE_SPLIT_LATE")) return std::max(-1, atoi(getenv("KGE_SPLIT_LATE")));
+#endif
+    const int64_t row_bytes = D * 4 * (is_split(fn) ? 2 : 1);
+    if (row_bytes >= 4096 && fn == KGE_INTERHT) return 5;
+    return -1;
+}
+
+static bool planner_split_fits(const kge_step_planner* sp, int R, Split s, const char** why) {
+    const char* none;
+    if (!why) why = &none;
+    if (!split_valid(sp->B, R, s.G, s.L)) return *why = "the rows do not fit the groups", false;
+    const int64_t ng = split_groups(sp->B, R, s.G, s.L);
+    if (plan_words_g(ng, sp->N, R) * 4 > sp->plan_bytes)
+        return *why = "the plan buffers are too small (kge_step_planner_plan_size)", false;
+    if (s.G > 0 && planner_form(sp).waves != kTileSharedWaves) return *why = "an even split needs a 12-wave step", false;
+    if (s.L > 0) {
+        if (ng < 8) return *why = "late rows need a step that plans at least 8 groups", false;
+        const int64_t cap = planner_capacity(sp, R);
+        if (cap <= 0 || 8 * ng > cap) return *why = "late rows need 8 blocks resident beside the scoring blocks", false;
+    }
+    return true;
+}
+
+static void planner_take_split(kge_step_planner* sp, Split s) {
+    const int64_t ng = split_groups(sp->B, sp->rows, s.G, s.L);
+    if (ng > sp->groups) sp->clk = nullptr;
+    sp->groups = ng;
+    sp->split = s;
+    sp->plan_blocks = s.L > 0 ? 8 : sp->rule_plan_blocks;
+    sp->split_set = 1;
+}
+
 static int planner_rows(kge_step_planner* sp) {
     if (!sp->rows) {
         sp->rows = planned_rows_rule(sp->t, sp->B, sp->N, planner_form(sp).waves, sp->plan_bytes,
@@ -1110,7 +1162,20 @@
         if (plan_groups(sp->B, sp->rows) > sp->groups) sp->clk = nullptr;
         sp->groups = plan_groups(sp->B, sp->rows);
         const int64_t cap = sp->rule ? planner_capacity(sp, sp->rows) : 0;
-        sp->plan_blocks = (cap > 0 && 8 * sp->groups <= cap - 8) ? 8 : 0;
+        sp->plan_blocks = sp->rule_plan_blocks = (cap > 0 && 8 * sp->groups <= cap - 8) ? 8 : 0;
+    }
+    if (!sp->split_set) {
+        Split s = {0, 0};
+        ScoreParams tp;
+        const int late = planner_late_rows(sp->t.fn, sp->t.D);
+        if (sp->even_ask < 0 && late >= 0 && sp->rule && sp->plan_blocks == 8 &&
+            sp->rows > planned_tile_params(sp->t, sp->B, sp->N, tp)) {
+            s.G = (int)plan_groups(sp->B, sp->rows);
+            s.L = late;
+            if (s.L > 0 && !planner_split_fits(sp, sp->rows, s, nullptr)) s.L = 0;
+            if (!planner_split_fits(sp, sp->rows, s, nullptr)) s = {0, 0};
+        }
+        planner_take_split(sp, s);
     }
     return sp->rows;
 }
@@ -1122,7 +1187,8 @@
     ScoreParams tp;
     const int R0 = planned_tile_params(t, B, N, tp);
     int64_t words = 0;
-    for (int R = R0; R0 && R <= kTileMaxRows; ++R) words = std::max(words, plan_words(B, N, R));
+    for (int R = R0; R0 && R <= kTileMaxRows; ++R)
+        words = std::max(words, plan_words_g(std::max<int64_t>(plan_groups(B, R), 8) + 1, N, R));
     return words * 4;
 }
 
@@ -1189,6 +1255,21 @@
     }
     if (waves && sp->rows > 2 * waves)
         return fail(KGE_ENOTSUP, "kge_step_planner_set_form: this wave count changes the rows per group");
+    int eff = 0, d0 = 0, l0 = 0;
+    planned_sweep_defaults(sp->t.fn, sp->t.D, eff, d0, l0);
+    if (waves) eff = waves;
+    if (sp->split_set && sp->split.G > 0 && eff != kTileSharedWaves && (sp->even_ask > 0 || sp->cur >= 0))
+        return fail(KGE_ENOTSUP, sp->even_ask > 0
+                                     ? "kge_step_planner_set_form: the even split that was set needs 12 waves"
+                                     : "kge_step_planner_set_form: a plan made under the library's even split waits for "
+                                       "its step (12 waves); change the wave count before the first plan or after a "
+                                       "step without a next batch");
+    if (sp->split_set && sp->even_ask < 0 && sp->cur < 0) {
+        sp->split = {0, 0};
+        sp->split_set = 0;
+        if (sp->rows) sp->groups = plan_groups(sp->B, sp->rows);
+        sp->plan_blocks = sp->rule_plan_blocks;
+    }
     sp->waves = waves;
     sp->depth = depth;
     return ok();
@@ -1209,8 +1290,39 @@
         sp->groups = plan_groups(sp->B, rows);
     }
     sp->rule = rows == KGE_PLANNER_ROWS_RULE || (rows == 0 && planner_row_rule(sp->t.fn, sp->t.D));
-    sp->plan_blocks = 0;
+    sp->plan_blocks = sp->rule_plan_blocks = 0;
     sp->rows = chosen ? rows : 0;
+    sp->even_ask = sp->late_ask = chosen ? 0 : -1;
+    sp->split = {0, 0};
+    sp->split_set = 0;
+    return ok();
+}
+
+int kge_step_planner_set_split(kge_step_planner* sp, int even, int late_rows) {
+    if (!sp) return fail(KGE_EINVAL, "kge_step_planner_set_split: null pointer");
+    if (even < -1 || late_rows < -1 || (even <= 0 && late_rows > 0))
+        return fail(KGE_EINVAL, "kge_step_planner_set_split: even -1, 0 or the regular groups; late_rows -1 or 0 .. rows "
+                                "(only with an even split)");
+    if (even <= 0) {
+        sp->even_ask = even;
+        sp->late_ask = even < 0 ? -1 : 0;
+        if (sp->rows) sp->groups = plan_groups(sp->B, sp->rows);
+        sp->split = {0, 0};
+        sp->split_set = 0;
+        return ok();
+    }
+    const kge_step_planner before = *sp;
+    const int R = planner_rows(sp);
+    const char* why = "";
+    Split s = {even, late_rows < 0 ? std::max(0, planner_late_rows(sp->t.fn, sp->t.D)) : late_rows};
+    if (late_rows < 0 && s.L > 0 && !planner_split_fits(sp, R, s, nullptr)) s.L = 0;
+    if (!planner_split_fits(sp, R, s, &why)) {
+        *sp = before;
+        return fail(KGE_ENOTSUP, std::string("kge_step_planner_set_split: ") + why);
+    }
+    sp->even_ask = even;
+    sp->late_ask = late_rows;
+    planner_take_split(sp, s);
     return ok();
 }
 
@@ -1243,6 +1355,8 @@
         case KGE_PLANNER_ROWS: return sp->rows;
         case KGE_PLANNER_PLAN_BLOCKS:
             return !sp->rows ? 0 : (sp->plan_blocks > 0 && f.waves == kTileSharedWaves) ? (int)std::min<int64_t>(sp->plan_blocks, sp->groups) : (int)sp->groups;
+        case KGE_PLANNER_GROUPS: return sp->split_set ? sp->split.G : 0;
+        case KGE_PLANNER_LATE_ROWS: return sp->split_set ? sp->split.L : 0;
         default: return -1;
     }
 }
@@ -1278,7 +1392,8 @@
 int kge_step_planner_plan(kge_step_planner* sp, const int64_t* pos, const int64_t* neg, int64_t neg_ld, int mode) {
     if (!sp) return fail(KGE_EINVAL, "kge_step_planner_plan: null pointer");
     const int buf = sp->cur < 0 ? 0 : sp->cur;
-    const int rc = step_plan(sp->t, {mode, pos, neg, neg_ld, sp->B, sp->N}, sp->plans[buf], sp->stream, planner_rows(sp));
+    const int rows = planner_rows(sp);
+    const int rc = step_plan(sp->t, {mode, pos, neg, neg_ld, sp->B, sp->N}, sp->plans[buf], sp->stream, rows, sp->split);
     if (rc) return rc;
     sp->cur = buf;
     sp->mode = mode;
@@ -1297,7 +1412,7 @@
                                         {next_mode, next_pos, next_neg, next_neg_ld, sp->B, sp->N},
                                         nxt ? sp->plans[1 - sp->cur] : nullptr,
                                         {neg_scores, sp->N, out_neg, pos_scores, out_pos}, &sf, sp->stream, rows,
-                                        nullptr, sp->plan_blocks);
+                                        nullptr, sp->plan_blocks, sp->split);
     if (rc) return rc;
     ++sp->steps;
     if (nxt) {
diff --git a/customknowledgegraphembedding_amd/csrc/kge_device.h b/customknowledgegraphembedding_amd/csrc/kge_device.h
--- a/customknowledgegraphembedding_amd/csrc/kge_device.h
+++ b/customknowledgegraphembedding_amd/csrc/kge_device.h
@@ -894,13 +894,16 @@
     vecf<V> q2[G];
 };
 
-template <int NWV>
+template <int NWV, bool SPLIT = true>
 __device__ void tile_plan_group(const PlanArgs& a, int g, int* sm) {
     constexpr int NT = NWV * kWave, NB = kTileSortRel, MU = (kTileSortMaxB + NT - 1) / NT;
     const int t = threadIdx.x, lane = t & 63, w = t >> 6;
     const int R = a.R;
-    const int64_t g0 = (int64_t)g * R;
-    const int nr = (int)min<int64_t>(R, a.B - g0);
+    const int aG = SPLIT ? a.G : 0, aL = SPLIT ? a.L : 0;
+    const int64_t ng = split_groups(a.B, R, aG, aL);
+    int64_t g0;
+    int nr;
+    split_group_rows(a.B, R, aG, aL, g, g0, nr);
     int* brow = sm;
     int* hist = brow + kTileMaxRows;
     int* wc = hist + 8 * kTileBuckets;
@@ -1042,7 +1045,7 @@
             if (lane >= o) incl += y;
         }
         int run = incl - sum;
-        int* soff = a.plan + plan_soff(a.B, R) + (int64_t)g * 9;
+        int* soff = a.plan + plan_soff_g(ng, R) + (int64_t)g * 9;
         if ((lane * PL) % kTileBuckets == 0) soff[lane * PL / kTileBuckets] = run;
         if (lane == kWave - 1) soff[8] = incl;
 #pragma unroll
@@ -1052,7 +1055,7 @@
         }
     }
     __syncthreads();
-    int2* list = reinterpret_cast<int2*>(a.plan + plan_list(a.B, R)) + (int64_t)g * R * (a.N + 1);
+    int2* list = reinterpret_cast<int2*>(a.plan + plan_list_g(ng, R)) + (int64_t)g * R * (a.N + 1);
     if (in_regs) {
 #pragma unroll
         for (int u = 0; u < TPI; ++u)
@@ -1077,6 +1080,7 @@
         h[4] = R;
         h[5] = (int)a.nent;
         h[6] = a.sort;
+        h[7] = split_word(aG, aL);
     }
 }
 
@@ -1109,30 +1113,41 @@
     int* list = cntp + 4;
     const int t = threadIdx.x, lane = t & 63, w = t >> 6;
     if constexpr (PLANNED) {
-        if (p.tile_next.plan && (int)blockIdx.x >= p.tile_blocks) {
+        if ((SHARED || p.tile_next.plan) && (int)blockIdx.x >= p.tile_blocks) {
             if constexpr (SHARED) {
-                const int ng = (int)plan_groups(p.tile_next.B, p.tile_next.R);
-                for (int g = (int)blockIdx.x - p.tile_blocks; g < ng; g += p.tile_plan_blocks) {
-                    tile_plan_group<NWV>(p.tile_next, g, reinterpret_cast<int*>(tile_smem));
-                    __syncthreads();
+                if (p.tile_next.plan) {
+                    const int ng = (int)split_groups(p.tile_next.B, p.tile_next.R, p.tile_next.G, p.tile_next.L);
+                    for (int g = (int)blockIdx.x - p.tile_blocks; g < ng; g += p.tile_plan_blocks) {
+                        tile_plan_group<NWV>(p.tile_next, g, reinterpret_cast<int*>(tile_smem));
+                        __syncthreads();
+                    }
                 }
             } else {
-                tile_plan_group<NWV>(p.tile_next, (int)blockIdx.x - p.tile_blocks, reinterpret_cast<int*>(tile_smem));
+                tile_plan_group<NWV, false>(p.tile_next, (int)blockIdx.x - p.tile_blocks, reinterpret_cast<int*>(tile_smem));
             }
 #ifdef KGE_PROFILING_KNOBS
             if (p.tile_clk && t == 0) {
-                long long* const pc = p.tile_clk + (int64_t)p.tile_blocks * kSweepClkMarks + 2 * ((int)blockIdx.x - p.tile_blocks);
+                long long* const pc = p.tile_clk + (int64_t)(p.tile_blocks + (p.tile_late > 0 ? 8 : 0)) * kSweepClkMarks +
+                                      2 * ((int)blockIdx.x - p.tile_blocks);
                 pc[0] = clk_entry;
                 pc[1] = wall_clock64();
             }
 #endif
-            return;
+            if constexpr (SHARED) {
+                if (p.tile_late <= 0) return;
+                __syncthreads();
+            } else {
+                return;
+            }
         }
     }
     const int x = (int)(blockIdx.x & 7);
     const int gi = (int)(blockIdx.x >> 3);
-    const int64_t g0 = (int64_t)gi * R;
-    const int nr = (int)min<int64_t>(R, p.B - g0);
+    [[maybe_unused]] const bool late = PLANNED && SHARED && (int)blockIdx.x >= p.tile_blocks;
+    int64_t g0;
+    int nr;
+    [[maybe_unused]] const int sG = (PLANNED && SHARED) ? p.tile_groups : 0, sL = (PLANNED && SHARED) ? p.tile_late : 0;
+    split_group_rows(p.B, R, sG, sL, gi, g0, nr);
     if (nr <= 0) return;
     const int64_t S = (p.c_rows + 7) / 8;
     const int64_t e_lo = min((int64_t)x * S, p.c_rows), e_hi = min(p.c_rows, e_lo + S);
@@ -1146,19 +1161,20 @@
     if constexpr (PLANNED) {
         const int* pl = p.tile_plan;
         pmeta = reinterpret_cast<const int4*>(pl + kPlanHdr) + (int64_t)gi * R;
-        const int2* plist = reinterpret_cast<const int2*>(pl + plan_list(p.B, R)) + (int64_t)gi * R * (p.N + 1);
+        const int64_t png = split_groups(p.B, R, sG, sL);
+        const int2* plist = reinterpret_cast<const int2*>(pl + plan_list_g(png, R)) + (int64_t)gi * R * (p.N + 1);
         constexpr bool TWO = NWV < kTileRows;
         static_assert(TWO || kTileMaxRows <= 2 * NWV, "two rows per wave (8 and 12 waves: the host caps the rows)");
-        const int* so = pl + plan_soff(p.B, R) + (int64_t)gi * 9;
+        const int* so = pl + plan_soff_g(png, R) + (int64_t)gi * 9;
         const bool hasA = w < nr, hasB = TWO && w + NWV < nr;
         const int rA = hasA ? w : 0, rB = hasB ? w + NWV : rA;
-        const int h0 = pl[0], h1 = pl[1], h2 = pl[2], h3 = pl[3], h4 = pl[4], h5 = pl[5], h6 = pl[6];
+        const int h0 = pl[0], h1 = pl[1], h2 = pl[2], h3 = pl[3], h4 = pl[4], h5 = pl[5], h6 = pl[6], h7 = pl[7];
         const int plo = so[x], phi = so[x + 1];
         const int4 mA = pmeta[rA], mB = pmeta[rB];
         const int4 ml = pmeta[min(lane, R - 1)];
         const int mode = CH ? KGE_HEAD_BATCH : KGE_TAIL_BATCH;
         if (h0 != kPlanMagic || h1 != (int)p.B || h2 != (int)p.N || h3 != mode || h4 != R || h5 != (int)p.c_rows ||
-            (h6 != 0) != (p.tile_sort != 0)) {
+            (h6 != 0) != (p.tile_sort != 0) || h7 != split_word(sG, sL)) {
             if (x == 0)
                 for (int r = w; r < nr; r += NWV) {
                     for (int64_t n = lane; n < p.N; n += kWave) p.out[(g0 + r) * p.out_ld + n] = __builtin_nanf("");
@@ -1486,12 +1502,12 @@
     constexpr bool has_board = BOARD;
     const rsrc_t brs = make_rsrc(has_board ? p.tile_board + x * kSweepBoardLine : nullptr, has_board ? kSweepBoardLine * 4u : 0u);
     const uint32_t boff_ld = (uint32_t)(lane & (kSweepBoardLine - 1)) * 4u;
-    const uint32_t boff_st = t == 0 ? (uint32_t)gi * 4u : kSweepBoardLine * 4u;
+    const uint32_t boff_st = (t == 0 && !late) ? (uint32_t)gi * 4u : kSweepBoardLine * 4u;
     const int btag = p.tile_tag << kSweepTagShift;
-    const bool bpeer = has_board && lane < (p.tile_blocks >> 3) && lane != gi;
+    const bool bpeer = has_board && !late && lane < (p.tile_blocks >> 3) && lane != gi;
     int bv = 0;
 #ifdef KGE_PROFILING_KNOBS
-    long long* const bclk = (PLANNED && p.tile_clk) ? p.tile_clk + ((int64_t)x * (p.tile_blocks >> 3) + gi) * kSweepClkMarks : nullptr;
+    long long* const bclk = (PLANNED && p.tile_clk) ? p.tile_clk + ((int64_t)x * ((p.tile_blocks >> 3) + (p.tile_late > 0 ? 1 : 0)) + gi) * kSweepClkMarks : nullptr;
     long long* const clk = w == 0 ? bclk : nullptr;
     int cmark = 0;
     if (clk && lane == 0) {
diff --git a/customknowledgegraphembedding_amd/csrc/kge_internal.h b/customknowledgegraphembedding_amd/csrc/kge_internal.h
--- a/customknowledgegraphembedding_amd/csrc/kge_internal.h
+++ b/customknowledgegraphembedding_amd/csrc/kge_internal.h
@@ -145,11 +145,33 @@
 constexpr int kPlanMagic = 0x4B475031;
 constexpr int kPlanHdr = 16;
 __host__ __device__ inline int64_t plan_groups(int64_t B, int R) { return (B + R - 1) / R; }
-__host__ __device__ inline int64_t plan_soff(int64_t B, int R) { return kPlanHdr + plan_groups(B, R) * R * 4; }
-__host__ __device__ inline int64_t plan_list(int64_t B, int R) { return (plan_soff(B, R) + plan_groups(B, R) * 9 + 3) & ~(int64_t)3; }
-__host__ __device__ inline int64_t plan_words(int64_t B, int64_t N, int R) {
-    return plan_list(B, R) + plan_groups(B, R) * R * (N + 1) * 2;
-}
+__host__ __device__ inline int64_t split_groups(int64_t B, int R, int G, int L) {
+    return G > 0 ? G + (L > 0 ? 1 : 0) : plan_groups(B, R);
+}
+__host__ __device__ inline int split_word(int G, int L) { return G > 0 ? (G << 8) | L : 0; }
+__host__ __device__ inline void split_group_rows(int64_t B, int R, int G, int L, int g, int64_t& g0, int& nr) {
+    if (G <= 0) {
+        g0 = (int64_t)g * R;
+        nr = (int)(B - g0 < R ? B - g0 : R);
+        return;
+    }
+    const int reg = (int)B - L, q = reg / G, rem = reg - q * G;
+    if (g < G) {
+        g0 = (int64_t)g * q + (g < rem ? g : rem);
+        nr = q + (g < rem ? 1 : 0);
+    } else {
+        g0 = reg;
+        nr = g == G ? L : 0;
+    }
+}
+__host__ __device__ inline bool split_valid(int64_t B, int R, int G, int L) {
+    if (G <= 0) return G == 0 && L == 0;
+    return L >= 0 && L <= R && L < (1 << 8) && G < (1 << 22) && B - L >= G && B - L <= (int64_t)G * R;
+}
+__host__ __device__ inline int64_t plan_soff_g(int64_t ng, int R) { return kPlanHdr + ng * R * 4; }
+__host__ __device__ inline int64_t plan_list_g(int64_t ng, int R) { return (plan_soff_g(ng, R) + ng * 9 + 3) & ~(int64_t)3; }
+__host__ __device__ inline int64_t plan_words_g(int64_t ng, int64_t N, int R) { return plan_list_g(ng, R) + ng * R * (N + 1) * 2; }
+__host__ __device__ inline int64_t plan_words(int64_t B, int64_t N, int R) { return plan_words_g(plan_groups(B, R), N, R); }
 struct PlanArgs {
     const int64_t* pos;
     const int64_t* neg;
@@ -157,6 +179,7 @@
     int64_t B, N, nent, nrel;
     int mode;
     int R;
+    int G, L;
     int sort;
     int* plan;
 };
@@ -202,6 +225,8 @@
     int tile_blocks;
     PlanArgs tile_next;
     int tile_plan_blocks;
+    int tile_groups;
+    int tile_late;
     struct {
         const int64_t* truth;
         const int64_t* fptr;
@@ -296,7 +321,9 @@
 };
 constexpr int kTileSharedWaves = 12;
 inline bool tile_plan_shared(const ScoreParams& p) {
-    return p.tile_next.plan && p.tile_plan_blocks < plan_groups(p.tile_next.B, p.tile_next.R);
+    if (p.tile_groups > 0) return true;
+    return p.tile_next.plan &&
+           p.tile_plan_blocks < split_groups(p.tile_next.B, p.tile_next.R, p.tile_next.G, p.tile_next.L);
 }
 
 struct AdamArgs {
diff --git a/customknowledgegraphembedding_amd/ops.py b/customknowledgegraphembedding_amd/ops.py
--- a/customknowledgegraphembedding_amd/ops.py
+++ b/customknowledgegraphembedding_amd/ops.py
@@ -206,13 +206,16 @@
     def set_rows(self, rows):
         check(self._lib.kge_step_planner_set_rows(self._h, int(rows)), "kge_step_planner_set_rows")
 
+    def set_split(self, even=-1, late_rows=-1):
+        check(self._lib.kge_step_planner_set_split(self._h, int(even), int(late_rows)), "kge_step_planner_set_split")
+
     def set_lead(self, lead):
         check(self._lib.kge_step_planner_set_lead(self._h, int(lead)), "kge_step_planner_set_lead")
 
     def form(self):
         return {k: int(self._lib.kge_step_planner_get(self._h, i))
                 for k, i in (("waves", 0), ("depth", 1), ("lead", 2), ("throttle", 3), ("tag", 4), ("rows", 6),
-                             ("plan_blocks", 7))}
+                             ("plan_blocks", 7), ("groups", 8), ("late_rows", 9))}
 
     def set_modulus(self, modulus):
         check(self._lib.kge_step_planner_set_modulus(self._h, float(modulus)), "kge_step_planner_set_modulus")
diff --git a/include/kge_hip.h b/include/kge_hip.h
--- a/include/kge_hip.h
+++ b/include/kge_hip.h
@@ -119,11 +119,14 @@
 #define KGE_PLANNER_TAG 4
 #define KGE_PLANNER_ROWS 6
 #define KGE_PLANNER_PLAN_BLOCKS 7
+#define KGE_PLANNER_GROUPS 8
+#define KGE_PLANNER_LATE_ROWS 9
 int kge_step_planner_get(const kge_step_planner* planner, int what);
 int64_t kge_step_planner_plan_size(int fn, int64_t nentity, int64_t ent_ld, int64_t nrelation, int64_t rel_ld,
                                    int64_t rel_off, int64_t B, int64_t N, int64_t D);
 #define KGE_PLANNER_ROWS_RULE (-1)
 int kge_step_planner_set_rows(kge_step_planner* planner, int rows);
+int kge_step_planner_set_split(kge_step_planner* planner, int even, int late_rows);
 int kge_step_planned_rows(int fn, int64_t nentity, int64_t ent_ld, int64_t nrelation, int64_t rel_ld, int64_t rel_off,
                           int64_t B, int64_t N, int64_t D, int waves, int64_t capacity, int* out);
 int kge_step_planner_set_clocks(kge_step_planner* planner, void* clocks, int64_t clocks_bytes);
```

Measured after the change: 1.641 billion triples/s, median of 6. Within noise of the previous version (+0.9%).
